# tridivb/attention_based_tbn

Hardware: AMD Instinct MI355X
Metric: clips/sec (3-seg RGB+Flow+Audio TBN fwd+bwd) (higher is better)
Workload: dtype f32; 1 GPU; BASELINE config 4: RGB+Flow+Audio async, attention off, 3 segments, 224x224 frames + 1.279 s (256x256) spectrogram, train step fwd+loss+bwd+clip+SGD; batch_per_gpu=32, global_batch=32, segments=3, parallelism=single, launch_plans=committed (bench_plans.json)

## Files before the change

### attention_based_tbn_amd/_lib.py

```python
import ctypes as C
import os

_HERE = os.path.dirname(os.path.abspath(__file__))
LIB_PATH = os.path.join(_HERE, "libtbn_hip.so")
if os.environ.get("TBN_LIB"):
    import sys as _sys
    LIB_PATH = os.path.abspath(os.environ["TBN_LIB"])
    print(f"[tbn] TBN_LIB set: loading {LIB_PATH} instead of the shipped libtbn_hip.so", file=_sys.stderr)

c_fp = C.c_void_p
c_i = C.c_int
c_sz = C.c_size_t
c_f = C.c_float


class ConvInfo(C.Structure):
    _fields_ = [("name", C.c_char * 64), ("cin", c_i), ("cout", c_i), ("ksize", c_i), ("stride", c_i),
                ("pad", c_i), ("weight_offset", c_sz), ("channel_offset", c_sz)]


class BackboneParams(C.Structure):
    _fields_ = [("weight", c_fp), ("bias", c_fp), ("gamma", c_fp), ("beta", c_fp), ("running_mean", c_fp),
                ("running_var", c_fp), ("momentum", c_f), ("eps", c_f), ("side_stream", c_fp), ("flags", c_i),
                ("weight_planes", c_fp)]
# ... 44 lines not shown
    _fields_ = [("param", c_fp), ("grad", c_fp), ("exp_avg", c_fp), ("exp_avg_sq", c_fp), ("count", c_sz),
                ("step_size", c_f), ("inv_sqrt_bc2", c_f)]


class JpegGeometry(C.Structure):
    _fields_ = [("width", c_i), ("height", c_i), ("components", c_i), ("hsamp", c_i * 3), ("vsamp", c_i * 3),
                ("blocks_w", c_i * 3), ("blocks_h", c_i * 3), ("restart_interval", c_i), ("coef_count", c_sz)]


class FramesClip(C.Structure):
    _fields_ = [("first_img", c_i), ("box_x", c_i), ("box_y", c_i), ("box_w", c_i), ("box_h", c_i), ("resized_w", c_i),
                ("resized_h", c_i), ("crop_x", c_i), ("crop_y", c_i), ("flip", c_i), ("out_row", c_i), ("reserved", c_i)]


SIGNATURES = {
    "tbn_version": (c_i, []),
    "tbn_capabilities": (c_i, []),
    "tbn_last_error": (C.c_char_p, []),
    "tbn_profile_enable": (c_i, [c_i]),
    "tbn_profile_reset": (c_i, []),
    "tbn_profile_num_entries": (c_i, []),
    "tbn_profile_entry": (c_i, [c_i, C.c_char_p, c_i, C.POINTER(C.c_long), C.POINTER(C.c_double),
                                C.POINTER(C.c_double)]),
    "tbn_profile_entry_bytes": (c_i, [c_i, C.POINTER(C.c_double)]),
    "tbn_timeline_enable": (c_i, [c_i]),
    "tbn_timeline_dump": (c_i, [C.c_char_p]),
    "tbn_diag_mfma_burst": (c_i, [c_fp, c_i, c_i, C.POINTER(C.c_double), c_fp]),
    "tbn_backbone_plan_create": (c_i, [c_i, c_i, c_i, c_i, C.POINTER(C.c_void_p)]),
    "tbn_backbone_plan_destroy": (None, [C.c_void_p]),
    "tbn_backbone_num_convs": (c_i, [C.c_void_p]),
    "tbn_backbone_conv_info": (c_i, [C.c_void_p, c_i, C.POINTER(ConvInfo)]),
    "tbn_backbone_weight_floats": (c_sz, [C.c_void_p]),
    "tbn_backbone_channel_floats": (c_sz, [C.c_void_p]),
    "tbn_backbone_workspace_bytes": (c_sz, [C.c_void_p, c_i]),
    "tbn_backbone_out_shape": (c_i, [C.c_void_p, C.POINTER(c_i), C.POINTER(c_i), C.POINTER(c_i)]),
    "tbn_backbone_num_streams": (c_i, [C.c_void_p]),
    "tbn_backbone_rider_launches": (c_i, [C.c_void_p, C.POINTER(c_i), C.POINTER(c_i)]),
    "tbn_backbone_tensor_info": (c_i, [C.c_void_p, C.c_char_p, c_i, C.POINTER(C.c_long), C.POINTER(c_i),
                                       C.POINTER(c_i), C.POINTER(c_i)]),
    "tbn_backbone_launch_info": (c_i, [C.c_void_p, C.c_char_p, c_i, C.POINTER(c_i)]),
    "tbn_backbone_plan_export_bytes": (c_sz, [C.c_void_p]),
    "tbn_backbone_plan_export": (c_i, [C.c_void_p, C.c_void_p, c_sz]),
    "tbn_backbone_plan_import": (c_i, [C.c_void_p, C.c_void_p, c_sz]),
    "tbn_backbone_plan_fingerprint": (C.c_ulonglong, [C.c_void_p]),
    "tbn_backbone_forward": (c_i, [C.c_void_p, c_i, c_fp, C.POINTER(BackboneParams), c_fp, c_sz,
                                   C.POINTER(C.c_void_p), c_fp]),
    "tbn_backbone_weight_planes_bytes": (c_sz, [C.c_void_p, c_i]),
    "tbn_backbone_split_weights": (c_i, [C.c_void_p, c_fp, c_i, c_fp, c_fp]),
    "tbn_backbone_autotune": (c_i, [C.c_void_p, c_i, C.POINTER(BackboneParams), c_fp, c_sz, c_fp]),
    "tbn_backbone_backward": (c_i, [C.c_void_p, c_fp, C.POINTER(BackboneParams), C.POINTER(BackboneGrads), c_fp,
                                    c_sz, c_fp]),
    "tbn_backbone_flip_weights": (c_i, [C.c_void_p, C.POINTER(BackboneParams), c_fp, c_sz, c_fp]),
    "tbn_conv2d_fwd": (c_i, [c_fp, c_i, c_fp, c_fp, c_fp, c_i] + [c_i] * 10 + [c_fp, c_fp, c_fp, c_fp]),
    "tbn_conv2d_stat_tiles": (c_i, [c_i] * 8),
    "tbn_conv_weight_planes_bytes": (c_sz, [c_i, c_i, c_i, c_i]),
    "tbn_conv_split_weights": (c_i, [c_fp, c_i, c_i, c_i, c_i, c_fp, c_fp]),
    "tbn_conv2d_fwd_tile": (c_i, [c_fp, c_i, c_fp, c_fp, c_fp, c_i] + [c_i] * 10 + [c_fp, c_i, c_i, c_fp]),
    "tbn_conv2d_dgrad": (c_i, [c_fp, c_i, c_fp, c_fp, c_i] + [c_i] * 9 + [c_fp, c_fp]),
    "tbn_conv_partial_rows": (c_i, [C.POINTER(ConvDesc), c_i, c_i]),
    "tbn_conv_launch": (c_i, [C.POINTER(ConvDesc), c_i, c_i, c_fp, c_fp]),
    "tbn_conv_launch_pair": (c_i, [C.POINTER(ConvDesc), C.POINTER(ConvDesc), c_i, c_i, c_i, c_fp, c_fp, c_fp]),
    "tbn_conv2d_wgrad_workspace_floats": (c_sz, [c_i] * 8),
    "tbn_conv2d_wgrad": (c_i, [c_fp, c_i, c_fp, c_i, c_fp] + [c_i] * 8 + [c_fp, c_fp]),
    "tbn_stem_geometry": (c_i, [c_i, c_i, c_i, c_i, C.POINTER(c_i)]),
    "tbn_stem_workspace_floats": (c_sz, [c_i] * 6),
    "tbn_stem_conv_fwd": (c_i, [c_fp, c_fp, c_fp, c_fp] + [c_i] * 8 + [c_fp, c_fp, c_fp] + [c_i] * 3 + [c_fp, c_fp]),
    "tbn_stem_conv_wgrad": (c_i, [c_fp, c_i, c_fp, c_fp] + [c_i] * 8 + [c_fp, c_fp]),
    "tbn_linear_fwd": (c_i, [c_fp, c_i, c_fp, c_fp, c_fp, c_i, c_i, c_i, c_i, c_i, c_fp]),
    "tbn_linear_dgrad": (c_i, [c_fp, c_i, c_fp, c_fp, c_i, c_i, c_i, c_i, c_i, c_fp, c_fp]),
    "tbn_linear_wgrad_workspace_floats": (c_sz, [c_i, c_i, c_i]),
    "tbn_linear_wgrad": (c_i, [c_fp, c_i, c_fp, c_i, c_fp, c_fp, c_i, c_i, c_i, c_fp, c_fp]),
    "tbn_bn_workspace_floats": (c_sz, [c_i, c_i]),
    "tbn_bn_relu_train_fwd": (c_i, [c_fp, c_i, c_i, c_fp, c_fp, c_fp, c_fp, c_f, c_f, c_fp, c_fp, c_fp, c_fp, c_fp,
                                    c_i, c_fp, c_fp]),
    "tbn_bn_relu_train_bwd": (c_i, [c_fp, c_i, c_fp, c_i, c_i, c_fp, c_fp, c_fp, c_fp, c_fp, c_fp, c_fp, c_fp, c_fp]),
    "tbn_bn_stats_partials": (c_i, [c_fp, c_i, c_i, c_i, c_fp, C.POINTER(c_i), c_fp]),
    "tbn_bn_fwd_batch": (c_i, [C.POINTER(BnFwdDesc), c_i, c_f, c_f, c_fp]),
    "tbn_bn_bwd_partial_floats": (c_sz, [c_i, c_i]),
    "tbn_bn_bwd_batch": (c_i, [C.POINTER(BnBwdDesc), c_i, c_fp]),
    "tbn_bn_relu_maxpool_train_fwd": (c_i, [c_fp, c_i, c_i, c_i, c_i, c_fp, c_fp, c_fp, c_fp, c_f, c_f, c_fp, c_fp, c_fp,
                                            c_fp, c_fp, c_i, c_fp, c_i, c_i, c_i, c_i, c_fp, c_fp]),
    "tbn_bn_relu_maxpool_train_bwd": (c_i, [c_fp, c_i, c_fp, c_fp, c_i, c_i, c_i, c_i, c_i, c_i, c_i, c_i, c_fp, c_fp,
                                            c_fp, c_fp, c_fp, c_fp, c_fp, c_fp, c_fp]),
    "tbn_bn_res_apply": (c_i, [c_fp, c_i, c_i, c_i, c_fp, c_fp, c_fp, c_i, c_i, c_fp, c_i, c_fp]),
    "tbn_bn_res_fwd": (c_i, [c_fp, c_i, c_i, c_i, c_fp, c_i, c_i, c_fp, c_fp, c_fp, c_fp, c_f, c_f, c_fp, c_fp, c_fp,
                             c_fp, c_fp, c_i, c_i, c_fp, c_i, c_fp]),
    "tbn_bn_res_bwd_workspace_floats": (c_sz, [c_i, c_i]),
    "tbn_bn_res_bwd": (c_i, [c_fp, c_i, c_fp, c_i, c_fp, c_i, c_i, c_i, c_fp, c_fp, c_fp, c_i, c_fp, c_i, c_fp, c_i, c_i,
                             c_fp, c_fp, c_fp, c_fp]),
    "tbn_maxpool3_fwd": (c_i, [c_fp, c_i, c_fp, c_i, c_fp] + [c_i] * 8 + [c_fp]),
    "tbn_maxpool3_bwd": (c_i, [c_fp, c_i, c_fp, c_fp, c_i] + [c_i] * 9 + [c_fp]),
    "tbn_avgpool3_fwd": (c_i, [c_fp, c_i, c_fp, c_i] + [c_i] * 5 + [c_fp]),
    "tbn_spatial_mean_fwd": (c_i, [c_fp, c_i, c_fp, c_i] + [c_i] * 5 + [c_fp]),
    "tbn_spatial_mean_bwd": (c_i, [c_fp, c_i, c_fp, c_i] + [c_i] * 5 + [c_fp]),
    "tbn_pe_concat_fwd": (c_i, [c_fp, c_i, c_fp, c_fp, c_i, c_i, c_i, c_i, c_i, c_fp]),
    "tbn_groupnorm_fwd": (c_i, [c_fp, c_fp, c_fp, c_fp, c_fp, c_fp, c_i, c_i, c_i, c_i, c_f, c_fp]),
    "tbn_groupnorm_bwd": (c_i, [c_fp] * 8 + [c_i] * 4 + [c_fp]),
    "tbn_colsum": (c_i, [c_fp, c_i, c_fp, c_i, c_i, c_fp]),
    "tbn_mha_q1_fwd": (c_i, [c_fp] * 6 + [c_i] * 4 + [c_f, c_fp]),
    "tbn_mha_q1_bwd": (c_i, [c_fp] * 8 + [c_i] * 4 + [c_f, c_fp]),
    "tbn_mha_fwd": (c_i, [c_fp, c_i, c_fp, c_i, c_fp, c_i, c_fp, c_fp, c_i, c_fp, c_fp] + [c_i] * 5 + [c_f, c_fp]),
    "tbn_mha_bwd": (c_i, [c_fp, c_i, c_fp, c_fp, c_i, c_fp, c_i, c_fp, c_i, c_fp, c_fp, c_fp, c_fp, c_i, c_fp, c_i, c_fp,
                          c_i] + [c_i] * 5 + [c_f, c_fp]),
    "tbn_attn_weights_fwd": (c_i, [c_fp, c_i, c_fp, c_f, c_i, c_fp, c_fp, c_fp, c_i, c_i, c_i, c_fp]),
    "tbn_attn_weights_bwd": (c_i, [c_fp, c_fp, c_fp, c_f, c_fp, c_i, c_i, c_i, c_fp]),
    "tbn_attn_reg_fwd": (c_i, [c_fp, c_i, c_fp, c_i, c_i, c_i, c_i, c_i, c_i, c_f, c_i, c_f, c_f, c_f, c_i, c_f, c_i, c_fp, c_fp,
                               c_fp]),
    "tbn_attn_reg_bwd": (c_i, [c_fp, c_fp, c_i, c_fp, c_i, c_fp, c_i, c_i, c_i, c_i, c_i, c_f, c_i, c_f, c_f, c_f, c_i, c_f,
                               c_i, c_fp, c_i, c_fp]),
    "tbn_weighted_sum_fwd": (c_i, [c_fp, c_fp, c_fp, c_i, c_i, c_i, c_i, c_fp]),
    "tbn_weighted_sum_bwd": (c_i, [c_fp, c_i, c_fp, c_fp, c_i, c_i, c_i, c_fp]),
    "tbn_segment_mean_fwd": (c_i, [c_fp, c_fp, c_i, c_i, c_i, c_fp]),
    "tbn_segment_mean_bwd": (c_i, [c_fp, c_fp, c_i, c_i, c_i, c_fp]),
    "tbn_dropout_fwd": (c_i, [c_fp, c_fp, c_f, c_fp, c_fp, c_sz, c_fp]),
    "tbn_ce_heads_fwd": (c_i, [c_fp, c_i, c_i, c_i, C.POINTER(c_i), C.POINTER(c_i), C.POINTER(C.c_void_p), c_fp, c_fp, c_fp, c_fp]),
    "tbn_ce_heads_bwd": (c_i, [c_fp, c_i, c_i, c_i, C.POINTER(c_i), C.POINTER(c_i), c_fp, c_fp, c_fp]),
    "tbn_mul_mask": (c_i, [c_fp, c_fp, c_fp, c_sz, c_fp]),
    "tbn_relu_mask_bwd": (c_i, [c_fp, c_fp, c_fp, c_fp, c_sz, c_fp]),
    "tbn_stft_twiddle_floats": (c_sz, []),
    "tbn_stft_make_twiddle": (c_i, [c_fp]),
    "tbn_stft_logpower": (c_i, [c_fp, c_i, c_i, c_fp, c_fp, c_f, c_fp]),
    "tbn_stft_windows": (c_i, [c_fp, c_fp, c_i, c_i, c_fp, c_fp, c_f, c_i, c_fp, c_fp, c_fp]),
    "tbn_attn_prior_loud": (c_i, [c_fp, c_i, c_i, c_i, c_i, c_fp, c_fp, c_fp]),
    "tbn_opt_num_partials": (c_i, [C.POINTER(OptTensor), c_i]),
    "tbn_opt_sqnorm_partials": (c_i, [C.POINTER(OptTensor), c_i, c_fp, c_fp]),
    "tbn_opt_clip_coef": (c_i, [c_fp, c_i, c_f, c_fp, c_fp, c_fp]),
    "tbn_opt_scale_grads": (c_i, [C.POINTER(OptTensor), c_i, c_fp, c_fp]),
    "tbn_opt_sgd_step": (c_i, [C.POINTER(OptTensor), c_i, c_f, c_f, c_f, c_fp, c_fp]),
    "tbn_opt_adam_step": (c_i, [C.POINTER(AdamTensor), c_i, c_f, c_f, c_f, c_f, c_fp, c_fp]),
    "tbn_topk_correct": (c_i, [c_fp, c_i, c_fp, c_i, c_i, c_i, c_fp, c_fp, c_fp, c_fp]),
    "tbn_frames_to_tensor": (c_i, [c_fp] + [c_i] * 16 + [c_fp, c_fp, c_i, c_i, c_fp, c_fp]),
    "tbn_frames_to_tensor_crops": (c_i, [c_fp] + [c_i] * 10 + [C.POINTER(c_i), C.POINTER(c_i)] + [c_i] * 5 +
                                   [c_fp, c_fp, c_i, c_i, c_fp, c_fp]),
    "tbn_frames_to_tensor_batch": (c_i, [c_fp] + [c_i] * 4 + [C.POINTER(FramesClip), c_fp] + [c_i] * 5 +
                                   [c_fp, c_fp, c_i, c_i, c_fp, c_i, c_fp]),
    "tbn_jpeg_parse": (c_i, [C.c_char_p, c_sz, C.POINTER(JpegGeometry)]),
    "tbn_jpeg_entropy_decode": (c_i, [C.c_char_p, c_sz, C.POINTER(JpegGeometry), c_fp, c_fp]),
    "tbn_jpeg_workspace_bytes": (c_sz, [C.POINTER(JpegGeometry), c_i]),
    "tbn_jpeg_reconstruct": (c_i, [c_fp, c_fp, c_i, C.POINTER(JpegGeometry), c_i, c_fp, c_fp, c_fp]),
    "tbn_jpeg_scan_pack_bytes": (c_sz, [c_sz, c_i]),
    "tbn_jpeg_scan_pack": (c_i, [C.c_char_p, c_sz, C.POINTER(JpegGeometry), c_fp, c_sz, c_i, c_fp, C.POINTER(c_i),
                                 C.POINTER(c_sz)]),
    "tbn_jpeg_entropy_workspace_bytes": (c_sz, [C.POINTER(JpegGeometry), c_i]),
    "tbn_jpeg_entropy_decode_dev": (c_i, [c_fp, c_sz, c_fp, c_i, C.POINTER(JpegGeometry), c_i, c_fp, c_fp, c_fp, c_fp, c_fp]),
}

_lib = None


class TbnHipError(RuntimeError):
    pass


def lib():
    global _lib
    if _lib is None:
        if not os.path.exists(LIB_PATH):
            raise TbnHipError(
                f"{LIB_PATH} not found: build it with `python -m attention_based_tbn_amd.build` "
                "(hipcc --offload-arch=gfx950).  There is no CPU fallback for the TBN hot path.")
        import torch
        handle = C.CDLL(LIB_PATH)
        for name, (res, args) in SIGNATURES.items():
            fn = getattr(handle, name)
            fn.restype = res
            fn.argtypes = args
        _lib = handle
# ... 35 lines not shown
```

### attention_based_tbn_amd/core/models/bn_inception.py

```python
import ctypes as C
import os
import weakref
from collections import OrderedDict

import torch
import torch.nn as nn

from ... import _lib
from ..._lib import BUCKET_CB, BackboneGrads, BackboneParams, ConvInfo, TbnHipError, call, lib, ptr, stream_ptr
from ... import ops

_BLOCKS = [("3a", True, True), ("3b", True, True), ("3c", False, False), ("4a", True, True), ("4b", True, True),
           ("4c", True, True), ("4d", True, True), ("4e", False, False), ("5a", True, True), ("5b", True, True)]


def reference_conv_order():
    names = ["conv1_7x7_s2", "conv2_3x3_reduce", "conv2_3x3"]
    for b, has1, hasp in _BLOCKS:
        p = "inception_" + b
        if has1:
            names.append(p + "_1x1")
        names += [p + "_3x3_reduce", p + "_3x3", p + "_double_3x3_reduce", p + "_double_3x3_1", p + "_double_3x3_2"]
        if hasp:
            names.append(p + "_pool_proj")
# ... 156 lines not shown
            module._last_flip = weakref.ref(f)
        ctx.need_grad = need_grad
        ctx.eval_mode = not training
        return out

    @staticmethod
    def backward(ctx, dout):
        if ctx.needs_input_grad[0]:
            raise TbnHipError("BNInception: the gradient with respect to the input frames is not implemented (the "
                              "first conv's data gradient is never formed); detach the input")
        if not ctx.need_grad:
            if ctx.eval_mode and any(ctx.needs_input_grad[1:7]):
                raise TbnHipError("BNInception: backward through an eval-mode backbone (running-statistics BN) is not "
                                  "implemented; call .train() for fine-tuning or wrap inference in torch.no_grad()")
            return (None,) * 9
        weight, bias, gamma, beta = ctx.saved_tensors
        plan, ws, module = ctx.plan, ctx.ws, ctx.module
        N, H, W, Cc = plan.out_shape
        st = stream_ptr()
        if ctx.freq_only or dout.dim() != 2 or dout.stride(1) != 1 or dout.dtype != torch.float32:
            dout = dout.contiguous().float()
        dout_ld = Cc if ctx.freq_only else dout.stride(0)
        dfeat = torch.empty(plan.out_shape, device=dout.device, dtype=torch.float32)
        call("tbn_spatial_mean_bwd", ptr(dout), dout_ld, ptr(dfeat), Cc, N, H, W, Cc, int(ctx.freq_only), st)
        dw = torch.empty_like(weight)
        db = torch.empty_like(bias)
        need = ctx.needs_input_grad
        bn_first, bn_rest = need[3] or need[5], need[4] or need[6]
        dg = torch.zeros_like(gamma) if (bn_first or bn_rest) else None
        dbe = torch.zeros_like(beta) if (bn_first or bn_rest) else None
        flipped = ctx.flip.done and ctx.flip.version == weight._version
        prm = BackboneParams(ptr(weight), ptr(bias), ptr(gamma), ptr(beta), ptr(module.running_mean),
                             ptr(module.running_var), 0.1, 1e-5, module._side_stream_ptr(),
                             module._engine_flags() | (4 if flipped else 0))
        aux = 0
        if module.use_aux_stream and not torch.cuda.is_current_stream_capturing():
            cur = torch.cuda.current_stream()
            a = module._aux_streams.get(cur.cuda_stream)
            if a is None:
                a = module._aux_streams[cur.cuda_stream] = torch.cuda.Stream(device=dout.device)
            aux = a.cuda_stream
        bucket_fn = module.grad_bucket_fn if need[1] else None
        waits, failure = [], []

        def on_bucket(_user, first, count):
            try:
                w = bucket_fn(module.flat_weight, dw, int(first), int(first) + int(count))
                if w is not None:
                    waits.append(w)
            except BaseException as e:
                failure.append(e)

        cb = BUCKET_CB(on_bucket) if bucket_fn is not None else BUCKET_CB()
        grads = BackboneGrads(ptr(dw), ptr(db), ptr(dg), ptr(dbe), 2 if bn_rest else (1 if bn_first else 0), aux, cb, 0)
        call("tbn_backbone_backward", plan.handle, ptr(dfeat), C.byref(prm), C.byref(grads), ptr(ws), ws.numel(), st)
        ctx.token = None
        for w in waits:
            w()
        if failure:
            raise failure[0]
        n0 = module.first_bn_channels
        return (None, dw if need[1] else None, db if need[2] else None,
                dg[:n0] if need[3] else None, dg[n0:] if need[4] else None,
                dbe[:n0] if need[5] else None, dbe[n0:] if need[6] else None, None, None)


class BNInception(nn.Module):

    def __init__(self, num_classes=1000, in_channels=3):
        super().__init__()
        self.in_channels = in_channels
        self.num_classes = num_classes
        self.is_audio = False
        self.attend = False
        self.feature_size = 1024
        self.eval_chunk = 256
        self.autotune = True
        self.use_aux_stream = True
        self._aux_streams = {}
        self.use_branch_streams = True
        self._side_streams = {}
        self.use_riders = True
        self.stem_wgrad_last = False
        self._conv_math = "f32"
        self._conv_math_layers = "3x3"
        self._planes = None
        self._planes_key = None
        self._last_flip = None
        self._out_slot = None
        self.plan_sync = None
        self.grad_bucket_fn = None
        self._plans = OrderedDict()
        probe = C.c_void_p()
        call("tbn_backbone_plan_create", in_channels, 1, 64, 64, C.byref(probe))
        self._layers = OrderedDict()
        info = ConvInfo()
        for i in range(lib().tbn_backbone_num_convs(probe)):
            call("tbn_backbone_conv_info", probe, i, C.byref(info))
            self._layers[info.name.decode()] = dict(cin=info.cin, cout=info.cout, k=info.ksize, stride=info.stride,
                                                    pad=info.pad, w_off=info.weight_offset, c_off=info.channel_offset)
        nw, nc = lib().tbn_backbone_weight_floats(probe), lib().tbn_backbone_channel_floats(probe)
        lib().tbn_backbone_plan_destroy(probe)
        order = reference_conv_order()
        assert sorted(order) == sorted(self._layers), "engine layer table does not match the reference graph"
        self._order = order
        assert self._layers["conv1_7x7_s2"]["c_off"] == 0
        self.first_bn_channels = self._layers["conv1_7x7_s2"]["cout"]
        n0 = self.first_bn_channels
        self.flat_weight = nn.Parameter(torch.empty(nw))
        self.flat_bias = nn.Parameter(torch.empty(nc))
        self.bn_weight_first = nn.Parameter(torch.ones(n0))
        self.bn_weight_rest = nn.Parameter(torch.ones(nc - n0))
        self.bn_bias_first = nn.Parameter(torch.zeros(n0))
        self.bn_bias_rest = nn.Parameter(torch.zeros(nc - n0))
        self.register_buffer("running_mean", torch.zeros(nc))
        self.register_buffer("running_var", torch.ones(nc))
        self.register_buffer("num_batches_tracked", torch.zeros(len(order), dtype=torch.long))
        self.last_linear = nn.Linear(1024, num_classes)
        self.reset_parameters()

    def reset_parameters(self):
        with torch.no_grad():
            for name, L in self._layers.items():
                w = self.conv_weight(name)
                nn.init.kaiming_uniform_(w, a=5 ** 0.5)
                bound = 1.0 / (L["cin"] * L["k"] * L["k"]) ** 0.5
                self.flat_bias[L["c_off"]:L["c_off"] + L["cout"]].uniform_(-bound, bound)
            torch.autograd.graph.increment_version(self.flat_weight)

    def conv_weight(self, name):
        L = self._layers[name]
        n = L["cout"] * L["k"] * L["k"] * L["cin"]
        return self.flat_weight.data[L["w_off"]:L["w_off"] + n].view(L["cout"], L["k"], L["k"], L["cin"]).permute(
            0, 3, 1, 2)

    def _chan(self, name, flat_first, flat_rest=None):
        L = self._layers[name]
        a, b = L["c_off"], L["c_off"] + L["cout"]
        if flat_rest is None:
            return flat_first.data[a:b]
        n0 = self.first_bn_channels
        return flat_first.data[a:b] if b <= n0 else flat_rest.data[a - n0:b - n0]

    def reference_param_views(self, flat):
        n0 = self.first_bn_channels
        for name in self._order:
            L = self._layers[name]
            n = L["cout"] * L["k"] * L["k"] * L["cin"]
            a, b = L["c_off"], L["c_off"] + L["cout"]
            yield name + ".weight", flat["flat_weight"][L["w_off"]:L["w_off"] + n].view(
                L["cout"], L["k"], L["k"], L["cin"]).permute(0, 3, 1, 2)
            yield name + ".bias", flat["flat_bias"][a:b]
            first = b <= n0
            yield name + "_bn.weight", (flat["bn_weight_first"][a:b] if first else flat["bn_weight_rest"][a - n0:b - n0])
            yield name + "_bn.bias", (flat["bn_bias_first"][a:b] if first else flat["bn_bias_rest"][a - n0:b - n0])

    def named_reference_tensors(self):
        for i, name in enumerate(self._order):
            yield name + ".weight", self.conv_weight(name)
            yield name + ".bias", self._chan(name, self.flat_bias)
            yield name + "_bn.weight", self._chan(name, self.bn_weight_first, self.bn_weight_rest)
            yield name + "_bn.bias", self._chan(name, self.bn_bias_first, self.bn_bias_rest)
            yield name + "_bn.running_mean", self._chan(name, self.running_mean)
            yield name + "_bn.running_var", self._chan(name, self.running_var)
            yield name + "_bn.num_batches_tracked", self.num_batches_tracked[i]

# ... 19 lines not shown
                    continue
                dst.copy_(src)
            torch.autograd.graph.increment_version(self.flat_weight)
        if strict:
            child_prefixes = tuple(prefix + n + "." for n, _ in self.named_children())
            for key in state_dict:
                if key.startswith(prefix) and key not in own and not key.startswith(child_prefixes):
                    unexpected_keys.append(key)

    def set_bn_trainable(self, first, rest):
        self.bn_weight_first.requires_grad = self.bn_bias_first.requires_grad = first
        self.bn_weight_rest.requires_grad = self.bn_bias_rest.requires_grad = rest

    def _plan(self, frames, h, w):
        key = (frames, h, w)
        if key not in self._plans:
            if len(self._plans) >= 4:
                self._plans.popitem(last=False)
            self._plans[key] = _Plan(self.in_channels, frames, h, w)
        else:
            self._plans.move_to_end(key)
        return self._plans[key]

    def plan_fingerprints(self):
        return {k: p.fingerprint() for k, p in self._plans.items()}

    def flip_weights_early(self):
        f = self._last_flip() if getattr(self, "_last_flip", None) is not None else None
        self._last_flip = None
        if f is None or f.done or f.weight._version != f.version or torch.cuda.is_current_stream_capturing():
            return False
        prm = BackboneParams(ptr(f.weight), 0, 0, 0, 0, 0, 0.1, 1e-5, 0, 0)
        call("tbn_backbone_flip_weights", f.plan.handle, C.byref(prm), ptr(f.ws), f.ws.numel(), stream_ptr())
        f.done = True
        return True

    CONV_MATH = {"f32": 0, "bf16x6": 8, "bf16x3": 16}

    @property
    def conv_math(self):
        return self._conv_math

    @conv_math.setter
    def conv_math(self, value):
        if value not in self.CONV_MATH:
            raise ValueError("conv_math must be one of %s, got %r" % (", ".join(map(repr, self.CONV_MATH)), value))
        self._conv_math = value
        if value == "f32":
            self._planes = self._planes_key = None

    CONV_MATH_LAYERS = ("3x3", "all")

    @property
    def conv_math_layers(self):
        return self._conv_math_layers

    @conv_math_layers.setter
    def conv_math_layers(self, value):
        if value not in self.CONV_MATH_LAYERS:
            raise ValueError("conv_math_layers must be one of %s, got %r"
                             % (", ".join(map(repr, self.CONV_MATH_LAYERS)), value))
        self._conv_math_layers = value
        if value != "all":
            self._planes = self._planes_key = None

    def _planes_on(self):
        return not self.training and self._conv_math != "f32" and self._conv_math_layers == "all"

    def _weight_planes(self, plan):
        w = self.flat_weight
        np_ = 6 if self._conv_math == "bf16x6" else 3
        key = (w.data_ptr(), w._version, self._conv_math)
        nbytes = lib().tbn_backbone_weight_planes_bytes(plan.handle, np_)
        if self._planes is None or self._planes.numel() != nbytes or self._planes.device != w.device:
            self._planes, self._planes_key = torch.empty(nbytes, dtype=torch.uint8, device=w.device), None
        capturing = torch.cuda.is_current_stream_capturing()
        if self._planes_key != key or capturing:
            call("tbn_backbone_split_weights", plan.handle, ptr(w), np_, ptr(self._planes), stream_ptr())
            if not capturing:
                self._planes_key = key
        return self._planes

    def _engine_flags(self):
        return ((1 if self.use_riders else 0) | (2 if self.stem_wgrad_last else 0)
                | (0 if self.training else self.CONV_MATH[self._conv_math]) | (32 if self._planes_on() else 0))

    def _side_stream_ptr(self):
        if not self.use_branch_streams or torch.cuda.is_current_stream_capturing():
            return 0
        cur = torch.cuda.current_stream()
        s = self._side_streams.get(cur.cuda_stream)
        if s is None:
            s = self._side_streams[cur.cuda_stream] = torch.cuda.Stream(device=cur.device)
        return s.cuda_stream

    def _run(self, x, freq_only):
        if not x.is_cuda:
            raise TbnHipError("BNInception: input is on the CPU; this backbone only runs on an MI355X via "
                              "libtbn_hip.so (no CPU fallback)")
        x = x.contiguous().float()
        args = (self.flat_weight, self.flat_bias, self.bn_weight_first, self.bn_weight_rest, self.bn_bias_first,
                self.bn_bias_rest, self, freq_only)
        if self.training or x.shape[0] <= self.eval_chunk:
            return _BackboneFn.apply(x, *args)
        outs = [_BackboneFn.apply(x[i:i + self.eval_chunk], *args) for i in range(0, x.shape[0], self.eval_chunk)]
        return torch.cat(outs, 0)

    def forward(self, x):
        freq = bool(self.is_audio and self.attend)
        out = self._run(x, freq)
        if freq:
            return out.permute(0, 2, 1).unsqueeze(2)
        return out

    def forward_sequence(self, x):
        return self._run(x, True)

    def features(self, x):
        x = x.contiguous().float()
        plan = self._plan(x.shape[0], x.shape[2], x.shape[3])
        ws = plan.workspace(False, x.device)
        gamma = torch.cat([self.bn_weight_first, self.bn_weight_rest])
        beta = torch.cat([self.bn_bias_first, self.bn_bias_rest])
        if self.training:
            raise TbnHipError("features(): only available in eval mode; use forward() for training")
        prm = BackboneParams(ptr(self.flat_weight), ptr(self.flat_bias), ptr(gamma), ptr(beta),
                             ptr(self.running_mean), ptr(self.running_var), 0.1, 1e-5, 0,
                             self.CONV_MATH[self._conv_math] | (32 if self._planes_on() else 0))
        if self._planes_on():
            prm.weight_planes = ptr(self._weight_planes(plan))
        feat_ptr = C.c_void_p()
        call("tbn_backbone_forward", plan.handle, 0, ptr(x), C.byref(prm), ptr(ws), ws.numel(), C.byref(feat_ptr),
             stream_ptr())
        N, H, W, Cc = plan.out_shape
        off = (feat_ptr.value - ws.data_ptr()) // 4
        nhwc = ws.view(torch.float32)[off:off + N * H * W * Cc].view(N, H, W, Cc).clone()
        return nhwc.permute(0, 3, 1, 2)

    def logits(self, features):
        nhwc = features.permute(0, 2, 3, 1).contiguous()
        if self.is_audio and self.attend:
            return ops.spatial_mean(nhwc, True).permute(0, 2, 1).unsqueeze(2)
        return ops.spatial_mean(nhwc, False)


def bninception(in_channels, modality, pretrained="imagenet", model_dir="", is_audio=False, attend=False,
                state_dict=None):
    num_classes = 1000
    data_dict = state_dict
    if pretrained is not None:
        if pretrained == "kinetics":
            num_classes = 400
            file = os.path.join(model_dir, "kinetics_bninception_flow.pth")
        elif pretrained == "imagenet":
            file = os.path.join(model_dir, "imagenet_bninception_rgb.pth")
        if data_dict is None:
            data_dict = torch.load(file, map_location="cpu")
    model = BNInception(num_classes=num_classes, in_channels=in_channels)
    if data_dict is not None:
        data_dict = dict(data_dict)
        if modality == "Audio":
            data_dict["conv1_7x7_s2.weight"] = data_dict["conv1_7x7_s2.weight"].mean(dim=1).unsqueeze(dim=1)
            own = model.state_dict()
            for k in [k for k in own.keys() if k not in data_dict]:
                data_dict[k] = own[k]
            for k in [k for k in data_dict.keys() if k not in own]:
                del data_dict[k]
# ... 8 lines not shown
```

### attention_based_tbn_amd/csrc/api.hip

```cpp
#include <cstdarg>
#include <cstdio>
#include <cstdlib>
#include <cstring>

#include "tbn_common.h"
#include "tbn_kernels.h"
#include "../../include/tbn_hip.h"

static thread_local char g_err[512] = "";

void tbn_set_error(const char* fmt, ...) {
  va_list ap;
  va_start(ap, fmt);
  vsnprintf(g_err, sizeof(g_err), fmt, ap);
  va_end(ap);
}

#if TBN_EXPERIMENT
int tbn_env_int(const char* name, int def, int lo, int hi) {
  const char* e = getenv(name);
  if (e == nullptr || *e == 0) return def;
  char* end = nullptr;
  const long v = strtol(e, &end, 10);
  if (end == e || *end != 0 || v < lo || v > hi) {
// ... 7 lines not shown

#define TBN_TRY(expr)                \
  do {                               \
    int rc__ = (expr);               \
    if (rc__ != TBN_OK) return rc__; \
  } while (0)

static void conv_geom(ConvP* p, int n, int h, int w, int cin, int cout, int k, int stride, int pad) {
  memset(p, 0, sizeof(*p));
  p->N = n;
  p->H = h;
  p->W = w;
  p->OH = (h + 2 * pad - k) / stride + 1;
  p->OW = (w + 2 * pad - k) / stride + 1;
  p->Cin = cin;
  p->Cout = cout;
  p->R = p->S = k;
  p->stride = stride;
  p->pad = pad;
  p->up = 1;
  p->M = n * p->OH * p->OW;
  p->K = k * k * cin;
}

#include <map>
#include <atomic>
#include <mutex>
#include <string>
#include <vector>
namespace {
struct ProfRec {
  int name;
  double flops, bytes;
  hipEvent_t a, b;
  bool used;
};
struct ProfAgg {
  long launches = 0;
  double ms = 0, flops = 0, bytes = 0;
};
std::mutex g_prof_mu;
bool g_prof_on = false;
bool g_prof_layers = false;
std::string g_prof_label;
thread_local const char* g_prof_prefix = nullptr;
std::vector<std::string> g_prof_names;
std::vector<ProfRec> g_prof_recs;
std::vector<hipEvent_t> g_prof_pool;
std::map<std::string, ProfAgg> g_prof_agg;
std::vector<std::string> g_prof_keys;
int g_prof_open = -1;

hipEvent_t prof_event() {
  if (!g_prof_pool.empty()) {
    hipEvent_t e = g_prof_pool.back();
    g_prof_pool.pop_back();
    return e;
  }
  hipEvent_t e = nullptr;
  (void)hipEventCreate(&e);
  return e;
}
void prof_collect() {
  for (auto& r : g_prof_recs) {
    if (r.used) {
      (void)hipEventSynchronize(r.b);
      float ms = 0.f;
      (void)hipEventElapsedTime(&ms, r.a, r.b);
      ProfAgg& a = g_prof_agg[g_prof_names[r.name]];
      a.launches += 1;
      a.ms += ms;
      a.flops += r.flops;
      a.bytes += r.bytes;
    }
    g_prof_pool.push_back(r.a);
    g_prof_pool.push_back(r.b);
  }
  g_prof_recs.clear();
  g_prof_keys.clear();
  for (auto& kv : g_prof_agg) g_prof_keys.push_back(kv.first);
}
}

void tbn_prof_begin(const char* kernel, double flops, hipStream_t st, double bytes) {
  if (!g_prof_on) return;
  std::lock_guard<std::mutex> lk(g_prof_mu);
  std::string key = g_prof_prefix ? std::string(g_prof_prefix) + kernel : std::string(kernel);
  if (g_prof_layers) key += " | " + g_prof_label;
  kernel = key.c_str();
  int idx = -1;
  for (size_t i = 0; i < g_prof_names.size(); ++i)
    if (g_prof_names[i] == kernel) idx = (int)i;
  if (idx < 0) {
    g_prof_names.push_back(kernel);
    idx = (int)g_prof_names.size() - 1;
  }
  ProfRec r;
  r.name = idx;
  r.flops = flops;
  r.bytes = bytes;
  r.a = prof_event();
  r.b = prof_event();
  r.used = false;
  (void)st;
  g_prof_recs.push_back(r);
  g_prof_open = (int)g_prof_recs.size() - 1;
}
bool tbn_prof_enabled() { return g_prof_on; }

namespace {
struct TlRec {
  std::string name;
  void* stream;
  hipEvent_t a, b;
};
std::mutex g_tl_mu;
std::atomic<bool> g_tl_on{false};
std::vector<TlRec> g_tl;
void tl_free_events() {
  for (auto& r : g_tl) {
    if (r.a) (void)hipEventDestroy(r.a);
    if (r.b) (void)hipEventDestroy(r.b);
  }
  g_tl.clear();
}
}
bool tbn_tl_on(hipStream_t st) {
  if (!g_tl_on.load(std::memory_order_relaxed)) return false;
  hipStreamCaptureStatus cs = hipStreamCaptureStatusNone;
  if (hipStreamIsCapturing(st, &cs) != hipSuccess) {
    (void)hipGetLastError();
    return false;
  }
  return cs == hipStreamCaptureStatusNone;
}
void tbn_tl_events(const char* name, hipStream_t st, hipEvent_t* start, hipEvent_t* stop) {
  std::lock_guard<std::mutex> lk(g_tl_mu);
  TlRec r;
  r.name = name;
  r.stream = (void*)st;
  r.a = r.b = nullptr;
  (void)hipEventCreate(&r.a);
  (void)hipEventCreate(&r.b);
  *start = r.a;
  *stop = r.b;
  g_tl.push_back(r);
}
extern "C" int tbn_timeline_enable(int on) {
  std::lock_guard<std::mutex> lk(g_tl_mu);
  if (on) {
    (void)hipDeviceSynchronize();
    tl_free_events();
  }
  g_tl_on.store(on != 0, std::memory_order_relaxed);
  return TBN_OK;
}
extern "C" int tbn_timeline_dump(const char* path) {
  TBN_REQUIRE(path != nullptr, "timeline_dump: null path");
  (void)hipDeviceSynchronize();
  std::lock_guard<std::mutex> lk(g_tl_mu);
  FILE* f = fopen(path, "w");
  TBN_REQUIRE(f != nullptr, "timeline_dump: cannot open %s", path);
  fprintf(f, "Kernel_Name,Queue_Id,Start_Timestamp,End_Timestamp\n");
  if (!g_tl.empty()) {
    const hipEvent_t ref = g_tl[0].a;
    for (auto& r : g_tl) {
      float a = 0.f, d = 0.f;
      if (hipEventElapsedTime(&a, ref, r.a) != hipSuccess || hipEventElapsedTime(&d, r.a, r.b) != hipSuccess) {
        (void)hipGetLastError();
        continue;
      }
      std::string nm = r.name;
      for (auto& ch : nm)
        if (ch == ',' || ch == '"') ch = ';';
      const long long s0 = (long long)((double)a * 1e6) + 1000000000ll;
      fprintf(f, "%s,%p,%lld,%lld\n", nm.c_str(), r.stream, s0, s0 + (long long)((double)d * 1e6));
    }
  }
  fclose(f);
  if (!g_tl_on.load(std::memory_order_relaxed)) tl_free_events();
  return TBN_OK;
}
bool tbn_prof_launch_events(hipEvent_t* start, hipEvent_t* stop) {
  if (!g_prof_on) return false;
  std::lock_guard<std::mutex> lk(g_prof_mu);
  if (g_prof_open < 0 || g_prof_recs[g_prof_open].used || !g_prof_recs[g_prof_open].a || !g_prof_recs[g_prof_open].b)
    return false;
  g_prof_recs[g_prof_open].used = true;
  *start = g_prof_recs[g_prof_open].a;
  *stop = g_prof_recs[g_prof_open].b;
  return true;
}
void tbn_prof_label(const char* label) {
  if (!g_prof_on || !g_prof_layers) return;
  std::lock_guard<std::mutex> lk(g_prof_mu);
  g_prof_label = label;
}
void tbn_prof_end(hipStream_t st) {
  if (!g_prof_on) return;
  std::lock_guard<std::mutex> lk(g_prof_mu);
  (void)st;
  g_prof_open = -1;
}

__global__ __launch_bounds__(256) void mfma_burst_kernel(float* sink, int iters) {
  f32x16 a0, a1, a2, a3;
#pragma unroll
  for (int e = 0; e < 16; ++e) a0[e] = a1[e] = a2[e] = a3[e] = 0.f;
  const float x = 1e-3f * (float)(threadIdx.x & 63) + 0.5f, y = 1.0f - 1e-3f * (float)(threadIdx.x >> 6);
  for (int i = 0; i < iters; ++i) {
#pragma unroll
    for (int k = 0; k < 4; ++k) {
      a0 = __builtin_amdgcn_mfma_f32_32x32x2f32(x, y, a0, 0, 0, 0);
      a1 = __builtin_amdgcn_mfma_f32_32x32x2f32(y, x, a1, 0, 0, 0);
      a2 = __builtin_amdgcn_mfma_f32_32x32x2f32(x, x, a2, 0, 0, 0);
      a3 = __builtin_amdgcn_mfma_f32_32x32x2f32(y, y, a3, 0, 0, 0);
    }
  }
  float s = 0.f;
#pragma unroll
  for (int e = 0; e < 16; ++e) s += (a0[e] + a1[e]) + (a2[e] + a3[e]);
  if (s == -1.2345f) sink[0] = s;
}

extern "C" {

int tbn_version(void) { return 102 | (TBN_EXPERIMENT ? 0x10000 : 0); }

int tbn_capabilities(void) { return TBN_CAP_CONV_BF16X | TBN_CAP_CONV_BF16X_PLANES | TBN_CAP_FRAMES_CROPS | TBN_CAP_ATTN_GENERAL | TBN_CAP_ATTN_REG | TBN_CAP_AUDIO_LAYER | TBN_CAP_STEM_OPS | TBN_CAP_BN_BATCH_OPS; }

int tbn_diag_mfma_burst(float* sink, int workgroups, int iters, double* flops, void* stream) {
  TBN_REQUIRE(sink != nullptr && workgroups > 0 && workgroups <= 65536 && iters > 0, "diag_mfma_burst: bad argument");
  hipLaunchKernelGGL(mfma_burst_kernel, dim3(workgroups), dim3(256), 0, (hipStream_t)stream, sink, iters);
  TBN_CHECK_LAUNCH("mfma_burst");
  if (flops) *flops = (double)workgroups * 4.0 * (double)iters * 16.0 * 4096.0;
  return TBN_OK;
}

int tbn_profile_enable(int on) {
  std::lock_guard<std::mutex> lk(g_prof_mu);
  g_prof_on = on != 0;
  g_prof_layers = on == 2;
  return TBN_OK;
}
int tbn_profile_reset(void) {
  std::lock_guard<std::mutex> lk(g_prof_mu);
  prof_collect();
  g_prof_agg.clear();
  g_prof_keys.clear();
  return TBN_OK;
}
int tbn_profile_num_entries(void) {
  std::lock_guard<std::mutex> lk(g_prof_mu);
  prof_collect();
  return (int)g_prof_keys.size();
}
int tbn_profile_entry(int i, char* name, int name_len, long* launches, double* total_ms, double* total_flops) {
  std::lock_guard<std::mutex> lk(g_prof_mu);
  TBN_REQUIRE(i >= 0 && i < (int)g_prof_keys.size() && name && name_len > 0, "profile_entry: bad index");
  const ProfAgg& a = g_prof_agg[g_prof_keys[i]];
  snprintf(name, name_len, "%s", g_prof_keys[i].c_str());
  if (launches) *launches = a.launches;
  if (total_ms) *total_ms = a.ms;
  if (total_flops) *total_flops = a.flops;
  return TBN_OK;
}
int tbn_profile_entry_bytes(int i, double* total_alg_bytes) {
  std::lock_guard<std::mutex> lk(g_prof_mu);
  TBN_REQUIRE(i >= 0 && i < (int)g_prof_keys.size() && total_alg_bytes, "profile_entry_bytes: bad index");
  *total_alg_bytes = g_prof_agg[g_prof_keys[i]].bytes;
  return TBN_OK;
}
const char* tbn_last_error(void) { return g_err; }

int tbn_conv2d_stat_tiles(int n, int h, int w, int cin, int cout, int ksize, int stride, int pad) {
  ConvP p;
  conv_geom(&p, n, h, w, cin, cout, ksize, stride, pad);
  int mt, nt;
  tbn_conv_pick_tile(p.M, p.Cout, p.K, &mt, &nt);
  return cdiv(p.M, 128 * mt);
}
// ... 352 lines not shown
  wp.dy = dy;
  wp.dy_ld = dy_ld;
  wp.x = image;
  wp.N = n;
  wp.H = g.H;
  wp.W = g.W;
  wp.OH = g.OH;
  wp.OW = g.OW;
  wp.Cin = g.rows * g.kw;
  wp.Cout = cout;
  wp.R = g.rows;
  wp.S = 1;
  wp.taps = 1;
  wp.stride = g.stride;
  wp.pad = g.pad;
  wp.M = n * g.OH * g.OW;
  wp.cp = wp.x_ld = g.cp;
  wp.rl = g.kw;
  wp.mt = mt;
  wp.nt = nt;
  wp.alg_flops = 2.0 * wp.M * (double)cout * 49 * cin;
  TBN_TRY(tbn_launch_wgrad(wp, 1, dwpack, workspace + ws.wsplit, st));
  if (g.mode == 1) return tbn_launch_unpack_stem_wgrad_rows(dwpack, dweight, cout, cin, g.kw, st);
  return tbn_launch_unpack_stem_wgrad_s2d(dwpack, dweight, cout, cin, st);
}

namespace {
struct ProfPrefix {
  explicit ProfPrefix(const char* p) { g_prof_prefix = p; }
  ~ProfPrefix() { g_prof_prefix = nullptr; }
};
}

int tbn_linear_fwd(const float* x, int x_ld, const float* w, const float* bias, float* out, int out_ld, int m, int k,
                   int n, int relu, void* stream) {
  ProfPrefix scope("linear: ");
  return tbn_conv2d_fwd(x, x_ld, w, bias, out, out_ld, m, 1, 1, k, n, 1, 1, 0, CONV_EPI_PLAIN,
                        relu ? CONV_FLAG_RELU : 0, nullptr, nullptr, nullptr, stream);
}

int tbn_linear_dgrad(const float* dy, int dy_ld, const float* w, float* dx, int dx_ld, int m, int k, int n,
                     int accumulate, float* workspace, void* stream) {
  ProfPrefix scope("linear: ");
  return tbn_conv2d_dgrad(dy, dy_ld, w, dx, dx_ld, m, 1, 1, k, n, 1, 1, 0, accumulate, workspace, stream);
}

size_t tbn_linear_wgrad_workspace_floats(int m, int k, int n) { return tbn_wgrad_workspace_floats(m, n, k, 1); }

int tbn_linear_wgrad(const float* dy, int dy_ld, const float* x, int x_ld, float* dw, float* dbias, int m, int k,
                     int n, float* workspace, void* stream) {
  ProfPrefix scope("linear: ");
  TBN_TRY(tbn_conv2d_wgrad(dy, dy_ld, x, x_ld, dw, m, 1, 1, k, n, 1, 1, 0, workspace, stream));
  if (dbias) TBN_TRY(tbn_colsum(dy, dy_ld, dbias, m, n, stream));
  return TBN_OK;
}

size_t tbn_bn_workspace_floats(int p, int c) { return (size_t)tbn_bn_stats_parts(p, c) * 2 * c + 3 * (size_t)c; }

int tbn_bn_relu_train_fwd(const float* y, int p, int c, const float* gamma, const float* beta, float* running_mean,
                          float* running_var, float momentum, float eps, float* save_mean, float* save_rstd,
                          float* scale, float* shift, float* z, int z_ld, float* workspace, void* stream) {
  hipStream_t st = (hipStream_t)stream;
  int parts = 0;
  TBN_TRY(tbn_launch_bn_stats(y, c, p, c, workspace, &parts, st));
  TBN_TRY(tbn_launch_bn_finalize(workspace, parts, p, c, gamma, beta, nullptr, running_mean, running_var, momentum, eps,
                                 save_mean, save_rstd, scale, shift, st));
  Seg s;
  s.ptr = z;
  s.ld = z_ld;
  s.col_begin = 0;
  return tbn_launch_bn_apply(y, p, c, scale, shift, &s, 1, st);
}

int tbn_bn_relu_train_bwd(const float* dz, int dz_ld, const float* y, int p, int c, const float* save_mean,
                          const float* save_rstd, const float* scale, const float* shift, float* dy, float* dgamma,
                          float* dbeta, float* workspace, void* stream) {
  hipStream_t st = (hipStream_t)stream;
  CSeg s;
  s.ptr = dz;
  s.ld = dz_ld;
  s.col_begin = 0;
  const int parts = tbn_bn_bwd_parts(p, c);
  float* coef = workspace + (size_t)parts * 2 * c;
  TBN_TRY(tbn_launch_bn_bwd_reduce(&s, 1, y, p, c, scale, shift, save_mean, save_rstd, workspace, st));
  TBN_TRY(tbn_launch_bn_bwd_finalize(workspace, parts, p, c, scale, save_mean, save_rstd, coef, dgamma, dbeta, nullptr,
                                     st));
  return tbn_launch_bn_bwd_apply(&s, 1, y, p, c, scale, shift, coef, dy, st);
}

int tbn_bn_stats_partials(const float* y, int y_ld, int p, int c, float* partial, int* nparts, void* stream) {
  TBN_REQUIRE(y && partial && nparts, "bn_stats_partials: null pointer");
  return tbn_launch_bn_stats(y, y_ld, p, c, partial, nparts, (hipStream_t)stream);
}

size_t tbn_bn_bwd_partial_floats(int p, int c) {
  if (p < 1 || c < 4 || c > 1024 || c % 4 != 0) return 0;
  return (size_t)tbn_bn_bwd_parts(p, c) * 2 * c;
}

int tbn_bn_fwd_batch(const tbn_bn_fwd_desc* members, int n, float momentum, float eps, void* stream) {
  TBN_REQUIRE(members != nullptr, "bn_fwd_batch: null pointer");
  static thread_local BnFwdBatch b;
  memset(&b, 0, sizeof(b));
  b.n = n;
  b.momentum = momentum;
  b.eps = eps;
  for (int i = 0; i < n && n <= TBN_BN_MAXL; ++i) {
    const tbn_bn_fwd_desc& d = members[i];
    TBN_REQUIRE(d.y && d.partial && d.gamma && d.beta && d.save_mean && d.save_rstd && d.scale && d.shift,
                "bn_fwd_batch: null pointer in member %d", i);
    TBN_REQUIRE(d.running_mean == nullptr || d.running_var != nullptr, "bn_fwd_batch: member %d has running_mean without running_var", i);
    BnFwdLayer& L = b.l[i];
    L.y = d.y; L.y_ld = d.y_ld; L.P = d.p; L.C = d.c;
    L.partial = d.partial; L.pld = d.pld; L.nparts = d.nparts;
    L.gamma = d.gamma; L.beta = d.beta; L.conv_bias = d.conv_bias;
    L.running_mean = d.running_mean; L.running_var = d.running_var;
    L.save_mean = d.save_mean; L.save_rstd = d.save_rstd; L.scale = d.scale; L.shift = d.shift;
    L.nseg = d.nseg;
    for (int s = 0; s < 3 && s < d.nseg; ++s) {
      TBN_REQUIRE(d.seg[s].ptr != nullptr, "bn_fwd_batch: null pointer in segment %d of member %d", s, i);
      L.seg[s].ptr = d.seg[s].ptr; L.seg[s].ld = d.seg[s].ld; L.seg[s].col_begin = d.seg[s].col_begin;
    }
  }
  return tbn_launch_bn_fwd_multi(b, (hipStream_t)stream);
}

int tbn_bn_bwd_batch(const tbn_bn_bwd_desc* members, int n, void* stream) {
  TBN_REQUIRE(members != nullptr, "bn_bwd_batch: null pointer");
  static thread_local BnBwdBatch b;
  memset(&b, 0, sizeof(b));
  b.n = n;
  for (int i = 0; i < n && n <= TBN_BN_MAXL; ++i) {
    const tbn_bn_bwd_desc& d = members[i];
    TBN_REQUIRE(d.y && d.dy && d.scale && d.shift && d.mean && d.rstd && d.partial && d.coef,
                "bn_bwd_batch: null pointer in member %d", i);
    BnBwdLayer& L = b.l[i];
    L.nseg = d.nseg;
    for (int s = 0; s < 3 && s < d.nseg; ++s) {
      TBN_REQUIRE(d.dz[s].ptr != nullptr, "bn_bwd_batch: null pointer in segment %d of member %d", s, i);
      L.dz[s].ptr = d.dz[s].ptr; L.dz[s].ld = d.dz[s].ld; L.dz[s].col_begin = d.dz[s].col_begin;
    }
    L.y = d.y; L.dy = d.dy; L.y_ld = d.y_ld; L.P = d.p; L.C = d.c;
    L.scale = d.scale; L.shift = d.shift; L.mean = d.mean; L.rstd = d.rstd;
    L.partial = d.partial; L.ext_parts = d.ext_parts; L.coef = d.coef;
    L.dgamma = d.dgamma; L.dbeta = d.dbeta; L.dbias = d.dbias;
  }
  return tbn_launch_bn_bwd_multi(b, (hipStream_t)stream);
}

int tbn_bn_relu_maxpool_train_fwd(const float* y, int n, int h, int w, int c, const float* gamma, const float* beta,
                                  float* running_mean, float* running_var, float momentum, float eps, float* save_mean,
                                  float* save_rstd, float* scale, float* shift, float* pooled, int pooled_ld,
                                  uint8_t* argmax, int oh, int ow, int stride, int pad, float* workspace, void* stream) {
  hipStream_t st = (hipStream_t)stream;
  TBN_REQUIRE(y && pooled && argmax && workspace, "bn_relu_maxpool_train_fwd: null pointer");
  const int p = n * h * w;
  int parts = 0;
  TBN_TRY(tbn_launch_bn_stats(y, c, p, c, workspace, &parts, st));
  TBN_TRY(tbn_launch_bn_finalize(workspace, parts, p, c, gamma, beta, nullptr, running_mean, running_var, momentum, eps,
                                 save_mean, save_rstd, scale, shift, st));
  return tbn_launch_bn_apply_maxpool(y, n, h, w, c, scale, shift, pooled, pooled_ld, argmax, oh, ow, stride, pad, st);
}

int tbn_bn_relu_maxpool_train_bwd(const float* dpooled, int dpooled_ld, const uint8_t* argmax, const float* y, int n, int h,
                                  int w, int c, int oh, int ow, int stride, int pad, const float* save_mean,
                                  const float* save_rstd, const float* scale, const float* shift, float* dy,
                                  float* dgamma, float* dbeta, float* workspace, void* stream) {
  hipStream_t st = (hipStream_t)stream;
  TBN_REQUIRE(dpooled && argmax && y && dy && workspace, "bn_relu_maxpool_train_bwd: null pointer");
  const int p = n * h * w;
  const int parts = tbn_bn_bwd_pooled_parts(n, h, w, c, stride, pad);
  TBN_REQUIRE(parts <= tbn_bn_bwd_parts(p, c), "bn_relu_maxpool_train_bwd: workspace sized by tbn_bn_workspace_floats is too small");
  float* coef = workspace + (size_t)tbn_bn_bwd_parts(p, c) * 2 * c;
  TBN_TRY(tbn_launch_bn_bwd_reduce_pooled(dpooled, dpooled_ld, argmax, n, h, w, oh, ow, stride, pad, y, c, scale, shift,
                                          save_mean, save_rstd, workspace, st));
  TBN_TRY(tbn_launch_bn_bwd_finalize(workspace, parts, p, c, scale, save_mean, save_rstd, coef, dgamma, dbeta, nullptr, st));
  return tbn_launch_bn_bwd_apply_pooled(dpooled, dpooled_ld, argmax, n, h, w, oh, ow, stride, pad, y, c, scale, shift, coef,
                                        dy, st);
}

int tbn_maxpool3_fwd(const float* in, int in_ld, float* out, int out_ld, uint8_t* argmax, int n, int h, int w, int c,
                     int oh, int ow, int stride, int pad, void* stream) {
  return tbn_launch_maxpool_fwd(in, in_ld, out, out_ld, argmax, n, h, w, c, oh, ow, stride, pad, (hipStream_t)stream);
}
int tbn_maxpool3_bwd(const float* dout, int dout_ld, const uint8_t* argmax, float* din, int din_ld, int n, int h,
                     int w, int c, int oh, int ow, int stride, int pad, int accumulate, void* stream) {
  return tbn_launch_maxpool_bwd(dout, dout_ld, argmax, din, din_ld, n, h, w, c, oh, ow, stride, pad, accumulate,
                                (hipStream_t)stream);
}
int tbn_avgpool3_fwd(const float* in, int in_ld, float* out, int out_ld, int n, int h, int w, int c, int accumulate,
                     void* stream) {
  return tbn_launch_avgpool3_fwd(in, in_ld, out, out_ld, n, h, w, c, accumulate, (hipStream_t)stream);
}
int tbn_spatial_mean_fwd(const float* in, int in_ld, float* out, int out_ld, int n, int h, int w, int c,
                         int freq_only, void* stream) {
  return tbn_launch_spatial_mean_fwd(in, in_ld, out, out_ld, n, h, w, c, freq_only, (hipStream_t)stream);
}
int tbn_spatial_mean_bwd(const float* dout, int dout_ld, float* din, int din_ld, int n, int h, int w, int c,
                         int freq_only, void* stream) {
  return tbn_launch_spatial_mean_bwd(dout, dout_ld, din, din_ld, n, h, w, c, freq_only, (hipStream_t)stream);
}

}
```

### attention_based_tbn_amd/csrc/bn.hip

```cpp
#include "tbn_common.h"
#include "tbn_kernels.h"
#include "tbn_bn_dev.h"
#include "tbn_pool_dev.h"

static inline int pick_chunk(int P, int rp) {
  int pch = cdiv(P, 512);
  if (pch < 64) pch = 64;
  return cdiv(pch, rp) * rp;
}

__global__ __launch_bounds__(256) void bn_stats_kernel(const float* __restrict__ y, int ld, int P, int C, int pch,
                                                       float* __restrict__ partial) {
  __shared__ float red[2 * 2048];
  const int G = C >> 2, RP = 256 / G;
  const int tid = threadIdx.x, cg = tid % G, rs = tid / G;
  const int p0 = blockIdx.x * pch, p1 = min(P, p0 + pch);
  float4 s1 = make_float4(0, 0, 0, 0), s2 = s1;
  if (rs < RP)
    for (int p = p0 + rs; p < p1; p += RP) {
      const float4 v = *reinterpret_cast<const float4*>(y + (size_t)p * ld + cg * 4);
      s1.x += v.x; s1.y += v.y; s1.z += v.z; s1.w += v.w;
      s2.x = fmaf(v.x, v.x, s2.x); s2.y = fmaf(v.y, v.y, s2.y); s2.z = fmaf(v.z, v.z, s2.z); s2.w = fmaf(v.w, v.w, s2.w);
    }
  if (rs < RP) {
// ... 57 lines not shown
    }
  }
}

int tbn_launch_bn_finalize(const float* partial, int nparts, int P, int C, const float* gamma, const float* beta,
                           const float* conv_bias, float* running_mean, float* running_var, float momentum, float eps,
                           float* save_mean, float* save_rstd, float* scale, float* shift, hipStream_t st) {
  TBN_KLAUNCH(bn_finalize_kernel, dim3(cdiv(C, TBN_FIN_CH)), dim3(256), 0, st, partial, nparts, P, C, gamma, beta,
                     conv_bias, running_mean, running_var, momentum, eps, save_mean, save_rstd, scale, shift);
  TBN_CHECK_LAUNCH("bn_finalize");
  return TBN_OK;
}

struct Seg3 {
  Seg s[3];
  int n;
};
struct CSeg3 {
  CSeg s[3];
  int n;
};

__global__ __launch_bounds__(256) void bn_apply_kernel(const float* __restrict__ y, int P, int C,
                                                       const float* __restrict__ scale,
                                                       const float* __restrict__ shift, Seg3 segs, FastDiv divg) {
  const int G = C >> 2;
  const uint32_t total = (uint32_t)P * G;
  for (uint32_t i = blockIdx.x * 256u + threadIdx.x; i < total; i += gridDim.x * 256u) {
    const int p = (int)fdiv(i, divg), c = (int)(i - (uint32_t)p * (uint32_t)G) * 4;
    const float4 v = *reinterpret_cast<const float4*>(y + (size_t)p * C + c);
    const float4 sc = *reinterpret_cast<const float4*>(scale + c);
    const float4 sh = *reinterpret_cast<const float4*>(shift + c);
    float4 z;
    z.x = fmaxf(fmaf(v.x, sc.x, sh.x), 0.f);
    z.y = fmaxf(fmaf(v.y, sc.y, sh.y), 0.f);
    z.z = fmaxf(fmaf(v.z, sc.z, sh.z), 0.f);
    z.w = fmaxf(fmaf(v.w, sc.w, sh.w), 0.f);
    int sg = 0;
    if (segs.n > 1 && c >= segs.s[1].col_begin) sg = 1;
    if (segs.n > 2 && c >= segs.s[2].col_begin) sg = 2;
    *reinterpret_cast<float4*>(segs.s[sg].ptr + (size_t)p * segs.s[sg].ld + (c - segs.s[sg].col_begin)) = z;
  }
}

static inline int ew_grid(size_t items) {
  size_t g = (items + 255) / 256;
  return (int)(g > 4096 ? 4096 : (g < 1 ? 1 : g));
}

int tbn_launch_bn_apply(const float* y, int P, int C, const float* scale, const float* shift, const Seg* segs,
                        int nseg, hipStream_t st) {
  TBN_REQUIRE(C % 4 == 0 && nseg >= 1 && nseg <= 3, "bn_apply: bad C/nseg");
  Seg3 s3;
  s3.n = nseg;
  for (int i = 0; i < nseg; ++i) {
    s3.s[i] = segs[i];
    TBN_REQUIRE(segs[i].ld % 4 == 0 && segs[i].col_begin % 4 == 0, "bn_apply: segment pitch/offset must be x4");
  }
  TBN_REQUIRE((size_t)P * (C / 4) < (1ull << 31), "bn_apply: too many elements per call");
  TBN_KLAUNCH(bn_apply_kernel, dim3(ew_grid((size_t)P * C / 4)), dim3(256), 0, st, y, P, C, scale, shift, s3,
                     make_fastdiv((uint32_t)(C / 4)));
  TBN_CHECK_LAUNCH("bn_apply");
  return TBN_OK;
}

__global__ void bn_fold_kernel(const float* gamma, const float* beta, const float* mean, const float* var,
                               const float* bias, float eps, float* scale, float* shift, int C) {
  const int c = blockIdx.x * blockDim.x + threadIdx.x;
  if (c < C) {
    const float sc = gamma[c] / sqrtf(var[c] + eps);
    scale[c] = sc;
    shift[c] = fmaf((bias != nullptr ? bias[c] : 0.f) - mean[c], sc, beta[c]);
  }
}

int tbn_launch_bn_fold(const float* gamma, const float* beta, const float* mean, const float* var, const float* bias,
                       float eps, float* scale, float* shift, int C, hipStream_t st) {
  TBN_KLAUNCH(bn_fold_kernel, dim3(cdiv(C, 256)), dim3(256), 0, st, gamma, beta, mean, var, bias, eps, scale,
                     shift, C);
  TBN_CHECK_LAUNCH("bn_fold");
  return TBN_OK;
}

__global__ __launch_bounds__(256) void bn_apply_maxpool_kernel(const float* __restrict__ y, int N, int H, int W, int C,
                                                               const float* __restrict__ scale,
                                                               const float* __restrict__ shift,
                                                               float* __restrict__ out, int out_ld,
                                                               unsigned char* __restrict__ argmax, int OH, int OW,
                                                               int stride, int pad, PixDecode dec) {
  const int G = C >> 2;
  const uint32_t total = (uint32_t)N * OH * OW * G;
  const unsigned nb = gridDim.x, bid = blockIdx.x;
  const unsigned q8 = nb >> 3, r8 = nb & 7, xcd = bid & 7, idx = bid >> 3;
  const uint32_t b0 = (xcd < r8 ? xcd * (q8 + 1) : r8 * (q8 + 1) + (xcd - r8) * q8) + idx;
  for (uint32_t i = b0 * 256u + threadIdx.x; i < total; i += gridDim.x * 256u) {
    int g, ox, oy, n;
    uint32_t opix;
    pix_decode(dec, i, g, ox, oy, n, opix);
    const int y0 = oy * stride - pad, x0 = ox * stride - pad;
    const float4 sc = *reinterpret_cast<const float4*>(scale + g * 4);
    const float4 sh = *reinterpret_cast<const float4*>(shift + g * 4);
    float4 best = make_float4(-INFINITY, -INFINITY, -INFINITY, -INFINITY);
    int bx = 0, by = 0, bz = 0, bw = 0;
#pragma unroll
    for (int r = 0; r < 3; ++r)
#pragma unroll
      for (int s2 = 0; s2 < 3; ++s2) {
        const int iy = y0 + r, ix = x0 + s2;
        if ((unsigned)iy < (unsigned)H && (unsigned)ix < (unsigned)W) {
          const float4 v = *reinterpret_cast<const float4*>(y + ((size_t)(n * H + iy) * W + ix) * C + g * 4);
          float4 z;
          z.x = fmaxf(fmaf(v.x, sc.x, sh.x), 0.f);
          z.y = fmaxf(fmaf(v.y, sc.y, sh.y), 0.f);
          z.z = fmaxf(fmaf(v.z, sc.z, sh.z), 0.f);
          z.w = fmaxf(fmaf(v.w, sc.w, sh.w), 0.f);
          const int k = r * 3 + s2;
          if (z.x > best.x || z.x != z.x) { best.x = z.x; bx = k; }
          if (z.y > best.y || z.y != z.y) { best.y = z.y; by = k; }
          if (z.z > best.z || z.z != z.z) { best.z = z.z; bz = k; }
          if (z.w > best.w || z.w != z.w) { best.w = z.w; bw = k; }
        }
      }
    *reinterpret_cast<float4*>(out + (size_t)opix * out_ld + g * 4) = best;
    *reinterpret_cast<uint32_t*>(argmax + (size_t)opix * C + g * 4) =
        (uint32_t)bx | ((uint32_t)by << 8) | ((uint32_t)bz << 16) | ((uint32_t)bw << 24);
  }
}

int tbn_launch_bn_apply_maxpool(const float* y, int N, int H, int W, int C, const float* scale, const float* shift,
                                float* out, int out_ld, unsigned char* argmax, int OH, int OW, int stride, int pad,
                                hipStream_t st) {
  TBN_REQUIRE(C % 4 == 0 && out_ld % 4 == 0 && argmax != nullptr, "bn_apply_maxpool: bad C / pitch / argmax");
  size_t g = ((size_t)N * OH * OW * (C / 4) + 255) / 256;
  if (g > 8192) g = 8192;
  TBN_REQUIRE((size_t)N * H * W * (C / 4) < (1ull << 31), "bn_apply_maxpool: too many elements per call");
  TBN_KLAUNCH(bn_apply_maxpool_kernel, dim3((unsigned)(g < 1 ? 1 : g)), dim3(256), 0, st, y, N, H, W, C, scale,
                     shift, out, out_ld, argmax, OH, OW, stride, pad, make_pixdecode(C / 4, OW, OH));
  TBN_CHECK_LAUNCH("bn_apply_maxpool");
  return TBN_OK;
}

struct PoolGrad {
  const float* dout;
  const unsigned char* argmax;
  int dout_ld, H, W, OH, OW, C, stride, pad;
  FastDiv div_w, div_h;
};
__device__ __forceinline__ float4 pooled_grad(const PoolGrad& q, int p, int c) {
  const uint32_t row = fdiv((uint32_t)p, q.div_w);
  const int ix = p - (int)row * q.W;
  const uint32_t n = fdiv(row, q.div_h);
  const int iy = (int)row - (int)n * q.H;
  float4 acc = make_float4(0.f, 0.f, 0.f, 0.f);
  if (q.stride == 2 && q.pad == 0) {
    const int oyA = iy >> 1, ryA = iy & 1, oxA = ix >> 1, rxA = ix & 1;
    const bool vyA = oyA < q.OH, vyB = (ryA == 0) && (oyA >= 1);
    const bool vxA = oxA < q.OW, vxB = (rxA == 0) && (oxA >= 1);
    const int oy[2] = {vyA ? oyA : 0, vyB ? oyA - 1 : 0}, ry[2] = {ryA, 2};
    const int ox[2] = {vxA ? oxA : 0, vxB ? oxA - 1 : 0}, rx[2] = {rxA, 2};
    const bool vy[2] = {vyA, vyB}, vx[2] = {vxA, vxB};
    uint32_t am[4];
    float4 d[4];
#pragma unroll
    for (int a = 0; a < 2; ++a)
#pragma unroll
      for (int b = 0; b < 2; ++b) {
        const size_t opix = (size_t)((int)n * q.OH + oy[a]) * q.OW + ox[b];
        am[a * 2 + b] = *reinterpret_cast<const uint32_t*>(q.argmax + opix * q.C + c);
        d[a * 2 + b] = *reinterpret_cast<const float4*>(q.dout + opix * q.dout_ld + c);
      }
#pragma unroll
    for (int a = 0; a < 2; ++a)
#pragma unroll
      for (int b = 0; b < 2; ++b) {
        const uint32_t k = (uint32_t)(ry[a] * 3 + rx[b]);
        const uint32_t m = am[a * 2 + b];
        const bool v = vy[a] && vx[b];
        if (v && (m & 0xff) == k) acc.x += d[a * 2 + b].x;
        if (v && ((m >> 8) & 0xff) == k) acc.y += d[a * 2 + b].y;
        if (v && ((m >> 16) & 0xff) == k) acc.z += d[a * 2 + b].z;
        if (v && (m >> 24) == k) acc.w += d[a * 2 + b].w;
      }
    return acc;
  }
  const int oy_hi = min(q.OH - 1, (iy + q.pad) / q.stride);
  const int ox_hi = min(q.OW - 1, (ix + q.pad) / q.stride);
  for (int oy = oy_hi; oy >= 0; --oy) {
    const int r = iy - (oy * q.stride - q.pad);
    if (r > 2) break;
    for (int ox = ox_hi; ox >= 0; --ox) {
      const int s = ix - (ox * q.stride - q.pad);
      if (s > 2) break;
      const uint32_t k = (uint32_t)(r * 3 + s);
      const size_t opix = (size_t)((int)n * q.OH + oy) * q.OW + ox;
      const uint32_t am = *reinterpret_cast<const uint32_t*>(q.argmax + opix * q.C + c);
      const float4 d = *reinterpret_cast<const float4*>(q.dout + opix * q.dout_ld + c);
      if ((am & 0xff) == k) acc.x += d.x;
      if (((am >> 8) & 0xff) == k) acc.y += d.y;
      if (((am >> 16) & 0xff) == k) acc.z += d.z;
      if ((am >> 24) == k) acc.w += d.w;
    }
  }
  return acc;
}

template <bool POOLED>
__global__ __launch_bounds__(256) void bn_bwd_reduce_kernel(CSeg3 dz, PoolGrad pg, const float* __restrict__ y, int P,
                                                            int C, int pch, const float* __restrict__ scale,
                                                            const float* __restrict__ shift,
                                                            const float* __restrict__ mean,
                                                            const float* __restrict__ rstd,
                                                            float* __restrict__ partial) {
  __shared__ float red[2 * 2048];
  const int G = C >> 2, RP = 256 / G;
  const int tid = threadIdx.x, cg = tid % G, rs = tid / G, c = cg * 4;
  const int p0 = blockIdx.x * pch, p1 = min(P, p0 + pch);
  float4 s1 = make_float4(0, 0, 0, 0), s2 = s1;
  if (rs < RP) {
    int sg = 0;
    if (dz.n > 1 && c >= dz.s[1].col_begin) sg = 1;
    if (dz.n > 2 && c >= dz.s[2].col_begin) sg = 2;
    const float* dzp = POOLED ? nullptr : dz.s[sg].ptr + (c - dz.s[sg].col_begin);
    const int dld = dz.s[sg].ld;
    const float4 sc = *reinterpret_cast<const float4*>(scale + c);
    const float4 sh = *reinterpret_cast<const float4*>(shift + c);
    const float4 mu = *reinterpret_cast<const float4*>(mean + c);
    const float4 rs4 = *reinterpret_cast<const float4*>(rstd + c);
    for (int p = p0 + rs; p < p1; p += RP) {
      const float4 v = *reinterpret_cast<const float4*>(y + (size_t)p * C + c);
      const float4 d = POOLED ? pooled_grad(pg, p, c) : *reinterpret_cast<const float4*>(dzp + (size_t)p * dld);
      const float gx = fmaf(v.x, sc.x, sh.x) > 0.f ? d.x : 0.f;
      const float gy = fmaf(v.y, sc.y, sh.y) > 0.f ? d.y : 0.f;
      const float gz = fmaf(v.z, sc.z, sh.z) > 0.f ? d.z : 0.f;
      const float gw = fmaf(v.w, sc.w, sh.w) > 0.f ? d.w : 0.f;
      s1.x += gx; s1.y += gy; s1.z += gz; s1.w += gw;
      s2.x = fmaf(gx, (v.x - mu.x) * rs4.x, s2.x);
      s2.y = fmaf(gy, (v.y - mu.y) * rs4.y, s2.y);
      s2.z = fmaf(gz, (v.z - mu.z) * rs4.z, s2.z);
      s2.w = fmaf(gw, (v.w - mu.w) * rs4.w, s2.w);
    }
    *reinterpret_cast<float4*>(&red[(rs * G + cg) * 4]) = s1;
    *reinterpret_cast<float4*>(&red[2048 + (rs * G + cg) * 4]) = s2;
  }
  __syncthreads();
  for (int cc = tid; cc < C; cc += 256) {
    float a = 0.f, b = 0.f;
    for (int r = 0; r < RP; ++r) {
      a += red[r * C + cc];
      b += red[2048 + r * C + cc];
    }
    partial[((size_t)blockIdx.x * 2 + 0) * C + cc] = a;
    partial[((size_t)blockIdx.x * 2 + 1) * C + cc] = b;
  }
}

int tbn_bn_bwd_parts(int P, int C) { return tbn_bn_stats_parts(P, C); }

static int fill_cseg3(CSeg3* o, const CSeg* s, int n) {
  o->n = n;
  for (int i = 0; i < n; ++i) {
    o->s[i] = s[i];
    if (s[i].ld % 4 != 0 || s[i].col_begin % 4 != 0) return -1;
  }
  return 0;
}

int tbn_launch_bn_bwd_reduce(const CSeg* dz, int nseg, const float* y, int P, int C, const float* scale,
                             const float* shift, const float* mean, const float* rstd, float* partial,
                             hipStream_t st) {
  TBN_REQUIRE(C % 4 == 0 && C <= 1024 && nseg >= 1 && nseg <= 3, "bn_bwd_reduce: bad C/nseg");
  CSeg3 s3;
  TBN_REQUIRE(fill_cseg3(&s3, dz, nseg) == 0, "bn_bwd_reduce: segment pitch/offset must be x4");
  const int rp = 256 / (C / 4), pch = pick_chunk(P, rp), parts = cdiv(P, pch);
  PoolGrad none = {};
  TBN_KLAUNCH(bn_bwd_reduce_kernel<false>, dim3(parts), dim3(256), 0, st, s3, none, y, P, C, pch, scale, shift,
                     mean, rstd, partial);
  TBN_CHECK_LAUNCH("bn_bwd_reduce");
  return TBN_OK;
}

static PoolGrad make_poolgrad(const float* dout, int dout_ld, const unsigned char* argmax, int H, int W, int OH, int OW,
                              int C, int stride, int pad) {
  PoolGrad q;
  q.dout = dout; q.argmax = argmax; q.dout_ld = dout_ld;
  q.H = H; q.W = W; q.OH = OH; q.OW = OW; q.C = C; q.stride = stride; q.pad = pad;
  q.div_w = make_fastdiv((uint32_t)W);
  q.div_h = make_fastdiv((uint32_t)H);
  return q;
}

__global__ __launch_bounds__(256) void bn_bwd_reduce_pooled2x2_kernel(PoolBlk pb, const float* __restrict__ y, int NQ,
                                                                       int C, int qch, const float* __restrict__ scale,
                                                                       const float* __restrict__ shift,
                                                                       const float* __restrict__ mean,
                                                                       const float* __restrict__ rstd,
                                                                       float* __restrict__ partial) {
  __shared__ float red[2 * 2048];
  const int G = C >> 2, RP = 256 / G;
  const int tid = threadIdx.x, cg = tid % G, rs = tid / G, c = cg * 4;
  const int q0 = blockIdx.x * qch, q1 = min(NQ, q0 + qch);
  float4 s1 = make_float4(0, 0, 0, 0), s2 = s1;
  if (rs < RP) {
    const float4 sc = *reinterpret_cast<const float4*>(scale + c);
    const float4 sh = *reinterpret_cast<const float4*>(shift + c);
    const float4 mu = *reinterpret_cast<const float4*>(mean + c);
    const float4 rs4 = *reinterpret_cast<const float4*>(rstd + c);
    for (int q = q0 + rs; q < q1; q += RP) {
      const uint32_t row = fdiv((uint32_t)q, pb.div_bw);
      const int bx = q - (int)row * pb.BW;
      const uint32_t n = fdiv(row, pb.div_bh);
      const int by = (int)row - (int)n * pb.BH;
      float4 g[4];
      pooled_grad_2x2(pb, (int)n, by, bx, c, g);
#pragma unroll
      for (int i = 0; i < 4; ++i) {
        const int iy = 2 * by + (i >> 1), ix = 2 * bx + (i & 1);
        if (iy < pb.H && ix < pb.W) {
          const float4 v = *reinterpret_cast<const float4*>(y + ((size_t)((int)n * pb.H + iy) * pb.W + ix) * C + c);
          const float gx = fmaf(v.x, sc.x, sh.x) > 0.f ? g[i].x : 0.f;
          const float gy = fmaf(v.y, sc.y, sh.y) > 0.f ? g[i].y : 0.f;
          const float gz = fmaf(v.z, sc.z, sh.z) > 0.f ? g[i].z : 0.f;
          const float gw = fmaf(v.w, sc.w, sh.w) > 0.f ? g[i].w : 0.f;
          s1.x += gx; s1.y += gy; s1.z += gz; s1.w += gw;
          s2.x = fmaf(gx, (v.x - mu.x) * rs4.x, s2.x);
          s2.y = fmaf(gy, (v.y - mu.y) * rs4.y, s2.y);
          s2.z = fmaf(gz, (v.z - mu.z) * rs4.z, s2.z);
          s2.w = fmaf(gw, (v.w - mu.w) * rs4.w, s2.w);
        }
      }
    }
    *reinterpret_cast<float4*>(&red[(rs * G + cg) * 4]) = s1;
    *reinterpret_cast<float4*>(&red[2048 + (rs * G + cg) * 4]) = s2;
  }
  __syncthreads();
  for (int cc = tid; cc < C; cc += 256) {
    float a = 0.f, b = 0.f;
    for (int r = 0; r < RP; ++r) {
      a += red[r * C + cc];
      b += red[2048 + r * C + cc];
    }
    partial[((size_t)blockIdx.x * 2 + 0) * C + cc] = a;
    partial[((size_t)blockIdx.x * 2 + 1) * C + cc] = b;
  }
}

__global__ __launch_bounds__(256) void bn_bwd_apply_pooled2x2_kernel(PoolBlk pb, const float* y, int NQ, int C,
                                                                      const float* __restrict__ scale,
                                                                      const float* __restrict__ shift,
                                                                      const float* __restrict__ coef, float* dy,
                                                                      FastDiv divg) {
  const int G = C >> 2;
  const uint32_t total = (uint32_t)NQ * G;
  for (uint32_t i = blockIdx.x * 256u + threadIdx.x; i < total; i += gridDim.x * 256u) {
    const uint32_t q = fdiv(i, divg);
    const int c = (int)(i - q * (uint32_t)G) * 4;
    const uint32_t row = fdiv(q, pb.div_bw);
    const int bx = (int)q - (int)row * pb.BW;
    const uint32_t n = fdiv(row, pb.div_bh);
    const int by = (int)row - (int)n * pb.BH;
    float4 g[4];
    pooled_grad_2x2(pb, (int)n, by, bx, c, g);
    const float4 sc = *reinterpret_cast<const float4*>(scale + c);
    const float4 sh = *reinterpret_cast<const float4*>(shift + c);
    const float4 ca = *reinterpret_cast<const float4*>(coef + c);
    const float4 cb = *reinterpret_cast<const float4*>(coef + C + c);
    const float4 cc = *reinterpret_cast<const float4*>(coef + 2 * C + c);
#pragma unroll
    for (int k = 0; k < 4; ++k) {
      const int iy = 2 * by + (k >> 1), ix = 2 * bx + (k & 1);
      if (iy < pb.H && ix < pb.W) {
        const size_t off = ((size_t)((int)n * pb.H + iy) * pb.W + ix) * C + c;
        const float4 v = tbn_ld4<(TBN_BN_NT & 8) != 0>(y + off);
        float4 o;
        o.x = fmaf(ca.x, fmaf(v.x, sc.x, sh.x) > 0.f ? g[k].x : 0.f, fmaf(cb.x, v.x, cc.x));
        o.y = fmaf(ca.y, fmaf(v.y, sc.y, sh.y) > 0.f ? g[k].y : 0.f, fmaf(cb.y, v.y, cc.y));
        o.z = fmaf(ca.z, fmaf(v.z, sc.z, sh.z) > 0.f ? g[k].z : 0.f, fmaf(cb.z, v.z, cc.z));
        o.w = fmaf(ca.w, fmaf(v.w, sc.w, sh.w) > 0.f ? g[k].w : 0.f, fmaf(cb.w, v.w, cc.w));
        *reinterpret_cast<float4*>(dy + off) = o;
      }
    }
  }
}

int tbn_bn_bwd_pooled_parts(int N, int H, int W, int C, int stride, int pad) {
  if (stride == 2 && pad == 0) {
    const int NQ = N * ((H + 1) / 2) * ((W + 1) / 2);
    const int rp = 256 / (C / 4);
    return cdiv(NQ, pick_chunk(NQ, rp));
  }
  return tbn_bn_bwd_parts(N * H * W, C);
}

int tbn_launch_bn_bwd_reduce_pooled(const float* dpooled, int dpooled_ld, const unsigned char* argmax, int N, int H,
                                    int W, int OH, int OW, int stride, int pad, const float* y, int C,
                                    const float* scale, const float* shift, const float* mean, const float* rstd,
                                    float* partial, hipStream_t st) {
  TBN_REQUIRE(C % 4 == 0 && C <= 1024 && dpooled_ld % 4 == 0, "bn_bwd_reduce_pooled: bad C / pitch");
  TBN_REQUIRE((long)N * H * W < (1l << 31), "bn_bwd_reduce_pooled: too many pixels");
  if (stride == 2 && pad == 0) {
    const int NQ = N * ((H + 1) / 2) * ((W + 1) / 2);
    const int rp = 256 / (C / 4), qch = pick_chunk(NQ, rp), parts = cdiv(NQ, qch);
    TBN_KLAUNCH(bn_bwd_reduce_pooled2x2_kernel, dim3(parts), dim3(256), 0, st,
                       make_poolblk(dpooled, dpooled_ld, argmax, H, W, OH, OW, C), y, NQ, C, qch, scale, shift, mean, rstd,
                       partial);
    TBN_CHECK_LAUNCH("bn_bwd_reduce_pooled2x2");
    return TBN_OK;
  }
  const int P = N * H * W;
  CSeg3 s3 = {};
  s3.n = 1;
  const int rp = 256 / (C / 4), pch = pick_chunk(P, rp), parts = cdiv(P, pch);
  TBN_KLAUNCH(bn_bwd_reduce_kernel<true>, dim3(parts), dim3(256), 0, st, s3,
                     make_poolgrad(dpooled, dpooled_ld, argmax, H, W, OH, OW, C, stride, pad), y, P, C, pch, scale,
                     shift, mean, rstd, partial);
  TBN_CHECK_LAUNCH("bn_bwd_reduce_pooled");
  return TBN_OK;
}

__global__ __launch_bounds__(256) void bn_bwd_finalize_kernel(const float* __restrict__ partial, int nparts, int P,
                                                              int C, const float* __restrict__ scale,
                                                              const float* __restrict__ mean,
                                                              const float* __restrict__ rstd, float* coef,
                                                              float* dgamma, float* dbeta, float* dbias) {
  __shared__ double red[64 * 32];
  const int tid = threadIdx.x;
  const int c = blockIdx.x * TBN_FIN_CH + tid;
  double s1, s2;
  tbn_sum_partials<TBN_FIN_CH>(partial, C, nparts, blockIdx.x * TBN_FIN_CH, C, red, &s1, &s2);
  if (tid < TBN_FIN_CH && c < C) {
    const double sc = scale[c], rs = rstd[c], mu = mean[c];
    const double bb = -sc * rs * (s2 / P);
    coef[c] = (float)sc;
    coef[C + c] = (float)bb;
    coef[2 * C + c] = (float)(-sc * (s1 / P) - bb * mu);
    if (dgamma) dgamma[c] = (float)s2;
    if (dbeta) dbeta[c] = (float)s1;
    if (dbias) dbias[c] = 0.f;
  }
}

int tbn_launch_bn_bwd_finalize(const float* partial, int nparts, int P, int C, const float* scale, const float* mean,
                               const float* rstd, float* coef, float* dgamma, float* dbeta, float* dbias,
                               hipStream_t st) {
  TBN_KLAUNCH(bn_bwd_finalize_kernel, dim3(cdiv(C, TBN_FIN_CH)), dim3(256), 0, st, partial, nparts, P, C, scale, mean,
                     rstd, coef, dgamma, dbeta, dbias);
  TBN_CHECK_LAUNCH("bn_bwd_finalize");
  return TBN_OK;
}

template <bool POOLED>
__global__ __launch_bounds__(256) void bn_bwd_apply_kernel(CSeg3 dz, PoolGrad pg, const float* y, int P, int C,
                                                           const float* __restrict__ scale,
                                                           const float* __restrict__ shift,
                                                           const float* __restrict__ coef, float* dy, FastDiv divg) {
  const int G = C >> 2;
  const uint32_t total = (uint32_t)P * G;
  for (uint32_t i = blockIdx.x * 256u + threadIdx.x; i < total; i += gridDim.x * 256u) {
    const int p = (int)fdiv(i, divg), c = (int)(i - (uint32_t)p * (uint32_t)G) * 4;
    int sg = 0;
    if (dz.n > 1 && c >= dz.s[1].col_begin) sg = 1;
    if (dz.n > 2 && c >= dz.s[2].col_begin) sg = 2;
    const float4 d = POOLED ? pooled_grad(pg, p, c)
                            : *reinterpret_cast<const float4*>(dz.s[sg].ptr + (size_t)p * dz.s[sg].ld +
                                                               (c - dz.s[sg].col_begin));
    const float4 v = *reinterpret_cast<const float4*>(y + (size_t)p * C + c);
    const float4 sc = *reinterpret_cast<const float4*>(scale + c);
    const float4 sh = *reinterpret_cast<const float4*>(shift + c);
    const float4 ca = *reinterpret_cast<const float4*>(coef + c);
    const float4 cb = *reinterpret_cast<const float4*>(coef + C + c);
    const float4 cc = *reinterpret_cast<const float4*>(coef + 2 * C + c);
    float4 o;
    o.x = fmaf(ca.x, fmaf(v.x, sc.x, sh.x) > 0.f ? d.x : 0.f, fmaf(cb.x, v.x, cc.x));
    o.y = fmaf(ca.y, fmaf(v.y, sc.y, sh.y) > 0.f ? d.y : 0.f, fmaf(cb.y, v.y, cc.y));
    o.z = fmaf(ca.z, fmaf(v.z, sc.z, sh.z) > 0.f ? d.z : 0.f, fmaf(cb.z, v.z, cc.z));
    o.w = fmaf(ca.w, fmaf(v.w, sc.w, sh.w) > 0.f ? d.w : 0.f, fmaf(cb.w, v.w, cc.w));
    *reinterpret_cast<float4*>(dy + (size_t)p * C + c) = o;
  }
}

int tbn_launch_bn_bwd_apply(const CSeg* dz, int nseg, const float* y, int P, int C, const float* scale,
                            const float* shift, const float* coef, float* dy, hipStream_t st) {
  CSeg3 s3;
  TBN_REQUIRE(C % 4 == 0 && nseg >= 1 && nseg <= 3 && fill_cseg3(&s3, dz, nseg) == 0, "bn_bwd_apply: bad segments");
  PoolGrad none = {};
  TBN_REQUIRE((size_t)P * (C / 4) < (1ull << 31), "bn_bwd_apply: too many elements per call");
  TBN_KLAUNCH(bn_bwd_apply_kernel<false>, dim3(ew_grid((size_t)P * C / 4)), dim3(256), 0, st, s3, none, y, P, C,
                     scale, shift, coef, dy, make_fastdiv((uint32_t)(C / 4)));
  TBN_CHECK_LAUNCH("bn_bwd_apply");
  return TBN_OK;
}

int tbn_launch_bn_bwd_apply_pooled(const float* dpooled, int dpooled_ld, const unsigned char* argmax, int N, int H, int W,
                                   int OH, int OW, int stride, int pad, const float* y, int C, const float* scale,
                                   const float* shift, const float* coef, float* dy, hipStream_t st) {
  TBN_REQUIRE(C % 4 == 0 && dpooled_ld % 4 == 0, "bn_bwd_apply_pooled: bad C / pitch");
  if (stride == 2 && pad == 0) {
// ... 18 lines not shown
```

### attention_based_tbn_amd/csrc/engine.hip

```cpp
#include <string>
#include <vector>
#include <cstring>
#include <cstdio>

#include <cstdlib>
#include "tbn_common.h"
#include "tbn_kernels.h"
#include "../../include/tbn_hip.h"

namespace {

struct BlockSpec {
  const char* name;
  int cin, c1, c3r, c3, cdr, cd1, cd2;
  int pool;
  int cp, stride;
};
const BlockSpec kBlocks[] = {
    {"3a", 192, 64, 64, 64, 64, 96, 96, 0, 32, 1},     {"3b", 256, 64, 64, 96, 64, 96, 96, 0, 64, 1},
    {"3c", 320, 0, 128, 160, 64, 96, 96, 2, 0, 2},     {"4a", 576, 224, 64, 96, 96, 128, 128, 0, 128, 1},
    {"4b", 576, 192, 96, 128, 96, 128, 128, 0, 128, 1}, {"4c", 576, 160, 128, 160, 128, 160, 160, 0, 128, 1},
    {"4d", 608, 96, 128, 192, 160, 192, 192, 0, 128, 1}, {"4e", 608, 0, 128, 192, 192, 256, 256, 2, 0, 2},
    {"5a", 1056, 352, 192, 320, 160, 224, 224, 0, 128, 1}, {"5b", 1024, 352, 192, 320, 192, 224, 224, 1, 128, 1},
};
const int kNumBlocks = 10;
const int kGradBuckets = 2;
const int kBucketBlock[kGradBuckets] = {8, 3};
const int kMaxParts = TBN_CONV_MAXSEG;

struct Buf {
  int H, W, C;
  size_t off, doff;
};

struct Part {
  std::string name;
  int cout, col0;
  int dst_buf, dst_choff;
  size_t c_off;
  bool pooled = false;
  size_t y2_off = 0;
  size_t yraw_off = 0;
  size_t bpart_off = 0;
  int red_src = -1;
  int slot = 0;
  int slot_b = 0;
};

struct Conv {
  int nparts;
  Part parts[kMaxParts];
  int cin, cout, k, stride, pad;
  int inbuf, inH, inW, outH, outW;
  size_t w_off, c_off;
  size_t y_off;
  int slot = 0;
  int slot_b = 0;
  struct FwdTune {
    int mt = 1, nt = 1, stages = 0;
    int halo = 0;
    bool pair = false;
    int p_variant = 1, p_mt = 1, p_nt = 1;
    float t = 0.f;
  } ft[2];
  int d_mt = 1, d_nt = 1, d_stages = 0;
  int d_halo = 0;
  int pair_next = -1, pair_prev = -1;
  bool pair_dgrad = false;
  int pd_variant = 1, pd_mt = 1, pd_nt = 1;
  float t_dgrad = 0.f;
  int w_mt = 0, w_nt = 0;
  bool stem;
  bool dgrad_accum;
  bool need_dgrad;
  int fuse_pool = -1;
  int nred = 0;
  int red_conv[kMaxParts], red_part[kMaxParts];
};

struct Pool {
  int kind;
  int inbuf, outbuf, out_choff, stride, pad;
  size_t argmax_off;
  bool bwd_accum;
  bool fused = false;
};

struct BnStep {
  int n;
  int conv[kMaxParts], part[kMaxParts];
  int slot0 = 0;
};

enum { OP_CONV = 0, OP_POOL = 1, OP_BN = 2, OP_PREPOOL = 3, OP_FORK = 4, OP_JOIN = 5 };
struct Op {
  int kind;
  int idx;
  int part;
  int side;
};

int pool_out(int in, int k, int stride, int pad, bool ceil_mode) {
  int num = in + 2 * pad - k;
  int o = (ceil_mode ? (num + stride - 1) / stride : num / stride) + 1;
  if (ceil_mode && (o - 1) * stride >= in + pad) --o;
  return o;
}

}

struct tbn_backbone_plan {
  int cin0, frames, H, W;
  int cp, kw;
  int stem_rows, stem_stride, stem_pad, stem_H, stem_W;
  int stem_mode, stem_K;
  std::vector<Buf> bufs;
  std::vector<Conv> convs;
  std::vector<Pool> pools;
  std::vector<BnStep> bns;
  std::vector<Op> ops;
  std::vector<Op> ops_b;
  struct BlockRiders {
    int bn_g, bn_mid, bn_d2;
    int c3, cd2;
    unsigned g_defer, mid_defer;
  };
  std::vector<BlockRiders> riders;
  std::vector<int> bn_block;
  int block_conv[10], block_op[10], block_op_b[10];
  int rider_launches[2] = {0, 0};
  int out_buf;
  size_t weight_floats, chan_floats;
  size_t x0_off, stats_off, partial_off, coef_off, wsplit_off, wt_off, wpack_off, dwpack_off;
  size_t diag_fold_off;
  FlipTab flip;
  size_t partial_floats, wsplit_floats, wt_floats;
  size_t argmax_bytes_off, total_bytes_train, total_bytes_eval;
  size_t eval_floats;
  static const int kEvents = 128;
  hipEvent_t ev[kEvents];
  int n_ev = 0;
};

namespace {

int add_buf(tbn_backbone_plan* P, int H, int W, int C) {
  Buf b;
  b.H = H;
  b.W = W;
  b.C = C;
  b.off = b.doff = 0;
  P->bufs.push_back(b);
  return (int)P->bufs.size() - 1;
}

int add_conv(tbn_backbone_plan* P, int nparts, const std::string* names, const int* couts, int cin, int k, int stride,
             int pad, int inbuf, const int* dst_buf, const int* dst_choff, bool stem) {
  Conv c;
  c.nparts = nparts;
  c.cout = 0;
  c.c_off = P->chan_floats;
  for (int i = 0; i < nparts; ++i) {
    Part& q = c.parts[i];
    q.name = names[i];
    q.cout = couts[i];
    q.col0 = c.cout;
// ... 265 lines not shown
      }
      push(OP_CONV, cd2, 0, 0);
      push(OP_BN, bn_d2, 0, 0);
      push(OP_JOIN, 0, 0, 0);
    }
    x = O;
    h = oh;
    w = ow;
  }
  P->out_buf = x;
  P->bn_block.assign(P->bns.size(), -1);
  for (size_t b = 0; b < P->riders.size(); ++b) {
    P->bn_block[P->riders[b].bn_g] = P->bn_block[P->riders[b].bn_mid] = P->bn_block[P->riders[b].bn_d2] = (int)b;
  }

  std::vector<char> written(P->bufs.size(), 0);
  std::vector<int> last_conv(P->bufs.size(), -1);
  for (int i = (int)P->ops.size() - 1; i >= 0; --i) {
    const Op& o = P->ops[i];
    if (o.kind == OP_CONV) {
      Conv& c = P->convs[o.idx];
      if (c.need_dgrad) {
        c.dgrad_accum = written[c.inbuf] != 0;
        written[c.inbuf] = 1;
        last_conv[c.inbuf] = o.idx;
      }
    } else if (o.kind == OP_POOL) {
      Pool& p = P->pools[o.idx];
      p.bwd_accum = written[p.inbuf] != 0;
      written[p.inbuf] = 1;
      last_conv[p.inbuf] = -1;
    }
  }

  {
    std::vector<char> w2(P->bufs.size(), 0);
    std::vector<int> last2(P->bufs.size(), -1);
    bool same = true;
    for (int i = (int)P->ops_b.size() - 1; i >= 0; --i) {
      const Op& o = P->ops_b[i];
      if (o.kind == OP_CONV) {
        const Conv& c = P->convs[o.idx];
        if (c.need_dgrad) {
          same = same && (c.dgrad_accum == (w2[c.inbuf] != 0));
          w2[c.inbuf] = 1;
          last2[c.inbuf] = o.idx;
        }
      } else if (o.kind == OP_POOL) {
        const Pool& q = P->pools[o.idx];
        same = same && (q.bwd_accum == (w2[q.inbuf] != 0));
        w2[q.inbuf] = 1;
        last2[q.inbuf] = -1;
      }
    }
    if (!same || last2 != last_conv) P->ops_b.clear();
  }

  std::vector<int> readers(P->bufs.size(), 0);
  for (auto& c : P->convs) ++readers[c.inbuf];
  for (auto& q : P->pools) ++readers[q.inbuf];
  for (size_t pi = 0; pi < P->pools.size(); ++pi) {
    Pool& q = P->pools[pi];
    if (q.kind != 1 || q.bwd_accum || readers[q.inbuf] != 1 || q.inbuf == P->out_buf) continue;
    for (auto& c : P->convs)
      if (c.nparts == 1 && c.parts[0].dst_buf == q.inbuf && c.parts[0].dst_choff == 0 && c.cout == P->bufs[q.inbuf].C) {
        c.fuse_pool = (int)pi;
        q.fused = true;
      }
  }

  for (size_t ci = 0; ci < P->convs.size(); ++ci) {
    Conv& f = P->convs[ci];
    if (!f.need_dgrad || last_conv[f.inbuf] != (int)ci || f.inbuf == P->out_buf) continue;
    struct Cand { int conv, part, choff; };
    std::vector<Cand> cand;
    bool ok = true;
    for (size_t cj = 0; cj < P->convs.size(); ++cj) {
      const Conv& c = P->convs[cj];
      for (int k = 0; k < c.nparts; ++k)
        if (c.parts[k].dst_buf == f.inbuf) {
          if (c.fuse_pool >= 0) ok = false;
          cand.push_back({(int)cj, k, c.parts[k].dst_choff});
        }
    }
    if (!ok || cand.empty() || (int)cand.size() > kMaxParts) continue;
    for (size_t a = 0; a < cand.size(); ++a)
      for (size_t b = a + 1; b < cand.size(); ++b)
        if (cand[b].choff < cand[a].choff) std::swap(cand[a], cand[b]);
    for (auto& cd : cand)
      if (cd.choff % 32 != 0) ok = false;
    if (!ok) continue;
    f.nred = (int)cand.size();
    for (int k = 0; k < f.nred; ++k) {
      f.red_conv[k] = cand[k].conv;
      f.red_part[k] = cand[k].part;
      P->convs[cand[k].conv].parts[cand[k].part].red_src = (int)ci;
    }
  }
  return true;
}

#ifndef TBN_DIAG
#define TBN_DIAG 0
#endif
static inline bool diag_skip(int bit) {
#if TBN_DIAG
  static const int mask = getenv("TBN_DIAG_SKIP") ? atoi(getenv("TBN_DIAG_SKIP")) : 0;
  return (mask & bit) != 0;
#else
  (void)bit;
  return false;
#endif
}
static inline bool diag_fold() {
#if TBN_DIAG
  static const int on = getenv("TBN_DIAG_FOLD") ? atoi(getenv("TBN_DIAG_FOLD")) : 0;
  return on != 0;
#else
  return false;
#endif
}
void plan_memory(tbn_backbone_plan* P) {
  const size_t R = P->frames;
  size_t off = 0;
  auto take = [&](size_t n) {
    size_t o = off;
    off += (n + 63) / 64 * 64;
    return o;
  };
  for (size_t i = 0; i < P->bufs.size(); ++i) {
    Buf& b = P->bufs[i];
    b.off = i == 0 ? take(R * P->stem_H * P->stem_W * P->cp) : take(R * b.H * b.W * b.C);
  }
  P->x0_off = P->bufs[0].off;
  P->stats_off = take(4 * P->chan_floats);
  size_t partial = 0, wsplit = 0, wtf = 0;
  for (auto& c : P->convs) {
    const int M = (int)(R * c.outH * c.outW);
    const int K = c.stem ? P->stem_K : c.k * c.k * c.cin;
    tbn_conv_pick_tile(M, c.cout, K, &c.ft[0].mt, &c.ft[0].nt);
    c.ft[1].mt = c.ft[0].mt;
    c.ft[1].nt = c.ft[0].nt;
    size_t a = (size_t)cdiv(M, M <= kSk4MaxRows ? 32 : 128) * 2 * c.cout;
    if (a > partial) partial = a;
    for (int k = 0; k < c.nparts; ++k) {
      size_t bparts = (size_t)tbn_bn_bwd_parts(M, c.parts[k].cout) * 2 * c.parts[k].cout;
      if (bparts > partial) partial = bparts;
    }
    const int taps = c.stem ? 1 : c.k * c.k, ci = c.stem ? P->stem_rows * P->kw : c.cin;
    size_t ws = tbn_wgrad_workspace_floats(M, c.cout, ci, taps);
    if (ws > wsplit) wsplit = ws;
    if (c.need_dgrad) {
      const int Md = (int)(R * c.inH * c.inW);
      tbn_conv_pick_tile(Md, c.cin, c.k * c.k * c.cout, &c.d_mt, &c.d_nt);
    }
  }
  wtf = P->weight_floats;
  memset(&P->flip, 0, sizeof(P->flip));
  for (auto& c : P->convs)
    if (c.need_dgrad && P->flip.n < 64) {
      FlipTab& f = P->flip;
      f.w_off[f.n] = (int)c.w_off;
      f.cout[f.n] = (short)c.cout;
      f.cin[f.n] = (short)c.cin;
      f.taps[f.n] = (short)(c.k * c.k);
      f.blk0[f.n + 1] = f.blk0[f.n] + cdiv(c.cin, 32) * cdiv(c.cout, 32);
      ++f.n;
    }
  P->partial_floats = partial;
  P->wsplit_floats = wsplit;
  P->wt_floats = wtf;
  P->partial_off = take(TBN_BN_MAXL * partial);
  P->wpack_off = take((size_t)64 * P->stem_K);
  for (auto& c : P->convs)
    for (int k = 0; k < c.nparts; ++k)
      if (c.parts[k].pooled) {
        c.parts[k].yraw_off = take(R * c.outH * c.outW * c.parts[k].cout);
        c.parts[k].y2_off = take(R * c.outH * c.outW * c.parts[k].cout);
      }
  P->eval_floats = off;
  for (auto& c : P->convs) c.y_off = take(R * c.outH * c.outW * c.cout);
  for (size_t i = 1; i < P->bufs.size(); ++i) {
    if ((int)i == P->out_buf) continue;
    P->bufs[i].doff = take(R * P->bufs[i].H * P->bufs[i].W * P->bufs[i].C);
  }
  for (auto& c : P->convs)
    for (int k = 0; k < c.nparts; ++k)
      if (c.parts[k].red_src >= 0) {
        const Buf& db = P->bufs[c.parts[k].dst_buf];
        const int drows = (int)(R * db.H * db.W);
        c.parts[k].bpart_off = take(((size_t)cdiv(drows, drows <= kSk4MaxRows ? 32 : 128) + 4) * 2 * c.parts[k].cout);
      }
  P->coef_off = take(TBN_BN_MAXL * 3 * 1024);
  P->diag_fold_off = take(2 * 2048);
  P->wsplit_off = take(wsplit);
  P->wt_off = take(wtf);
  P->dwpack_off = take((size_t)64 * P->stem_rows * P->kw);
  size_t bytes = off * sizeof(float);
  P->argmax_bytes_off = bytes;
  for (auto& p : P->pools)
    if (p.kind == 1) {
      const Buf& ob = P->bufs[p.outbuf];
      const Buf& ib = P->bufs[p.inbuf];
      p.argmax_off = bytes;
      bytes += align_up(R * ob.H * ob.W * ib.C, 256);
    }
  P->total_bytes_train = bytes;
  P->total_bytes_eval = P->eval_floats * sizeof(float);
}

}

extern "C" {

int tbn_backbone_plan_create(int in_channels, int frames, int height, int width, tbn_backbone_plan** out) {
  TBN_REQUIRE(out != nullptr, "plan_create: null out");
  TBN_REQUIRE(in_channels >= 1 && in_channels <= 16 && frames >= 1 && height >= 32 && width >= 32,
              "plan_create: unsupported shape (C=%d, frames=%d, %dx%d)", in_channels, frames, height, width);
  TBN_REQUIRE((long)frames * height * width < (1l << 31) / 4, "plan_create: too many pixels per call (chunk the batch)");
  tbn_backbone_plan* P = new tbn_backbone_plan();
  P->cin0 = in_channels;
  P->frames = frames;
  P->H = height;
  P->W = width;
  if (!build_graph(P) || P->bufs[P->out_buf].H < 1 || P->bufs[P->out_buf].W < 1) {
    delete P;
    tbn_set_error("plan_create: %dx%d input is not a valid BN-Inception size (the stride-2 conv branches and the "
                  "ceil-mode pass-through max pool of inception_3c / 4e disagree; the reference's torch.cat raises)",
                  height, width);
    return TBN_ERR_UNSUPPORTED;
  }
  {
    int nd = 0;
    for (auto& c : P->convs) nd += c.need_dgrad ? 1 : 0;
    if (nd > 64) {
      delete P;
      tbn_set_error("plan_create: %d data-gradient layers exceed the flip table (64)", nd);
      return TBN_ERR_UNSUPPORTED;
    }
  }
  {
    size_t worst = (size_t)frames * P->stem_H * P->stem_W * P->cp;
    const char* what = "network input";
    for (size_t i = 1; i < P->bufs.size(); ++i) {
      const size_t n = (size_t)frames * P->bufs[i].H * P->bufs[i].W * P->bufs[i].C;
      if (n > worst) {
        worst = n;
        what = "an activation buffer";
      }
    }
    for (auto& c : P->convs) {
      const size_t n = (size_t)frames * c.outH * c.outW * c.cout;
      if (n > worst) {
        worst = n;
        what = c.parts[0].name.c_str();
      }
    }
    if (worst * sizeof(float) >= (1ull << 31)) {
      tbn_set_error("plan_create: %d frames of %dx%d make a %.2f GiB tensor (%s); one engine call addresses at most 2 GiB per "
                    "tensor -- use fewer frames per call (eval: chunk them; training: a smaller per-GPU batch)",
                    frames, height, width, (double)(worst * sizeof(float)) / (1ull << 30), what);
      delete P;
      return TBN_ERR_UNSUPPORTED;
    }
  }
  plan_memory(P);
  *out = P;
  return TBN_OK;
}

void tbn_backbone_plan_destroy(tbn_backbone_plan* p) {
  if (!p) return;
  for (int i = 0; i < p->n_ev; ++i) (void)hipEventDestroy(p->ev[i]);
  delete p;
}
// ... 267 lines not shown
    p.mode = CONV_EPI_STATS;
    p.nseg = 1;
    p.seg[0].ptr = ws + c.y_off;
    p.seg[0].ld = c.cout;
    p.seg[0].col_begin = 0;
    p.stat_partial = ws + P->partial_off + (size_t)slot * P->partial_floats;
    return;
  }
  float* scale = ws + P->stats_off + 2 * P->chan_floats;
  p.mode = CONV_EPI_EVAL;
  p.scale = scale + c.c_off;
  p.shift = scale + P->chan_floats + c.c_off;
  p.nseg = c.nparts;
  for (int i = 0; i < c.nparts; ++i) {
    const Part& q = c.parts[i];
    const Buf& db = P->bufs[q.dst_buf];
    p.seg[i].ptr = q.pooled ? ws + q.yraw_off : ws + db.off + q.dst_choff;
    p.seg[i].ld = q.pooled ? q.cout : db.C;
    p.seg[i].col_begin = q.col0;
    if (q.pooled) p.raw_seg1 = i + 1;
  }
}

enum { GEMM_FWD_EVAL = 0, GEMM_FWD_TRAIN = 1, GEMM_DGRAD = 2 };
struct Tuned {
  int halo, mt;
  bool pair;
  int p_mt;
};
Tuned tuned(const Conv& c, int gemm) {
  if (gemm == GEMM_DGRAD) return {c.d_halo, c.d_mt, c.pair_dgrad, c.pd_mt};
  const Conv::FwdTune& T = c.ft[gemm];
  return {T.halo, T.mt, T.pair, T.p_mt};
}
int pair_role(const tbn_backbone_plan* P, const Conv& c, int gemm, bool br) {
  if (br) return 0;
  if (c.pair_next >= 0 && tuned(c, gemm).pair) return 1;
  if (c.pair_prev >= 0 && tuned(P->convs[c.pair_prev], gemm).pair) return 2;
  return 0;
}
int writer_rows(const tbn_backbone_plan* P, const Conv& c, int gemm, bool br) {
  const int role = pair_role(P, c, gemm, br);
  if (role == 0) return tile_rows(tuned(c, gemm).halo, tuned(c, gemm).mt);
  return 128 * tuned(role == 1 ? c : P->convs[c.pair_prev], gemm).p_mt;
}

void fill_dgrad(const tbn_backbone_plan* P, const Conv& c, float* ws, int R, ConvP* pp) {
  ConvP& p = *pp;
  const Buf& ib = P->bufs[c.inbuf];
  memset(&p, 0, sizeof(p));
  p.in = ws + c.y_off;
  p.in_ld = c.cout;
  p.wt = ws + P->wt_off + c.w_off;
  p.N = R;
  p.H = c.outH;
  p.W = c.outW;
  p.OH = c.inH;
  p.OW = c.inW;
  p.Cin = c.cout;
  p.Cout = c.cin;
  p.R = p.S = c.k;
  p.stride = 1;
  p.pad = c.k - 1 - c.pad;
  p.up = c.stride;
  p.M = R * c.inH * c.inW;
  p.K = c.k * c.k * c.cout;
  p.alg_flops = 2.0 * R * c.outH * c.outW * (double)c.cout * c.k * c.k * c.cin;
  p.mode = CONV_EPI_PLAIN;
  p.flags = c.dgrad_accum ? CONV_FLAG_ACCUM : 0;
  p.nseg = 1;
  p.seg[0].ptr = ws + ib.doff;
  p.seg[0].ld = ib.C;
  p.seg[0].col_begin = 0;
  p.stages = c.d_stages;
  p.halo = c.d_halo;
  p.nred = c.nred;
  p.red_chan = (int)P->chan_floats;
  for (int k = 0; k < c.nred; ++k) {
    const Conv& pc = P->convs[c.red_conv[k]];
    const Part& q = pc.parts[c.red_part[k]];
    RedSeg& r = p.red[k];
    r.y = q.pooled ? ws + q.y2_off : ws + pc.y_off + q.col0;
    r.y_ld = q.pooled ? q.cout : pc.cout;
    r.partial = ws + q.bpart_off;
    r.stats = ws + P->stats_off;
    r.col_begin = q.dst_choff;
    r.C = q.cout;
    r.c_off = (int)q.c_off;
  }
  if (c.nred > 0 && p.red[0].col_begin != 0) {
    p.nred = 0;
  }
}

void fill_wgrad(const tbn_backbone_plan* P, const Conv& c, float* ws, int R, WgradP* wp) {
  const Buf& ib = P->bufs[c.inbuf];
  memset(wp, 0, sizeof(*wp));
  wp->dy = ws + c.y_off;
  wp->dy_ld = c.cout;
  wp->x = ws + ib.off;
  wp->x_ld = ib.C;
  wp->N = R;
  wp->H = c.inH;
  wp->W = c.inW;
  wp->OH = c.outH;
  wp->OW = c.outW;
  wp->Cout = c.cout;
  wp->stride = c.stride;
  wp->pad = c.pad;
  wp->M = R * c.outH * c.outW;
  wp->alg_flops = 2.0 * wp->M * (double)c.cout * c.k * c.k * c.cin;
  wp->mt = c.w_mt;
  wp->nt = c.w_nt;
  if (c.stem) {
    wp->Cin = P->stem_rows * P->kw;
    wp->R = P->stem_rows;
    wp->S = 1;
    wp->taps = 1;
    wp->cp = wp->x_ld = P->cp;
    wp->rl = P->kw;
    wp->H = P->stem_H;
    wp->W = P->stem_W;
    wp->stride = P->stem_stride;
    wp->pad = P->stem_pad;
  } else {
    wp->Cin = c.cin;
    wp->R = wp->S = c.k;
    wp->taps = c.k * c.k;
    if (diag_fold() && c.k == 3) {
      wp->fold_scale = ws + P->diag_fold_off;
      wp->fold_shift = ws + P->diag_fold_off + 2048;
    }
  }
}

int ensure_events(tbn_backbone_plan* PM) {
  constexpr int NE = tbn_backbone_plan::kEvents;
  for (int i = PM->n_ev; i < NE; ++i) {
    if (hipEventCreateWithFlags(&PM->ev[i], hipEventDisableTiming) != hipSuccess) {
      tbn_set_error("backbone: hipEventCreate failed");
      return TBN_ERR_LAUNCH;
    }
    PM->n_ev = i + 1;
  }
  return TBN_OK;
}

void order_after(hipEvent_t e, hipStream_t from, hipStream_t to) {
  (void)hipEventRecord(e, from);
  (void)hipStreamWaitEvent(to, e, 0);
}

struct AuxJoin {
  hipStream_t st, aux;
  hipEvent_t ev;
  bool forked = false;
  ~AuxJoin() {
    if (aux != nullptr && forked) order_after(ev, aux, st);
  }
};

struct SideJoin {
  hipStream_t st, side;
  hipEvent_t ev;
  bool open = false;
  void turn(hipEvent_t e, bool fork) {
    order_after(e, fork ? st : side, fork ? side : st);
    open = fork;
  }
// ... 116 lines not shown
    }
    if (o.kind == OP_CONV) {
      const Conv& c = P->convs[o.idx];
      const Conv::FwdTune& T = c.ft[tr];
      int role = pair_role(P, c, tr, br);
      if (role != 0 && (bf16x_layer(c) || bf16x_layer(P->convs[role == 1 ? c.pair_next : c.pair_prev]))) role = 0;
      if (role == 2) continue;
      const RiderP* rd = (pend_host == o.idx) ? &pend_rider : nullptr;
      if (rd != nullptr) {
        pend_host = -1;
        ++PM->rider_launches[0];
      }
      ConvP p;
      if (role == 1) {
        const Conv& c2 = P->convs[c.pair_next];
        ConvP pb;
        for (int k = 0; k < 2; ++k) {
          const Conv& m = k ? c2 : c;
          fill_fwd(P, m, training, ws, prm->weight, R, k ? &pb : &p);
          fill_fwd_epilogue(P, m, training, ws, m.slot, k ? &pb : &p);
        }
        tbn_prof_label(("fwd " + c.parts[0].name + " | " + c2.parts[0].name).c_str());
        TBN_TRY(tbn_launch_conv_pair(p, pb, T.p_variant, T.p_mt, T.p_nt, st, rd));
        continue;
      }
      fill_fwd(P, c, training, ws, prm->weight, R, &p);
      fill_fwd_epilogue(P, c, training, ws, br ? c.slot_b : c.slot, &p);
      tbn_prof_label(("fwd " + c.parts[c.nparts - 1].name).c_str());
      const bool bx = bf16x_layer(c);
      if (bx || bf16x_pw_layer(c)) {
        p.flags |= bf16x_flag;
        p.halo = 0;
        if (bf16x_all) {
          p.flags |= CONV_FLAG_BF16X_PLANES;
          p.wt = reinterpret_cast<const float*>(static_cast<const char*>(prm->weight_planes) + planes_off[o.idx]);
        }
        const bool own_tile = bx && T.halo == 1;
        TBN_TRY(tbn_launch_conv(p, 0, own_tile ? T.mt : 0, own_tile ? T.nt : 0, st, nullptr));
        continue;
      }
      TBN_TRY(tbn_launch_conv(p, c.stem, T.mt, T.nt, st, rd));
    } else if (o.kind == OP_PREPOOL) {
      const Conv& c = P->convs[o.idx];
      const Part& q = c.parts[o.part];
      const int M = R * c.outH * c.outW;
      const float* src = training ? ws + c.y_off + q.col0 : ws + q.yraw_off;
      const int src_ld = training ? c.cout : q.cout;
      if (!diag_skip(4)) TBN_TRY(tbn_launch_avgpool3_fwd(src, src_ld, ws + q.y2_off, q.cout, R, c.outH, c.outW, q.cout, 0, st));
      if (training) {
        int nparts = 0;
        TBN_TRY(tbn_launch_bn_stats(ws + q.y2_off, q.cout, M, q.cout,
                                    ws + P->partial_off + (size_t)(br ? q.slot_b : q.slot) * P->partial_floats, &nparts, st));
      }
    } else if (o.kind == OP_BN) {
      const BnStep& s = P->bns[o.idx];
      if (!training) {
        for (int k = 0; k < s.n; ++k) {
          const Conv& c = P->convs[s.conv[k]];
          const Part& q = c.parts[s.part[k]];
          if (!q.pooled) continue;
          const Buf& db = P->bufs[q.dst_buf];
          Seg z;
          z.ptr = ws + db.off + q.dst_choff;
          z.ld = db.C;
          z.col_begin = 0;
          if (!diag_skip(2))
            TBN_TRY(tbn_launch_bn_apply(ws + q.y2_off, R * c.outH * c.outW, q.cout, scale + q.c_off, shift + q.c_off, &z, 1, st));
        }
        continue;
      }
      const Conv& c0 = P->convs[s.conv[0]];
      if (s.n == 1 && c0.fuse_pool >= 0) {
        const Part& q = c0.parts[0];
        const int M = R * c0.outH * c0.outW;
        const Pool& pl = P->pools[c0.fuse_pool];
        const Buf& ob = P->bufs[pl.outbuf];
        if (!diag_skip(2)) {
          TBN_TRY(tbn_launch_bn_finalize(ws + P->partial_off + (size_t)c0.slot * P->partial_floats, cdiv(M, writer_rows(P, c0, GEMM_FWD_TRAIN, br)), M,
                                         q.cout, prm->gamma + q.c_off, prm->beta + q.c_off, prm->bias + q.c_off,
                                         prm->running_mean + q.c_off, prm->running_var + q.c_off, prm->momentum, prm->eps,
                                         mean + q.c_off, rstd + q.c_off, scale + q.c_off, shift + q.c_off, st));
          TBN_TRY(tbn_launch_bn_apply_maxpool(ws + c0.y_off, (int)R, c0.outH, c0.outW, q.cout, scale + q.c_off,
                                              shift + q.c_off, ws + ob.off + pl.out_choff, ob.C,
                                              (uint8_t*)workspace + pl.argmax_off, ob.H, ob.W, pl.stride, pl.pad, st));
        }
        continue;
      }
      BnFwdBatch fb;
      memset(&fb, 0, sizeof(fb));
      fb.n = s.n;
      fb.momentum = prm->momentum;
      fb.eps = prm->eps;
      for (int k = 0; k < s.n; ++k) {
        const Conv& c = P->convs[s.conv[k]];
        const Part& q = c.parts[s.part[k]];
        const Buf& db = P->bufs[q.dst_buf];
        const int M = R * c.outH * c.outW;
        BnFwdLayer& L = fb.l[k];
        L.P = M;
        L.C = q.cout;
        if (q.pooled) {
          L.y = ws + q.y2_off;
          L.y_ld = q.cout;
          L.partial = ws + P->partial_off + (size_t)(br ? q.slot_b : q.slot) * P->partial_floats;
          L.pld = q.cout;
          L.nparts = tbn_bn_stats_parts(M, q.cout);
        } else {
          L.y = ws + c.y_off + q.col0;
          L.y_ld = c.cout;
          L.partial = ws + P->partial_off + (size_t)(br ? c.slot_b : c.slot) * P->partial_floats + q.col0;
          L.pld = c.cout;
          L.nparts = cdiv(M, writer_rows(P, c, GEMM_FWD_TRAIN, br));
        }
        L.gamma = prm->gamma + q.c_off;
        L.beta = prm->beta + q.c_off;
        L.conv_bias = prm->bias + q.c_off;
        L.running_mean = prm->running_mean + q.c_off;
        L.running_var = prm->running_var + q.c_off;
        L.save_mean = mean + q.c_off;
        L.save_rstd = rstd + q.c_off;
        L.scale = scale + q.c_off;
        L.shift = shift + q.c_off;
        L.nseg = 1;
        L.seg[0].ptr = ws + db.off + q.dst_choff;
        L.seg[0].ld = db.C;
        L.seg[0].col_begin = 0;
      }
      unsigned defer = 0;
      if (use_riders && P->bn_block[o.idx] >= 0) {
        const tbn_backbone_plan::BlockRiders& R = P->riders[P->bn_block[o.idx]];
        if (o.idx == R.bn_g && R.g_defer) {
          defer = R.g_defer;
          pend_host = R.c3;
        } else if (o.idx == R.bn_mid && R.mid_defer) {
          defer = R.mid_defer;
          pend_host = R.cd2;
        }
      }
      if (!diag_skip(2)) TBN_TRY(tbn_launch_bn_fwd_multi_defer(fb, defer, defer ? &pend_rider : nullptr, st));
    } else {
      const Pool& q = P->pools[o.idx];
      const Buf& ib = P->bufs[q.inbuf];
      const Buf& ob = P->bufs[q.outbuf];
      if (training && q.fused) continue;
      if (q.kind == 0) {
        if (!diag_skip(4)) TBN_TRY(tbn_launch_avgpool3_fwd(ws + ib.off, ib.C, ws + ob.off + q.out_choff, ob.C, R, ib.H, ib.W, ib.C, 0, st));
      } else {
        uint8_t* am = training ? (uint8_t*)workspace + q.argmax_off : nullptr;
        if (!diag_skip(4)) TBN_TRY(tbn_launch_maxpool_fwd(ws + ib.off, ib.C, ws + ob.off + q.out_choff, ob.C, am, R, ib.H, ib.W, ib.C,
                                       ob.H, ob.W, q.stride, q.pad, st));
      }
    }
  }
  st = st_main;
  TBN_REQUIRE(pend_host < 0, "backbone_forward: a rider was left without its host launch (conv %d)", pend_host);
  *features_out = ws + P->bufs[P->out_buf].off;
  return TBN_OK;
}

}

namespace {

constexpr int kMaxCand = 40;
struct Cand {
  int mt, nt, stages, halo;
  int variant;
// ... 191 lines not shown
      const int w = rank_candidates(cand, ms, ncand);
      const Cand win = w >= 0 ? cand[w] : Cand{1, 1, 1, 0, 1};
      const float singles = pass == 0 ? c.ft[tr].t + c2.ft[tr].t : c.t_dgrad + c2.t_dgrad;
      const bool take = w >= 0 && ms[w] < 0.97f * singles;
      if (pass == 0) {
        c.ft[tr].pair = take;
        c.ft[tr].p_variant = win.variant;
        c.ft[tr].p_mt = win.mt;
        c.ft[tr].p_nt = win.nt;
      } else {
        c.pair_dgrad = take;
        c.pd_variant = win.variant;
        c.pd_mt = win.mt;
        c.pd_nt = win.nt;
      }
    }
  }
  return TBN_OK;
}

int tbn_backbone_flip_weights(const tbn_backbone_plan* P, const tbn_backbone_params* prm, void* workspace, size_t workspace_bytes,
                              void* stream) {
  TBN_REQUIRE(P && prm && workspace && prm->weight, "backbone_flip_weights: null argument");
  TBN_REQUIRE(workspace_bytes >= P->total_bytes_train, "backbone_flip_weights: workspace too small (training workspace expected)");
  return tbn_launch_weight_flip_transpose_all(prm->weight, (float*)workspace + P->wt_off, P->flip, (hipStream_t)stream);
}

int tbn_backbone_backward(const tbn_backbone_plan* P, const float* dfeatures, const tbn_backbone_params* prm,
                          const tbn_backbone_grads* g, void* workspace, size_t workspace_bytes, void* stream) {
  TBN_REQUIRE(P && dfeatures && prm && g && workspace, "backbone_backward: null argument");
  TBN_REQUIRE(g->dweight && g->dbias, "backbone_backward: dweight/dbias required");
  TBN_REQUIRE(workspace_bytes >= P->total_bytes_train, "backbone_backward: workspace too small");
  hipStream_t st = (hipStream_t)stream;
  hipStream_t aux = (hipStream_t)g->aux_stream;
  tbn_backbone_plan* PM = const_cast<tbn_backbone_plan*>(P);
  if (aux == st) aux = nullptr;
  constexpr int NE = tbn_backbone_plan::kEvents;
  hipStream_t side = (hipStream_t)prm->side_stream;
  if (side == st || side == aux || P->ops_b.empty()) side = nullptr;
  hipStreamCaptureStatus cap = hipStreamCaptureStatusNone;
  if (hipStreamIsCapturing(st, &cap) != hipSuccess) {
    (void)hipGetLastError();
    tbn_set_error("backbone_backward: hipStreamIsCapturing failed on the launch stream (invalid stream handle?)");
    return TBN_ERR_LAUNCH;
  }
  const bool capturing = cap != hipStreamCaptureStatusNone;
  if (capturing) side = nullptr;
  const bool br = side != nullptr;
  if ((aux != nullptr || br) && !capturing) TBN_TRY(ensure_events(PM));
  TBN_REQUIRE((aux == nullptr && !br) || capturing || (PM->n_ev == NE && (int)P->convs.size() + 2 * kNumBlocks + 3 + kGradBuckets < NE),
              "backbone_backward: event pool too small");
  if (aux != nullptr) {
    if (capturing) {
      tbn_set_error("backbone_backward: aux_stream inside a stream capture is not supported (nested capture forks overflow "
                    "the stack of hipStreamEndCapture in ROCm 7.x): capture with aux_stream = NULL");
      return TBN_ERR_UNSUPPORTED;
    }
  }
  AuxJoin join{st, aux, aux != nullptr ? PM->ev[NE - 1] : nullptr};
  SideJoin sjoin{st, side, br ? PM->ev[NE - 2] : nullptr};
  int ev_next = 0;
  float* ws = (float*)workspace;
  const int R = P->frames;
  float* mean = ws + P->stats_off;
  float* rstd = mean + P->chan_floats;
  float* scale = rstd + P->chan_floats;
  float* shift = scale + P->chan_floats;
  float* partial = ws + P->partial_off;
  float* coef = ws + P->coef_off;
  auto dptr = [&](int buf) -> const float* {
    return buf == P->out_buf ? dfeatures : ws + P->bufs[buf].doff;
  };

  if ((prm->flags & TBN_BACKBONE_WEIGHTS_FLIPPED) == 0)
    TBN_TRY(tbn_launch_weight_flip_transpose_all(prm->weight, ws + P->wt_off, P->flip, st));
  const std::vector<Op>& prog = br ? P->ops_b : P->ops;
  const hipStream_t st_main = st;
  const bool use_riders = !br && (prm->flags & TBN_BACKBONE_RIDERS) != 0 && !tbn_prof_enabled() && !P->riders.empty();
  RiderP bpend;
  int bpend_host = -1;
  PM->rider_launches[1] = 0;
  int deferred[8], ndef = 0;
  const bool stem_last = !br && aux == nullptr && (prm->flags & TBN_BACKBONE_STEM_WGRAD_LAST) != 0;
  auto issue_wgrad = [&](const Conv& c, hipStream_t wst) -> int {
    tbn_prof_label(("wgrad " + c.parts[c.nparts - 1].name).c_str());
    WgradP wp;
    fill_wgrad(P, c, ws, R, &wp);
    if (c.stem) {
      float* dwp = ws + P->dwpack_off;
      TBN_TRY(tbn_launch_wgrad(wp, 1, dwp, ws + P->wsplit_off, wst));
      if (P->stem_mode == 1) return tbn_launch_unpack_stem_wgrad_rows(dwp, g->dweight + c.w_off, 64, P->cin0, P->kw, wst);
      return tbn_launch_unpack_stem_wgrad_s2d(dwp, g->dweight + c.w_off, 64, P->cin0, wst);
    }
    return tbn_launch_wgrad(wp, 0, g->dweight + c.w_off, ws + P->wsplit_off, wst);
  };
  const int* blk_op = br ? P->block_op_b : P->block_op;
  size_t bucket_hi = P->weight_floats;
  auto fire_bucket = [&](int blk) -> int {
    const size_t lo = P->convs[P->block_conv[blk]].w_off;
    TBN_REQUIRE(ndef == 0, "backbone_backward: a weight gradient of block %d is still deferred at its bucket boundary", blk);
    if (aux != nullptr && join.forked) {
      order_after(PM->ev[ev_next++], aux, st_main);
    }
    g->bucket_cb(g->bucket_user, lo, bucket_hi - lo);
    bucket_hi = lo;
    return TBN_OK;
  };
  for (int oi = (int)prog.size() - 1; oi >= 0; --oi) {
    if (g->bucket_cb != nullptr && !capturing)
      for (int k = 0; k < kGradBuckets; ++k)
        if (oi + 1 == blk_op[kBucketBlock[k]]) TBN_TRY(fire_bucket(kBucketBlock[k]));
    const Op& o = prog[oi];
    st = (br && o.side) ? side : st_main;
    if (o.kind == OP_FORK || o.kind == OP_JOIN) {
      const bool fork = o.kind == OP_JOIN;
      sjoin.turn(PM->ev[ev_next++], fork);
      if (!fork) {
        for (int k = 0; k < ndef; ++k) TBN_TRY(issue_wgrad(P->convs[deferred[k]], st_main));
        ndef = 0;
      }
      continue;
    }
    if (o.kind == OP_POOL) {
      const Pool& q = P->pools[o.idx];
      const Buf& ib = P->bufs[q.inbuf];
      const Buf& ob = P->bufs[q.outbuf];
      if (q.inbuf == 0) continue;
      if (q.fused) continue;
      float* din = ws + ib.doff;
      if (q.kind == 0) {
        if (!diag_skip(4)) TBN_TRY(tbn_launch_avgpool3_fwd(dptr(q.outbuf) + q.out_choff, ob.C, din, ib.C, R, ib.H, ib.W, ib.C, q.bwd_accum,
                                        st));
      } else {
        if (!diag_skip(4)) TBN_TRY(tbn_launch_maxpool_bwd(dptr(q.outbuf) + q.out_choff, ob.C, (const uint8_t*)workspace + q.argmax_off,
                                       din, ib.C, R, ib.H, ib.W, ib.C, ob.H, ob.W, q.stride, q.pad, q.bwd_accum, st));
      }
      continue;
    }
    if (o.kind == OP_PREPOOL) {
      const Conv& c = P->convs[o.idx];
      const Part& q = c.parts[o.part];
      if (!diag_skip(4))
        TBN_TRY(tbn_launch_avgpool3_fwd(ws + q.y2_off, q.cout, ws + c.y_off + q.col0, c.cout, R, c.outH, c.outW, q.cout, 0, st));
      continue;
    }
    if (o.kind == OP_BN) {
      const BnStep& s = P->bns[o.idx];
      const Conv& c0 = P->convs[s.conv[0]];
      if (s.n == 1 && c0.fuse_pool >= 0) {
        const Part& q = c0.parts[0];
        const int M = R * c0.outH * c0.outW;
        const Pool& pl = P->pools[c0.fuse_pool];
        const Buf& ob = P->bufs[pl.outbuf];
        const float* dpool = dptr(pl.outbuf) + pl.out_choff;
        const uint8_t* am = (const uint8_t*)workspace + pl.argmax_off;
        float* y = ws + c0.y_off;
        const bool bn_grad = g->dgamma && g->dbeta && (g->bn_grad_layers == 2 || (g->bn_grad_layers == 1 && s.conv[0] == 0));
        if (!diag_skip(8)) {
          TBN_TRY(tbn_launch_bn_bwd_reduce_pooled(dpool, ob.C, am, R, c0.outH, c0.outW, ob.H, ob.W, pl.stride, pl.pad, y,
                                                  q.cout, scale + q.c_off, shift + q.c_off, mean + q.c_off,
                                                  rstd + q.c_off, partial, st));
          TBN_TRY(tbn_launch_bn_bwd_finalize(partial, tbn_bn_bwd_pooled_parts(R, c0.outH, c0.outW, q.cout, pl.stride, pl.pad), M,
                                             q.cout, scale + q.c_off,
                                             mean + q.c_off, rstd + q.c_off, coef, bn_grad ? g->dgamma + q.c_off : nullptr,
                                             bn_grad ? g->dbeta + q.c_off : nullptr, g->dbias + q.c_off, st));
          TBN_TRY(tbn_launch_bn_bwd_apply_pooled(dpool, ob.C, am, R, c0.outH, c0.outW, ob.H, ob.W, pl.stride, pl.pad, y,
                                                 q.cout, scale + q.c_off, shift + q.c_off, coef, y, st));
        }
        continue;
      }
      auto fill_layer = [&](BnBwdLayer& L, int ci, int pk, int slot) {
        const Conv& c = P->convs[ci];
        const Part& q = c.parts[pk];
        const Buf& db = P->bufs[q.dst_buf];
        L.nseg = 1;
        L.dz[0].ptr = dptr(q.dst_buf) + q.dst_choff;
        L.dz[0].ld = db.C;
        L.dz[0].col_begin = 0;
        L.y = L.dy = q.pooled ? ws + q.y2_off : ws + c.y_off + q.col0;
        L.y_ld = q.pooled ? q.cout : c.cout;
        L.P = R * c.outH * c.outW;
        L.C = q.cout;
        L.scale = scale + q.c_off;
        L.shift = shift + q.c_off;
        L.mean = mean + q.c_off;
        L.rstd = rstd + q.c_off;
        if (q.red_src >= 0) {
          const Conv& f = P->convs[q.red_src];
          L.partial = ws + q.bpart_off;
          L.ext_parts = tbn_conv_red_rows(R, f.inH, f.inW, f.stride, writer_rows(P, f, GEMM_DGRAD, br));
        } else {
          L.partial = partial + (size_t)slot * P->partial_floats;
          L.ext_parts = 0;
        }
        L.coef = coef + (size_t)slot * 3 * 1024;
        const bool first = (ci == 0);
        const bool bg = g->dgamma && g->dbeta && (g->bn_grad_layers == 2 || (g->bn_grad_layers == 1 && first));
        L.dgamma = bg ? g->dgamma + q.c_off : nullptr;
        L.dbeta = bg ? g->dbeta + q.c_off : nullptr;
        L.dbias = g->dbias + q.c_off;
      };
      BnBwdBatch bb;
      memset(&bb, 0, sizeof(bb));
      unsigned skip = 0, defer = 0;
      const tbn_backbone_plan::BlockRiders* RB = (use_riders && P->bn_block[o.idx] >= 0) ? &P->riders[P->bn_block[o.idx]] : nullptr;
      if (RB != nullptr && o.idx == RB->bn_g) skip = RB->g_defer;
      if (RB != nullptr && o.idx == RB->bn_mid) skip = RB->mid_defer;
      for (int k = 0; k < s.n; ++k)
        if (!(skip & (1u << k))) {
          fill_layer(bb.l[bb.n], s.conv[k], s.part[k], s.slot0 + bb.n);
          ++bb.n;
        }
      if (RB != nullptr && o.idx == RB->bn_d2 && (RB->g_defer | RB->mid_defer)) {
        for (int pass = 0; pass < 2; ++pass) {
          const BnStep& t = P->bns[pass == 0 ? RB->bn_g : RB->bn_mid];
          const unsigned m = pass == 0 ? RB->g_defer : RB->mid_defer;
          for (int k = 0; k < t.n; ++k)
            if (m & (1u << k)) {
              TBN_REQUIRE(bb.n < TBN_BN_MAXL, "backbone_backward: too many rider members");
              defer |= 1u << bb.n;
              fill_layer(bb.l[bb.n], t.conv[k], t.part[k], bb.n);
              ++bb.n;
            }
        }
        bpend_host = RB->cd2;
      }
      if (bb.n == 0) continue;
      if (!diag_skip(8)) TBN_TRY(tbn_launch_bn_bwd_multi_defer(bb, defer, defer ? &bpend : nullptr, st));
      continue;
    }
    const Conv& c = P->convs[o.idx];
    if (aux != nullptr) {
      order_after(PM->ev[ev_next++], st, aux);
      join.forked = true;
      TBN_TRY(issue_wgrad(c, aux));
    } else if (br && o.side) {
      TBN_REQUIRE(ndef < 8, "backbone_backward: too many deferred weight gradients");
      deferred[ndef++] = o.idx;
    } else if (stem_last && (o.idx == 1 || o.idx == 2)) {
      deferred[ndef++] = o.idx;
    } else {
      TBN_TRY(issue_wgrad(c, st));
    }
    if (c.need_dgrad) {
      const int role = pair_role(P, c, GEMM_DGRAD, br);
      if (role == 2) continue;
      if (role == 1) {
        const Conv& c2 = P->convs[c.pair_next];
        ConvP pa, pb;
        fill_dgrad(P, c, ws, R, &pa);
        fill_dgrad(P, c2, ws, R, &pb);
        tbn_prof_label(("dgrad " + c.parts[0].name + " | " + c2.parts[0].name).c_str());
        TBN_TRY(tbn_launch_conv_pair(pa, pb, c.pd_variant, c.pd_mt, c.pd_nt, st));
        continue;
      }
      tbn_prof_label(("dgrad " + c.parts[c.nparts - 1].name).c_str());
      ConvP p;
      fill_dgrad(P, c, ws, R, &p);
      const RiderP* rd = (bpend_host == o.idx) ? &bpend : nullptr;
      if (rd != nullptr) {
        bpend_host = -1;
        ++PM->rider_launches[1];
      }
      TBN_TRY(tbn_launch_conv(p, 0, c.d_mt, c.d_nt, st, rd));
    }
  }
  if (stem_last) {
    for (int k = 0; k < ndef; ++k) TBN_TRY(issue_wgrad(P->convs[deferred[k]], st_main));
    ndef = 0;
  }
  TBN_REQUIRE(bpend_host < 0, "backbone_backward: a rider was left without its host launch (conv %d)", bpend_host);
  return TBN_OK;
}

}
```

### attention_based_tbn_amd/csrc/tbn_kernels.h

```cpp
#pragma once
#include "tbn_common.h"
#include <hip/hip_ext.h>
#include <type_traits>

enum { CONV_EPI_PLAIN = 0, CONV_EPI_STATS = 1, CONV_EPI_EVAL = 2 };
enum {
  CONV_FLAG_ACCUM = 1,
  CONV_FLAG_RELU = 2,
  CONV_FLAG_HALO = 4,
  CONV_FLAG_DMA = 8,
  CONV_FLAG_SK4 = 16,
  CONV_FLAG_BF16X6 = 32,
  CONV_FLAG_BF16X3 = 64,
  CONV_FLAG_BF16X_PLANES = 128,
  CONV_FLAG_DESC_OUT2 = 256
};

#define TBN_CONV_MAXSEG 4
struct RedSeg {
  const float* y;
  float* partial;
  const float* stats;
  int y_ld, col_begin, C, c_off;
  unsigned y_bytes;
// ... 143 lines not shown
  } while (0)

void tbn_conv_pick_tile(int M, int Cout, int K, int* mt, int* nt);
int tbn_launch_conv(ConvP p, int rowmode, int mt, int nt, hipStream_t st, const RiderP* rider = nullptr);
int tbn_launch_conv_pair(ConvP a, ConvP b, int variant, int mt, int nt, hipStream_t st, const RiderP* rider = nullptr);
int tbn_conv_red_rows(int N, int OH, int OW, int up, int tile_rows);
size_t tbn_conv_halo_lds_bytes(const ConvP& p, int mt, int nt);
template <int MAXM, int MAXN, int I = 0, class F>
static int with_tile(int mt, int nt, F&& f) {
  if constexpr (I == MAXM * MAXN) {
    tbn_set_error("conv: unsupported tile %dx%d", mt, nt);
    return TBN_ERR_UNSUPPORTED;
  } else {
    constexpr int MT = I / MAXN + 1, NT = I % MAXN + 1;
    if (mt == MT && nt == NT) return f(std::integral_constant<int, MT>{}, std::integral_constant<int, NT>{});
    return with_tile<MAXM, MAXN, I + 1>(mt, nt, f);
  }
}

static inline void conv_set_tiles(ConvP& p, int tile_rows, int mt, int nt) {
  p.tiles_m = cdiv(p.M, tile_rows * mt);
  p.tiles_n = cdiv(p.Cout, 32 * nt);
}
enum { TBN_DYN_LDS_DEFAULT = 64 * 1024, TBN_DYN_LDS_MAX = 160 * 1024 };
static inline int tbn_raise_dyn_lds(const void* kernel, size_t need, size_t& allowed, const char* who) {
  if (need <= allowed) return TBN_OK;
  if (hipFuncSetAttribute(kernel, hipFuncAttributeMaxDynamicSharedMemorySize, TBN_DYN_LDS_MAX) != hipSuccess) {
    tbn_set_error("%s: cannot raise the dynamic LDS limit", who);
    return TBN_ERR_LAUNCH;
  }
  allowed = TBN_DYN_LDS_MAX;
  return TBN_OK;
}

enum Bf16xLayer { BF16X_LAYER_NONE = 0, BF16X_LAYER_3X3, BF16X_LAYER_PW };
static inline bool bf16x_gemm_ok(int stride, int cin) { return stride == 1 && cin % 32 == 0; }
static inline Bf16xLayer bf16x_layer_kind(int k, int stride, int pad, int cin) {
  if (!bf16x_gemm_ok(stride, cin)) return BF16X_LAYER_NONE;
  if (k == 3 && pad == 1) return BF16X_LAYER_3X3;
  if (k == 1 && pad == 0) return BF16X_LAYER_PW;
  return BF16X_LAYER_NONE;
}
static inline bool bf16x_3x3_map_ok(int W) { return W <= 64; }
int tbn_launch_conv_bf16x(ConvP& p, int rowmode, int mt, int nt, double alg_bytes, hipStream_t st, const RiderP* rider);
struct SplitTab {
  int n;
  size_t w_off[64];
  size_t p_off[64];
  size_t floats[64];
  int blk0[65];
};
static inline bool split_tab_push(SplitTab& tab, size_t w_off, size_t p_off, size_t floats) {
  if (tab.n >= 64) return false;
  if (tab.n == 0) tab.blk0[0] = 0;
  tab.w_off[tab.n] = w_off;
  tab.p_off[tab.n] = p_off;
  tab.floats[tab.n] = floats;
  tab.blk0[tab.n + 1] = tab.blk0[tab.n] + (int)((floats + 1023) / 1024);
  ++tab.n;
  return true;
}
size_t tbn_bf16x_planes_bytes(size_t floats, int np);
int tbn_launch_bf16x_split(const float* w, void* planes, const SplitTab& tab, int np, hipStream_t st);
void tbn_wgrad_plan(int M, int Cout, int Cin, int taps, int* mt, int* nt, int* splits, int* rows_per_split);
size_t tbn_wgrad_workspace_floats(int M, int Cout, int Cin, int taps);
int tbn_launch_wgrad(WgradP p, int rowmode, float* dw, float* workspace, hipStream_t st);
int tbn_launch_weight_flip_transpose(const float* w, float* wt, int Cout, int taps, int Cin, hipStream_t st);
struct FlipTab {
  int n;
  int w_off[64];
  short cout[64], cin[64], taps[64];
  int blk0[65];
};
int tbn_launch_weight_flip_transpose_all(const float* w, float* wt, const FlipTab& tab, hipStream_t st);

int tbn_launch_bn_stats(const float* y, int ld, int P, int C, float* partial, int* nparts, hipStream_t st);
int tbn_bn_stats_parts(int P, int C);
int tbn_launch_bn_finalize(const float* partial, int nparts, int P, int C, const float* gamma, const float* beta,
                           const float* conv_bias, float* running_mean, float* running_var, float momentum, float eps,
                           float* save_mean, float* save_rstd, float* scale, float* shift, hipStream_t st);
int tbn_launch_bn_apply(const float* y, int P, int C, const float* scale, const float* shift, const Seg* segs,
                        int nseg, hipStream_t st);
int tbn_launch_bn_apply_maxpool(const float* y, int N, int H, int W, int C, const float* scale, const float* shift,
                                float* out, int out_ld, unsigned char* argmax, int OH, int OW, int stride, int pad,
                                hipStream_t st);
int tbn_launch_bn_bwd_reduce_pooled(const float* dpooled, int dpooled_ld, const unsigned char* argmax, int N, int H,
                                    int W, int OH, int OW, int stride, int pad, const float* y, int C,
                                    const float* scale, const float* shift, const float* mean, const float* rstd,
                                    float* partial, hipStream_t st);
int tbn_bn_bwd_pooled_parts(int N, int H, int W, int C, int stride, int pad);
int tbn_launch_bn_bwd_apply_pooled(const float* dpooled, int dpooled_ld, const unsigned char* argmax, int N, int H, int W,
                                   int OH, int OW, int stride, int pad, const float* y, int C, const float* scale,
                                   const float* shift, const float* coef, float* dy, hipStream_t st);
#define TBN_BN_MAXL 4
struct BnFwdLayer {
  const float* y;
  int y_ld;
  int P, C;
  const float* partial;
  int pld, nparts;
  const float *gamma, *beta, *conv_bias;
  float *running_mean, *running_var, *save_mean, *save_rstd, *scale, *shift;
  Seg seg[3];
  int nseg;
  int app_rows;
};
struct BnFwdBatch {
  int n;
  float momentum, eps;
  BnFwdLayer l[TBN_BN_MAXL];
  int fin_blk0[TBN_BN_MAXL + 1], app_blk0[TBN_BN_MAXL + 1];
};
struct BnBwdLayer {
  CSeg dz[3];
  int nseg;
  const float* y;
  float* dy;
  int y_ld;
  int P, C;
  const float *scale, *shift, *mean, *rstd;
  float* partial;
  int ext_parts;
  float* coef;
  float *dgamma, *dbeta, *dbias;
  int pch, nparts;
  int app_rows;
};
struct BnBwdBatch {
  int n;
  BnBwdLayer l[TBN_BN_MAXL];
  int red_blk0[TBN_BN_MAXL + 1], fin_blk0[TBN_BN_MAXL + 1], app_blk0[TBN_BN_MAXL + 1];
};
int tbn_launch_bn_fwd_multi(BnFwdBatch& b, hipStream_t st);
int tbn_launch_bn_bwd_multi(BnBwdBatch& b, hipStream_t st);
int tbn_launch_bn_fwd_multi_defer(BnFwdBatch& b, unsigned defer_mask, RiderP* rider, hipStream_t st);
int tbn_launch_bn_bwd_multi_defer(BnBwdBatch& b, unsigned defer_mask, RiderP* rider, hipStream_t st);
bool tbn_prof_enabled();
int tbn_launch_bn_fold(const float* gamma, const float* beta, const float* mean, const float* var, const float* bias,
                       float eps, float* scale, float* shift, int C, hipStream_t st);
int tbn_bn_bwd_parts(int P, int C);
int tbn_launch_bn_bwd_reduce(const CSeg* dz, int nseg, const float* y, int P, int C, const float* scale,
                             const float* shift, const float* mean, const float* rstd, float* partial, hipStream_t st);
int tbn_launch_bn_bwd_finalize(const float* partial, int nparts, int P, int C, const float* scale, const float* mean,
                               const float* rstd, float* coef, float* dgamma, float* dbeta, float* dbias,
                               hipStream_t st);
int tbn_launch_bn_bwd_apply(const CSeg* dz, int nseg, const float* y, int P, int C, const float* scale,
                            const float* shift, const float* coef, float* dy, hipStream_t st);

int tbn_launch_maxpool_fwd(const float* in, int in_ld, float* out, int out_ld, uint8_t* argmax, int N, int H, int W,
                           int C, int OH, int OW, int stride, int pad, hipStream_t st);
int tbn_launch_maxpool_bwd(const float* dout, int dout_ld, const uint8_t* argmax, float* din, int din_ld, int N,
                           int H, int W, int C, int OH, int OW, int stride, int pad, int accumulate, hipStream_t st);
int tbn_launch_avgpool3_fwd(const float* in, int in_ld, float* out, int out_ld, int N, int H, int W, int C,
                            int accumulate, hipStream_t st);
int tbn_launch_spatial_mean_fwd(const float* in, int in_ld, float* out, int out_ld, int N, int H, int W, int C,
                                int freq_only, hipStream_t st);
int tbn_launch_spatial_mean_bwd(const float* dout, int dout_ld, float* din, int din_ld, int N, int H, int W, int C,
                                int freq_only, hipStream_t st);
int tbn_launch_nchw_to_s2d_pad(const float* in, float* out, int N, int C, int H, int W, hipStream_t st);
int tbn_launch_pack_stem_weight_s2d(const float* w, float* wp, int Cout, int C, hipStream_t st);
int tbn_launch_unpack_stem_wgrad_s2d(const float* dwp, float* dw, int Cout, int C, hipStream_t st);
int tbn_launch_nchw_to_nhwc_pad(const float* in, float* out, int N, int C, int H, int W, int HP, int WP, hipStream_t st);
int tbn_launch_pack_stem_weight_rows(const float* w, float* wp, int Cout, int C, int RL, int K, hipStream_t st);
int tbn_launch_unpack_stem_wgrad_rows(const float* dwp, float* dw, int Cout, int C, int RL, hipStream_t st);
```

### attention_based_tbn_amd/ops_conv.py

```python
import ctypes as C

import torch

from ._lib import BnBwdDesc, BnFwdDesc, BnSeg, call, lib, ptr, stream_ptr, TbnHipError

MOMENTUM = 0.1
EPS = 1e-5


class BnState:
    __slots__ = ("stride", "pad", "running_mean", "running_var", "wcache", "fcache")

    def __init__(self, stride, pad, running_mean, running_var):
        self.stride, self.pad = stride, pad
        self.running_mean, self.running_var = running_mean, running_var
        self.wcache, self.fcache = {}, {}


def _need_cuda(t, what):
    if not t.is_cuda:
        raise TbnHipError(f"{what}: tensor is on {t.device}; the TBN hot path only runs on an MI355X "
                          "(HIP) device -- there is no CPU fallback")


# ... 269 lines not shown
            if pneed(i, 0):
                grads[3 * i] = _conv_wgrad(dy, inp, wk, states[i])
            grads[3 * i + 1] = dg if pneed(i, 1) else None
            grads[3 * i + 2] = db if pneed(i, 2) else None
            if i > 0:
                if need[0] or any(pneed(u, j) for u in range(i) for j in range(3)):
                    dz = _conv_dgrad(dy, wk, inp.shape, states[i])
            elif need[0]:
                dx = _conv_dgrad(dy, wk, x.shape, states[0], dx=dx)
        return (dx, None, None, None) + tuple(grads)


def residual_block(x, main, downsample=None, training=True):
    units = list(main) + ([downsample] if downsample is not None else [])
    params = [t for u in units for t in u[:3]]
    return _ResidualBlockFn.apply(x, [u[3] for u in units], len(main), bool(training), *params)


class _GlobalMeanFn(torch.autograd.Function):

    @staticmethod
    def forward(ctx, x):
        _need_cuda(x, "global_mean")
        x = _f32c(x)
        n, h, w, c = x.shape
        out = torch.empty(n, c, device=x.device, dtype=torch.float32)
        for c0 in range(0, c, 1024):
            call("tbn_spatial_mean_fwd", x.data_ptr() + 4 * c0, c, out.data_ptr() + 4 * c0, c, n, h, w, min(1024, c - c0),
                 0, stream_ptr())
        ctx.shape = tuple(x.shape)
        return out

    @staticmethod
    def backward(ctx, dout):
        n, h, w, c = ctx.shape
        dout = _f32c(dout)
        dx = torch.empty(ctx.shape, device=dout.device, dtype=torch.float32)
        call("tbn_spatial_mean_bwd", ptr(dout), c, ptr(dx), c, n, h, w, c, 0, stream_ptr())
        return dx


def global_mean(x_nhwc):
    return _GlobalMeanFn.apply(x_nhwc)


_NO_INPUT_GRAD = ("{}: the gradient with respect to the input frames is not implemented (the first conv's data gradient "
                  "is never formed); detach the input")


class _StemFn(torch.autograd.Function):
    @staticmethod
    def forward(ctx, x, weight, gamma, beta, state, training, who):
        _need_cuda(x, who)
        x = _f32c(x)
        n, cin, h, w = x.shape
        cout = weight.shape[0]
        if tuple(weight.shape[1:]) != (cin, 7, 7) or not 1 <= cin <= 16 or cout % 32:
            raise TbnHipError(f"{who}: the stem is a 7x7 / stride 2 / pad 3 conv of 1..16 input channels, got weight "
                              f"{tuple(weight.shape)} for input {tuple(x.shape)}")
        wk = kernel_weight(weight, state.wcache)
        st = stream_ptr()
        oh, ow = _out_size(h, w, 7, 2, 3)
        ph, pw = _out_size(oh, ow, 3, 2, 1)
        ws = torch.empty(lib().tbn_stem_workspace_floats(cin, h, w, 0, n, cout), device=x.device, dtype=torch.float32)
        y = torch.empty(n, oh, ow, cout, device=x.device, dtype=torch.float32)
        pooled = torch.empty(n, ph, pw, cout, device=x.device, dtype=torch.float32)
        argmax = torch.empty(n, ph, pw, cout, device=x.device, dtype=torch.uint8)
        ctx.eval_mode = not training
        ctx.live = training and any(ctx.needs_input_grad[1:4])
        ctx.who = who
        if not training:
            ss = folded_bn(gamma, beta, state)
            call("tbn_stem_conv_fwd", ptr(x), ptr(wk), 0, ptr(y), cout, n, h, w, cin, cout, 0, 2, ss[0].data_ptr(),
                 ss[1].data_ptr(), 0, 0, 0, 0, ptr(ws), st)
            call("tbn_maxpool3_fwd", ptr(y), cout, ptr(pooled), cout, ptr(argmax), n, oh, ow, cout, ph, pw, 2, 1, st)
            return pooled
        m = n * oh * ow
        partial = torch.zeros((m + 127) // 128 * 2 * cout, device=x.device, dtype=torch.float32)
        call("tbn_stem_conv_fwd", ptr(x), ptr(wk), 0, ptr(y), cout, n, h, w, cin, cout, 0, 1, 0, 0, ptr(partial), 0, 0, 0,
             ptr(ws), st)
        stats = torch.empty(4, cout, device=x.device, dtype=torch.float32)
        bnws = torch.empty(lib().tbn_bn_workspace_floats(m, cout), device=x.device, dtype=torch.float32)
        rm, rv = state.running_mean, state.running_var
        call("tbn_bn_relu_maxpool_train_fwd", ptr(y), n, oh, ow, cout, ptr(gamma), ptr(beta), ptr(rm), ptr(rv), MOMENTUM,
             EPS, stats[0].data_ptr(), stats[1].data_ptr(), stats[2].data_ptr(), stats[3].data_ptr(), ptr(pooled), cout,
             ptr(argmax), ph, pw, 2, 1, ptr(bnws), st)
        if rm is not None:
            torch.autograd.graph.increment_version((rm, rv))
        if ctx.live:
            ctx.save_for_backward(x, y, argmax, stats)
        return pooled

    @staticmethod
    def backward(ctx, dpooled):
        need = ctx.needs_input_grad
        if need[0]:
            raise TbnHipError(_NO_INPUT_GRAD.format(ctx.who))
        if not ctx.live:
            if ctx.eval_mode and any(need[1:4]):
                raise TbnHipError(_EVAL_BACKWARD.format(ctx.who))
            return (None,) * 7
        x, y, argmax, stats = ctx.saved_tensors
        n, cin, h, w = x.shape
        _, oh, ow, cout = y.shape
        ph, pw = argmax.shape[1], argmax.shape[2]
        st = stream_ptr()
        dpooled = _f32c(dpooled)
        m = n * oh * ow
        dy = torch.empty_like(y)
        dgb = torch.empty(2, cout, device=x.device, dtype=torch.float32)
        bnws = torch.empty(lib().tbn_bn_workspace_floats(m, cout), device=x.device, dtype=torch.float32)
        call("tbn_bn_relu_maxpool_train_bwd", ptr(dpooled), cout, ptr(argmax), ptr(y), n, oh, ow, cout, ph, pw, 2, 1,
             stats[0].data_ptr(), stats[1].data_ptr(), stats[2].data_ptr(), stats[3].data_ptr(), ptr(dy),
             dgb[0].data_ptr(), dgb[1].data_ptr(), ptr(bnws), st)
        dw = None
        if need[1]:
            ws = torch.empty(lib().tbn_stem_workspace_floats(cin, h, w, 0, n, cout), device=x.device, dtype=torch.float32)
            dwk = torch.empty(cout, 7, 7, cin, device=x.device, dtype=torch.float32)
            call("tbn_stem_conv_wgrad", ptr(dy), cout, ptr(x), ptr(dwk), n, h, w, cin, cout, 0, 0, 0, ptr(ws), st)
            dw = _oihw(dwk)
        return None, dw, dgb[0] if need[2] else None, dgb[1] if need[3] else None, None, None, None


def stem_bn_pool(x_nchw, weight, gamma, beta, state, training=True, who="stem_bn_pool"):
    return _StemFn.apply(x_nchw, weight, gamma, beta, state, bool(training), who)
```

### include/tbn_hip.h

```cpp
#ifndef TBN_HIP_H
#define TBN_HIP_H
#include <stddef.h>
#include <stdint.h>
#ifdef __cplusplus
extern "C" {
#endif

#define TBN_ERR_ARG (-1)
#define TBN_ERR_LAUNCH (-2)
#define TBN_ERR_UNSUPPORTED (-3)

int tbn_version(void);
#define TBN_CAP_CONV_BF16X 1
#define TBN_CAP_CONV_BF16X_PLANES 2
#define TBN_CAP_FRAMES_CROPS 4
#define TBN_CAP_ATTN_GENERAL 8
#define TBN_CAP_ATTN_REG 16
#define TBN_CAP_AUDIO_LAYER 32
#define TBN_CAP_STEM_OPS 64
#define TBN_CAP_BN_BATCH_OPS 128
int tbn_capabilities(void);
const char* tbn_last_error(void);

int tbn_profile_enable(int on);
int tbn_profile_reset(void);
int tbn_profile_num_entries(void);
int tbn_profile_entry(int i, char* name, int name_len, long* launches, double* total_ms, double* total_flops);
int tbn_profile_entry_bytes(int i, double* total_alg_bytes);
int tbn_diag_mfma_burst(float* sink, int workgroups, int iters, double* flops, void* stream);

typedef struct tbn_backbone_plan tbn_backbone_plan;

typedef struct {
  char name[64];
  int cin, cout, ksize, stride, pad;
  size_t weight_offset;
  size_t channel_offset;
} tbn_conv_info;

typedef struct {
  const float* weight;
  const float* bias;
  const float* gamma;
  const float* beta;
  float* running_mean;
  float* running_var;
  float momentum;
  float eps;
  void* side_stream;
  int flags;
  const void* weight_planes;
} tbn_backbone_params;
#define TBN_BACKBONE_RIDERS 1
#define TBN_BACKBONE_STEM_WGRAD_LAST 2
#define TBN_BACKBONE_WEIGHTS_FLIPPED 4
#define TBN_BACKBONE_CONV_BF16X6 8
#define TBN_BACKBONE_CONV_BF16X3 16
#define TBN_BACKBONE_CONV_BF16X_ALL 32

typedef struct {
  float* dweight;
  float* dbias;
  float* dgamma;
  float* dbeta;
  int bn_grad_layers;
  void* aux_stream;
  void (*bucket_cb)(void* user, size_t first_float, size_t num_floats);
  void* bucket_user;
} tbn_backbone_grads;

int tbn_backbone_plan_create(int in_channels, int frames, int height, int width, tbn_backbone_plan** plan);
void tbn_backbone_plan_destroy(tbn_backbone_plan* plan);
int tbn_backbone_num_convs(const tbn_backbone_plan* plan);
int tbn_backbone_conv_info(const tbn_backbone_plan* plan, int idx, tbn_conv_info* info);
size_t tbn_backbone_weight_floats(const tbn_backbone_plan* plan);
size_t tbn_backbone_channel_floats(const tbn_backbone_plan* plan);
size_t tbn_backbone_workspace_bytes(const tbn_backbone_plan* plan, int training);
int tbn_backbone_out_shape(const tbn_backbone_plan* plan, int* h, int* w, int* c);
int tbn_backbone_num_streams(const tbn_backbone_plan* plan);
int tbn_timeline_enable(int on);
int tbn_timeline_dump(const char* path);
int tbn_backbone_rider_launches(const tbn_backbone_plan* plan, int* forward, int* backward);
int tbn_backbone_tensor_info(const tbn_backbone_plan* plan, const char* conv_name, int kind, long* offset, int* rows,
                             int* cols, int* ld);
int tbn_backbone_launch_info(const tbn_backbone_plan* plan, const char* conv_name, int training, int* out16);
size_t tbn_backbone_plan_export_bytes(const tbn_backbone_plan* plan);
int tbn_backbone_plan_export(const tbn_backbone_plan* plan, void* buf, size_t bytes);
int tbn_backbone_plan_import(tbn_backbone_plan* plan, const void* buf, size_t bytes);
unsigned long long tbn_backbone_plan_fingerprint(const tbn_backbone_plan* plan);
int tbn_backbone_forward(const tbn_backbone_plan* plan, int training, const float* x_nchw,
                         const tbn_backbone_params* params, void* workspace, size_t workspace_bytes,
                         float** features_out, void* stream);
size_t tbn_backbone_weight_planes_bytes(const tbn_backbone_plan* plan, int np);
int tbn_backbone_split_weights(const tbn_backbone_plan* plan, const float* weight, int np, void* planes, void* stream);
int tbn_backbone_autotune(tbn_backbone_plan* plan, int training, const tbn_backbone_params* params, void* workspace,
                          size_t workspace_bytes, void* stream);
int tbn_backbone_backward(const tbn_backbone_plan* plan, const float* dfeatures,
                          const tbn_backbone_params* params, const tbn_backbone_grads* grads, void* workspace,
                          size_t workspace_bytes, void* stream);
int tbn_backbone_flip_weights(const tbn_backbone_plan* plan, const tbn_backbone_params* params, void* workspace,
                              size_t workspace_bytes, void* stream);


int tbn_conv2d_fwd(const float* in, int in_ld, const float* weight, const float* bias, float* out, int out_ld,
                   int n, int h, int w, int cin, int cout, int ksize, int stride, int pad, int epilogue, int flags,
                   const float* scale, const float* shift, float* stat_partial, void* stream);
int tbn_conv2d_stat_tiles(int n, int h, int w, int cin, int cout, int ksize, int stride, int pad);
size_t tbn_conv_weight_planes_bytes(int cout, int ksize, int cin, int np);
int tbn_conv_split_weights(const float* weight, int cout, int ksize, int cin, int np, void* planes, void* stream);
int tbn_conv2d_fwd_tile(const float* in, int in_ld, const float* weight, const float* bias, float* out, int out_ld,
                        int n, int h, int w, int cin, int cout, int ksize, int stride, int pad, int epilogue, int flags,
                        float* stat_partial, int mt, int nt, void* stream);
int tbn_conv2d_dgrad(const float* dout, int dout_ld, const float* weight, float* din, int din_ld, int n, int h, int w,
                     int cin, int cout, int ksize, int stride, int pad, int accumulate, float* workspace,
                     void* stream);
typedef struct {
  const float* y;
  int y_ld;
  int col_begin;
  int channels;
  int stat_offset;
  float* partial;
} tbn_conv_red;
typedef struct {
  const float* in;
  int in_ld;
  const float* weight;
  const float* bias;
  float* out;
  int out_ld;
  int n, h, w, cin, cout, ksize, stride, pad;
  int dgrad;
  int epilogue;
  int flags;
  int stages;
  const float* scale;
  const float* shift;
  float* stat_partial;
  int nred;
  tbn_conv_red red[4];
  const float* red_stats;
  int red_stats_stride;
  float* out2;
  int out2_ld;
  int out2_col_begin;
  int out2_raw;
} tbn_conv_desc;
int tbn_conv_partial_rows(const tbn_conv_desc* d, int mt, int pair);
int tbn_conv_launch(const tbn_conv_desc* d, int mt, int nt, float* workspace, void* stream);
int tbn_conv_launch_pair(const tbn_conv_desc* a, const tbn_conv_desc* b, int variant, int mt, int nt,
                         float* workspace_a, float* workspace_b, void* stream);

size_t tbn_conv2d_wgrad_workspace_floats(int n, int h, int w, int cin, int cout, int ksize, int stride, int pad);
int tbn_conv2d_wgrad(const float* dout, int dout_ld, const float* in, int in_ld, float* dweight, int n, int h, int w,
                     int cin, int cout, int ksize, int stride, int pad, float* workspace, void* stream);

int tbn_stem_geometry(int cin, int h, int w, int layout, int* out8);
size_t tbn_stem_workspace_floats(int cin, int h, int w, int layout, int n, int cout);
int tbn_stem_conv_fwd(const float* x_nchw, const float* weight, const float* bias, float* out, int out_ld, int n, int h, int w,
                      int cin, int cout, int layout, int epilogue, const float* scale, const float* shift, float* stat_partial,
                      int mt, int nt, int stages, float* workspace, void* stream);
int tbn_stem_conv_wgrad(const float* dy, int dy_ld, const float* x_nchw, float* dweight, int n, int h, int w, int cin, int cout,
                        int layout, int mt, int nt, float* workspace, void* stream);

int tbn_linear_fwd(const float* x, int x_ld, const float* w, const float* bias, float* out, int out_ld, int m, int k,
                   int n, int relu, void* stream);
int tbn_linear_dgrad(const float* dy, int dy_ld, const float* w, float* dx, int dx_ld, int m, int k, int n,
                     int accumulate, float* workspace, void* stream);
size_t tbn_linear_wgrad_workspace_floats(int m, int k, int n);
int tbn_linear_wgrad(const float* dy, int dy_ld, const float* x, int x_ld, float* dw, float* dbias, int m, int k,
                     int n, float* workspace, void* stream);

size_t tbn_bn_workspace_floats(int p, int c);
int tbn_bn_relu_train_fwd(const float* y, int p, int c, const float* gamma, const float* beta, float* running_mean,
                          float* running_var, float momentum, float eps, float* save_mean, float* save_rstd,
                          float* scale, float* shift, float* z, int z_ld, float* workspace, void* stream);
int tbn_bn_relu_train_bwd(const float* dz, int dz_ld, const float* y, int p, int c, const float* save_mean,
                          const float* save_rstd, const float* scale, const float* shift, float* dy, float* dgamma,
                          float* dbeta, float* workspace, void* stream);

int tbn_bn_relu_maxpool_train_fwd(const float* y, int n, int h, int w, int c, const float* gamma, const float* beta,
                                  float* running_mean, float* running_var, float momentum, float eps, float* save_mean,
                                  float* save_rstd, float* scale, float* shift, float* pooled, int pooled_ld,
                                  uint8_t* argmax, int oh, int ow, int stride, int pad, float* workspace, void* stream);
int tbn_bn_relu_maxpool_train_bwd(const float* dpooled, int dpooled_ld, const uint8_t* argmax, const float* y, int n, int h,
                                  int w, int c, int oh, int ow, int stride, int pad, const float* save_mean,
                                  const float* save_rstd, const float* scale, const float* shift, float* dy,
                                  float* dgamma, float* dbeta, float* workspace, void* stream);

typedef struct {
  float* ptr;
  int ld;
  int col_begin;
} tbn_bn_seg;
typedef struct {
  const float* y;
  int y_ld;
  int p, c;
  const float* partial;
  int pld, nparts;
  const float* gamma;
  const float* beta;
  const float* conv_bias;
  float* running_mean;
  float* running_var;
  float* save_mean;
  float* save_rstd;
  float* scale;
  float* shift;
  tbn_bn_seg seg[3];
  int nseg;
} tbn_bn_fwd_desc;
typedef struct {
  tbn_bn_seg dz[3];
  int nseg;
  const float* y;
  float* dy;
  int y_ld;
  int p, c;
  const float* scale;
  const float* shift;
  const float* mean;
  const float* rstd;
  float* partial;
  int ext_parts;
  float* coef;
  float* dgamma;
  float* dbeta;
  float* dbias;
} tbn_bn_bwd_desc;
int tbn_bn_stats_partials(const float* y, int y_ld, int p, int c, float* partial, int* nparts, void* stream);
int tbn_bn_fwd_batch(const tbn_bn_fwd_desc* members, int n, float momentum, float eps, void* stream);
size_t tbn_bn_bwd_partial_floats(int p, int c);
int tbn_bn_bwd_batch(const tbn_bn_bwd_desc* members, int n, void* stream);

int tbn_bn_res_apply(const float* y, int y_ld, int p, int c, const float* scale, const float* shift, const float* res,
                     int res_ld, int relu, float* z, int z_ld, void* stream);
int tbn_bn_res_fwd(const float* y, int y_ld, int p, int c, const float* partial, int pld, int nparts, const float* gamma,
                   const float* beta, float* running_mean, float* running_var, float momentum, float eps,
                   float* save_mean, float* save_rstd, float* scale, float* shift, const float* res, int res_ld,
                   int relu, float* z, int z_ld, void* stream);
size_t tbn_bn_res_bwd_workspace_floats(int p, int c);
int tbn_bn_res_bwd(const float* dz, int dz_ld, const float* z, int z_ld, const float* y, int y_ld, int p, int c,
                   const float* save_mean, const float* save_rstd, const float* scale, int relu, float* dy, int dy_ld,
                   float* dres, int dres_ld, int accumulate, float* dgamma, float* dbeta, float* workspace,
                   void* stream);

int tbn_maxpool3_fwd(const float* in, int in_ld, float* out, int out_ld, uint8_t* argmax, int n, int h, int w, int c,
                     int oh, int ow, int stride, int pad, void* stream);
int tbn_maxpool3_bwd(const float* dout, int dout_ld, const uint8_t* argmax, float* din, int din_ld, int n, int h,
                     int w, int c, int oh, int ow, int stride, int pad, int accumulate, void* stream);
int tbn_avgpool3_fwd(const float* in, int in_ld, float* out, int out_ld, int n, int h, int w, int c, int accumulate,
                     void* stream);
int tbn_spatial_mean_fwd(const float* in, int in_ld, float* out, int out_ld, int n, int h, int w, int c,
                         int freq_only, void* stream);
int tbn_spatial_mean_bwd(const float* dout, int dout_ld, float* din, int din_ld, int n, int h, int w, int c,
                         int freq_only, void* stream);

int tbn_pe_concat_fwd(const float* feat, int feat_ld, const float* pe, float* out, int out_ld, int r, int t, int c,
                      int pe_dim, void* stream);
int tbn_groupnorm_fwd(const float* x, float* y, const float* gamma, const float* beta, float* save_mean,
                      float* save_rstd, int r, int t, int c, int groups, float eps, void* stream);
int tbn_groupnorm_bwd(const float* dy, const float* x, const float* gamma, const float* save_mean,
                      const float* save_rstd, float* dx, float* dgamma_part, float* dbeta_part, int r, int t, int c,
                      int groups, void* stream);
int tbn_colsum(const float* x, int x_ld, float* out, int rows, int cols, void* stream);
int tbn_mha_q1_fwd(const float* q, const float* kv, const float* drop_mask, float* ctx, float* probs, float* avg_w,
                   int r, int t, int e, int heads, float scale, void* stream);
int tbn_mha_q1_bwd(const float* dctx, const float* davg_w, const float* q, const float* kv, const float* probs,
                   const float* drop_mask, float* dq, float* dkv, int r, int t, int e, int heads, float scale,
                   void* stream);
// ... 133 lines not shown
```

Before: 911.8 clips/s.

## Save pre-BN values at maxpool winners to reduce BN backward over pooled grid

The fused BN+ReLU+maxpool forward now also writes the pre-BN activation at each pooling argmax location (ypool). In backward, the BN gradient reduction reads only the pooled-size grid (ypool plus dpooled) rather than scattering through argmax over the full-resolution tensor. In the backbone engine, that reduction can also ride along as a rider on the upstream dgrad conv, so no separate pass is needed. This trades an extra pooled-size buffer write in forward and more workspace for a smaller backward read. The timeline-naming tweak in api.hip is incidental.

```diff
diff --git a/attention_based_tbn_amd/_lib.py b/attention_based_tbn_amd/_lib.py
--- a/attention_based_tbn_amd/_lib.py
+++ b/attention_based_tbn_amd/_lib.py
@@ -150,7 +150,11 @@
                                             c_fp, c_fp, c_i, c_fp, c_i, c_i, c_i, c_i, c_fp, c_fp]),
     "tbn_bn_relu_maxpool_train_bwd": (c_i, [c_fp, c_i, c_fp, c_fp, c_i, c_i, c_i, c_i, c_i, c_i, c_i, c_i, c_fp, c_fp,
                                             c_fp, c_fp, c_fp, c_fp, c_fp, c_fp, c_fp]),
-    "tbn_bn_res_apply": (c_i, [c_fp, c_i, c_i, c_i, c_fp, c_fp, c_fp, c_i, c_i, c_fp, c_i, c_fp]),
+    "tbn_bn_relu_maxpool_ypool_train_fwd": (c_i, [c_fp, c_i, c_i, c_i, c_i, c_fp, c_fp, c_fp, c_fp, c_f, c_f, c_fp, c_fp,
+                                                  c_fp, c_fp, c_fp, c_i, c_fp, c_fp, c_i, c_i, c_i, c_i, c_i, c_fp, c_fp]),
+    "tbn_bn_relu_maxpool_ypool_train_bwd": (c_i, [c_fp, c_i, c_fp, c_fp, c_i, c_fp, c_i, c_i, c_i, c_i, c_i, c_i, c_i, c_i,
+                                                  c_fp, c_fp, c_fp, c_fp, c_fp, c_fp, c_fp, c_fp, c_fp]),
+    "tbn_bn_res_apply":(c_i, [c_fp, c_i, c_i, c_i, c_fp, c_fp, c_fp, c_i, c_i, c_fp, c_i, c_fp]),
     "tbn_bn_res_fwd": (c_i, [c_fp, c_i, c_i, c_i, c_fp, c_i, c_i, c_fp, c_fp, c_fp, c_fp, c_f, c_f, c_fp, c_fp, c_fp,
                              c_fp, c_fp, c_i, c_i, c_fp, c_i, c_fp]),
     "tbn_bn_res_bwd_workspace_floats": (c_sz, [c_i, c_i]),
diff --git a/attention_based_tbn_amd/core/models/bn_inception.py b/attention_based_tbn_amd/core/models/bn_inception.py
--- a/attention_based_tbn_amd/core/models/bn_inception.py
+++ b/attention_based_tbn_amd/core/models/bn_inception.py
@@ -262,6 +262,7 @@
         self._side_streams = {}
         self.use_riders = True
         self.stem_wgrad_last = False
+        self.pool_reduce_own = False
         self._conv_math = "f32"
         self._conv_math_layers = "3x3"
         self._planes = None
@@ -447,7 +448,7 @@
         return self._planes
 
     def _engine_flags(self):
-        return ((1 if self.use_riders else 0) | (2 if self.stem_wgrad_last else 0)
+        return ((1 if self.use_riders else 0) | (2 if self.stem_wgrad_last else 0) | (64 if self.pool_reduce_own else 0)
                 | (0 if self.training else self.CONV_MATH[self._conv_math]) | (32 if self._planes_on() else 0))
 
     def _side_stream_ptr(self):
diff --git a/attention_based_tbn_amd/csrc/api.hip b/attention_based_tbn_amd/csrc/api.hip
--- a/attention_based_tbn_amd/csrc/api.hip
+++ b/attention_based_tbn_amd/csrc/api.hip
@@ -113,7 +113,9 @@
 }
 }
 
+static thread_local char g_tl_name[96] = "";
 void tbn_prof_begin(const char* kernel, double flops, hipStream_t st, double bytes) {
+  strncpy(g_tl_name, kernel, sizeof(g_tl_name) - 1);
   if (!g_prof_on) return;
   std::lock_guard<std::mutex> lk(g_prof_mu);
   std::string key = g_prof_prefix ? std::string(g_prof_prefix) + kernel : std::string(kernel);
@@ -168,7 +170,7 @@
 void tbn_tl_events(const char* name, hipStream_t st, hipEvent_t* start, hipEvent_t* stop) {
   std::lock_guard<std::mutex> lk(g_tl_mu);
   TlRec r;
-  r.name = name;
+  r.name = g_tl_name[0] ? g_tl_name : name;
   r.stream = (void*)st;
   r.a = r.b = nullptr;
   (void)hipEventCreate(&r.a);
@@ -228,6 +230,7 @@
   g_prof_label = label;
 }
 void tbn_prof_end(hipStream_t st) {
+  g_tl_name[0] = 0;
   if (!g_prof_on) return;
   std::lock_guard<std::mutex> lk(g_prof_mu);
   (void)st;
@@ -746,7 +749,7 @@
   s.col_begin = 0;
   const int parts = tbn_bn_bwd_parts(p, c);
   float* coef = workspace + (size_t)parts * 2 * c;
-  TBN_TRY(tbn_launch_bn_bwd_reduce(&s, 1, y, p, c, scale, shift, save_mean, save_rstd, workspace, st));
+  TBN_TRY(tbn_launch_bn_bwd_reduce(&s, 1, y, c, p, c, scale, shift, save_mean, save_rstd, workspace, st));
   TBN_TRY(tbn_launch_bn_bwd_finalize(workspace, parts, p, c, scale, save_mean, save_rstd, coef, dgamma, dbeta, nullptr,
                                      st));
   return tbn_launch_bn_bwd_apply(&s, 1, y, p, c, scale, shift, coef, dy, st);
@@ -823,7 +826,45 @@
   TBN_TRY(tbn_launch_bn_stats(y, c, p, c, workspace, &parts, st));
   TBN_TRY(tbn_launch_bn_finalize(workspace, parts, p, c, gamma, beta, nullptr, running_mean, running_var, momentum, eps,
                                  save_mean, save_rstd, scale, shift, st));
-  return tbn_launch_bn_apply_maxpool(y, n, h, w, c, scale, shift, pooled, pooled_ld, argmax, oh, ow, stride, pad, st);
+  return tbn_launch_bn_apply_maxpool(y, n, h, w, c, scale, shift, pooled, pooled_ld, argmax, nullptr, 0, oh, ow, stride, pad, st);
+}
+
+int tbn_bn_relu_maxpool_ypool_train_fwd(const float* y, int n, int h, int w, int c, const float* gamma, const float* beta,
+                                        float* running_mean, float* running_var, float momentum, float eps, float* save_mean,
+                                        float* save_rstd, float* scale, float* shift, float* pooled, int pooled_ld,
+                                        uint8_t* argmax, float* ypool, int ypool_ld, int oh, int ow, int stride, int pad,
+                                        float* workspace, void* stream) {
+  hipStream_t st = (hipStream_t)stream;
+  TBN_REQUIRE(y && pooled && argmax && ypool && workspace, "bn_relu_maxpool_ypool_train_fwd: null pointer");
+  const int p = n * h * w;
+  int parts = 0;
+  TBN_TRY(tbn_launch_bn_stats(y, c, p, c, workspace, &parts, st));
+  TBN_TRY(tbn_launch_bn_finalize(workspace, parts, p, c, gamma, beta, nullptr, running_mean, running_var, momentum, eps,
+                                 save_mean, save_rstd, scale, shift, st));
+  return tbn_launch_bn_apply_maxpool(y, n, h, w, c, scale, shift, pooled, pooled_ld, argmax, ypool, ypool_ld, oh, ow, stride,
+                                     pad, st);
+}
+
+int tbn_bn_relu_maxpool_ypool_train_bwd(const float* dpooled, int dpooled_ld, const uint8_t* argmax, const float* ypool,
+                                        int ypool_ld, const float* y, int n, int h, int w, int c, int oh, int ow, int stride,
+                                        int pad, const float* save_mean, const float* save_rstd, const float* scale,
+                                        const float* shift, float* dy, float* dgamma, float* dbeta, float* workspace,
+                                        void* stream) {
+  hipStream_t st = (hipStream_t)stream;
+  TBN_REQUIRE(dpooled && argmax && ypool && y && dy && workspace, "bn_relu_maxpool_ypool_train_bwd: null pointer");
+  TBN_REQUIRE(n >= 1 && oh >= 1 && ow >= 1 && (long)n * oh * ow < (1l << 31), "bn_relu_maxpool_ypool_train_bwd: bad pooled extent");
+  const int p = n * h * w, pq = n * oh * ow;
+  const int parts = tbn_bn_bwd_parts(pq, c);
+  TBN_REQUIRE(parts <= tbn_bn_bwd_parts(p, c), "bn_relu_maxpool_ypool_train_bwd: workspace sized by tbn_bn_workspace_floats is too small");
+  float* coef = workspace + (size_t)tbn_bn_bwd_parts(p, c) * 2 * c;
+  CSeg s;
+  s.ptr = dpooled;
+  s.ld = dpooled_ld;
+  s.col_begin = 0;
+  TBN_TRY(tbn_launch_bn_bwd_reduce(&s, 1, ypool, ypool_ld, pq, c, scale, shift, save_mean, save_rstd, workspace, st));
+  TBN_TRY(tbn_launch_bn_bwd_finalize(workspace, parts, p, c, scale, save_mean, save_rstd, coef, dgamma, dbeta, nullptr, st));
+  return tbn_launch_bn_bwd_apply_pooled(dpooled, dpooled_ld, argmax, n, h, w, oh, ow, stride, pad, y, c, scale, shift, coef,
+                                        dy, st);
 }
 
 int tbn_bn_relu_maxpool_train_bwd(const float* dpooled, int dpooled_ld, const uint8_t* argmax, const float* y, int n, int h,
diff --git a/attention_based_tbn_amd/csrc/bn.hip b/attention_based_tbn_amd/csrc/bn.hip
--- a/attention_based_tbn_amd/csrc/bn.hip
+++ b/attention_based_tbn_amd/csrc/bn.hip
@@ -163,11 +163,13 @@
   return TBN_OK;
 }
 
+template <bool YPOOL>
 __global__ __launch_bounds__(256) void bn_apply_maxpool_kernel(const float* __restrict__ y, int N, int H, int W, int C,
                                                                const float* __restrict__ scale,
                                                                const float* __restrict__ shift,
                                                                float* __restrict__ out, int out_ld,
-                                                               unsigned char* __restrict__ argmax, int OH, int OW,
+                                                               unsigned char* __restrict__ argmax,
+                                                               float* __restrict__ ypool, int ypool_ld, int OH, int OW,
                                                                int stride, int pad, PixDecode dec) {
   const int G = C >> 2;
   const uint32_t total = (uint32_t)N * OH * OW * G;
@@ -183,6 +185,7 @@
     const float4 sh = *reinterpret_cast<const float4*>(shift + g * 4);
     float4 best = make_float4(-INFINITY, -INFINITY, -INFINITY, -INFINITY);
     int bx = 0, by = 0, bz = 0, bw = 0;
+    float4 yb = make_float4(0.f, 0.f, 0.f, 0.f);
 #pragma unroll
     for (int r = 0; r < 3; ++r)
 #pragma unroll
@@ -196,12 +199,13 @@
           z.z = fmaxf(fmaf(v.z, sc.z, sh.z), 0.f);
           z.w = fmaxf(fmaf(v.w, sc.w, sh.w), 0.f);
           const int k = r * 3 + s2;
-          if (z.x > best.x || z.x != z.x) { best.x = z.x; bx = k; }
-          if (z.y > best.y || z.y != z.y) { best.y = z.y; by = k; }
-          if (z.z > best.z || z.z != z.z) { best.z = z.z; bz = k; }
-          if (z.w > best.w || z.w != z.w) { best.w = z.w; bw = k; }
+          if (z.x > best.x || z.x != z.x) { best.x = z.x; bx = k; if (YPOOL) yb.x = v.x; }
+          if (z.y > best.y || z.y != z.y) { best.y = z.y; by = k; if (YPOOL) yb.y = v.y; }
+          if (z.z > best.z || z.z != z.z) { best.z = z.z; bz = k; if (YPOOL) yb.z = v.z; }
+          if (z.w > best.w || z.w != z.w) { best.w = z.w; bw = k; if (YPOOL) yb.w = v.w; }
         }
       }
+    if (YPOOL) *reinterpret_cast<float4*>(ypool + (size_t)opix * ypool_ld + g * 4) = yb;
     *reinterpret_cast<float4*>(out + (size_t)opix * out_ld + g * 4) = best;
     *reinterpret_cast<uint32_t*>(argmax + (size_t)opix * C + g * 4) =
         (uint32_t)bx | ((uint32_t)by << 8) | ((uint32_t)bz << 16) | ((uint32_t)bw << 24);
@@ -209,14 +213,20 @@
 }
 
 int tbn_launch_bn_apply_maxpool(const float* y, int N, int H, int W, int C, const float* scale, const float* shift,
-                                float* out, int out_ld, unsigned char* argmax, int OH, int OW, int stride, int pad,
-                                hipStream_t st) {
+                                float* out, int out_ld, unsigned char* argmax, float* ypool, int ypool_ld, int OH, int OW,
+                                int stride, int pad, hipStream_t st) {
   TBN_REQUIRE(C % 4 == 0 && out_ld % 4 == 0 && argmax != nullptr, "bn_apply_maxpool: bad C / pitch / argmax");
+  TBN_REQUIRE(ypool == nullptr || (ypool_ld % 4 == 0 && ypool_ld >= C), "bn_apply_maxpool: bad ypool pitch");
   size_t g = ((size_t)N * OH * OW * (C / 4) + 255) / 256;
   if (g > 8192) g = 8192;
   TBN_REQUIRE((size_t)N * H * W * (C / 4) < (1ull << 31), "bn_apply_maxpool: too many elements per call");
-  TBN_KLAUNCH(bn_apply_maxpool_kernel, dim3((unsigned)(g < 1 ? 1 : g)), dim3(256), 0, st, y, N, H, W, C, scale,
-                     shift, out, out_ld, argmax, OH, OW, stride, pad, make_pixdecode(C / 4, OW, OH));
+  if (ypool != nullptr) {
+    TBN_KLAUNCH(bn_apply_maxpool_kernel<true>, dim3((unsigned)(g < 1 ? 1 : g)), dim3(256), 0, st, y, N, H, W, C, scale,
+                       shift, out, out_ld, argmax, ypool, ypool_ld, OH, OW, stride, pad, make_pixdecode(C / 4, OW, OH));
+  } else {
+    TBN_KLAUNCH(bn_apply_maxpool_kernel<false>, dim3((unsigned)(g < 1 ? 1 : g)), dim3(256), 0, st, y, N, H, W, C, scale,
+                       shift, out, out_ld, argmax, ypool, ypool_ld, OH, OW, stride, pad, make_pixdecode(C / 4, OW, OH));
+  }
   TBN_CHECK_LAUNCH("bn_apply_maxpool");
   return TBN_OK;
 }
@@ -286,7 +296,7 @@
 }
 
 template <bool POOLED>
-__global__ __launch_bounds__(256) void bn_bwd_reduce_kernel(CSeg3 dz, PoolGrad pg, const float* __restrict__ y, int P,
+__global__ __launch_bounds__(256) void bn_bwd_reduce_kernel(CSeg3 dz, PoolGrad pg, const float* __restrict__ y, int yld, int P,
                                                             int C, int pch, const float* __restrict__ scale,
                                                             const float* __restrict__ shift,
                                                             const float* __restrict__ mean,
@@ -308,7 +318,7 @@
     const float4 mu = *reinterpret_cast<const float4*>(mean + c);
     const float4 rs4 = *reinterpret_cast<const float4*>(rstd + c);
     for (int p = p0 + rs; p < p1; p += RP) {
-      const float4 v = *reinterpret_cast<const float4*>(y + (size_t)p * C + c);
+      const float4 v = *reinterpret_cast<const float4*>(y + (size_t)p * yld + c);
       const float4 d = POOLED ? pooled_grad(pg, p, c) : *reinterpret_cast<const float4*>(dzp + (size_t)p * dld);
       const float gx = fmaf(v.x, sc.x, sh.x) > 0.f ? d.x : 0.f;
       const float gy = fmaf(v.y, sc.y, sh.y) > 0.f ? d.y : 0.f;
@@ -346,15 +356,16 @@
   return 0;
 }
 
-int tbn_launch_bn_bwd_reduce(const CSeg* dz, int nseg, const float* y, int P, int C, const float* scale,
+int tbn_launch_bn_bwd_reduce(const CSeg* dz, int nseg, const float* y, int y_ld, int P, int C, const float* scale,
                              const float* shift, const float* mean, const float* rstd, float* partial,
                              hipStream_t st) {
   TBN_REQUIRE(C % 4 == 0 && C <= 1024 && nseg >= 1 && nseg <= 3, "bn_bwd_reduce: bad C/nseg");
+  TBN_REQUIRE(y_ld % 4 == 0 && y_ld >= C, "bn_bwd_reduce: bad y pitch");
   CSeg3 s3;
   TBN_REQUIRE(fill_cseg3(&s3, dz, nseg) == 0, "bn_bwd_reduce: segment pitch/offset must be x4");
   const int rp = 256 / (C / 4), pch = pick_chunk(P, rp), parts = cdiv(P, pch);
   PoolGrad none = {};
-  TBN_KLAUNCH(bn_bwd_reduce_kernel<false>, dim3(parts), dim3(256), 0, st, s3, none, y, P, C, pch, scale, shift,
+  TBN_KLAUNCH(bn_bwd_reduce_kernel<false>, dim3(parts), dim3(256), 0, st, s3, none, y, y_ld, P, C, pch, scale, shift,
                      mean, rstd, partial);
   TBN_CHECK_LAUNCH("bn_bwd_reduce");
   return TBN_OK;
@@ -492,7 +503,7 @@
   s3.n = 1;
   const int rp = 256 / (C / 4), pch = pick_chunk(P, rp), parts = cdiv(P, pch);
   TBN_KLAUNCH(bn_bwd_reduce_kernel<true>, dim3(parts), dim3(256), 0, st, s3,
-                     make_poolgrad(dpooled, dpooled_ld, argmax, H, W, OH, OW, C, stride, pad), y, P, C, pch, scale,
+                     make_poolgrad(dpooled, dpooled_ld, argmax, H, W, OH, OW, C, stride, pad), y, C, P, C, pch, scale,
                      shift, mean, rstd, partial);
   TBN_CHECK_LAUNCH("bn_bwd_reduce_pooled");
   return TBN_OK;
diff --git a/attention_based_tbn_amd/csrc/engine.hip b/attention_based_tbn_amd/csrc/engine.hip
--- a/attention_based_tbn_amd/csrc/engine.hip
+++ b/attention_based_tbn_amd/csrc/engine.hip
@@ -82,6 +82,7 @@
   int kind;
   int inbuf, outbuf, out_choff, stride, pad;
   size_t argmax_off;
+  size_t ypool_off = 0;
   bool bwd_accum;
   bool fused = false;
 };
@@ -513,6 +514,11 @@
           if (c.fuse_pool >= 0) ok = false;
           cand.push_back({(int)cj, k, c.parts[k].dst_choff});
         }
+      if (c.fuse_pool >= 0 && P->pools[c.fuse_pool].outbuf == f.inbuf) {
+        const Pool& q = P->pools[c.fuse_pool];
+        if (q.out_choff != 0 || c.cout != P->bufs[f.inbuf].C) ok = false;
+        cand.push_back({(int)cj, 0, q.out_choff});
+      }
     }
     if (!ok || cand.empty() || (int)cand.size() > kMaxParts) continue;
     for (size_t a = 0; a < cand.size(); ++a)
@@ -618,10 +624,12 @@
   for (auto& c : P->convs)
     for (int k = 0; k < c.nparts; ++k)
       if (c.parts[k].red_src >= 0) {
-        const Buf& db = P->bufs[c.parts[k].dst_buf];
+        const Buf& db = P->bufs[P->convs[c.parts[k].red_src].inbuf];
         const int drows = (int)(R * db.H * db.W);
         c.parts[k].bpart_off = take(((size_t)cdiv(drows, drows <= kSk4MaxRows ? 32 : 128) + 4) * 2 * c.parts[k].cout);
       }
+  for (auto& p : P->pools)
+    if (p.fused) p.ypool_off = take(R * P->bufs[p.outbuf].H * P->bufs[p.outbuf].W * P->bufs[p.inbuf].C);
   P->coef_off = take(TBN_BN_MAXL * 3 * 1024);
   P->diag_fold_off = take(2 * 2048);
   P->wsplit_off = take(wsplit);
@@ -1055,9 +1063,13 @@
     RedSeg& r = p.red[k];
     r.y = q.pooled ? ws + q.y2_off : ws + pc.y_off + q.col0;
     r.y_ld = q.pooled ? q.cout : pc.cout;
+    if (pc.fuse_pool >= 0) {
+      r.y = ws + P->pools[pc.fuse_pool].ypool_off;
+      r.y_ld = q.cout;
+    }
     r.partial = ws + q.bpart_off;
     r.stats = ws + P->stats_off;
-    r.col_begin = q.dst_choff;
+    r.col_begin = pc.fuse_pool >= 0 ? P->pools[pc.fuse_pool].out_choff : q.dst_choff;
     r.C = q.cout;
     r.c_off = (int)q.c_off;
   }
@@ -1340,7 +1352,8 @@
                                          mean + q.c_off, rstd + q.c_off, scale + q.c_off, shift + q.c_off, st));
           TBN_TRY(tbn_launch_bn_apply_maxpool(ws + c0.y_off, (int)R, c0.outH, c0.outW, q.cout, scale + q.c_off,
                                               shift + q.c_off, ws + ob.off + pl.out_choff, ob.C,
-                                              (uint8_t*)workspace + pl.argmax_off, ob.H, ob.W, pl.stride, pl.pad, st));
+                                              (uint8_t*)workspace + pl.argmax_off, ws + pl.ypool_off, q.cout, ob.H, ob.W,
+                                              pl.stride, pl.pad, st));
         }
         continue;
       }
@@ -1698,6 +1711,7 @@
   PM->rider_launches[1] = 0;
   int deferred[8], ndef = 0;
   const bool stem_last = !br && aux == nullptr && (prm->flags & TBN_BACKBONE_STEM_WGRAD_LAST) != 0;
+  const bool pool_red_own = (prm->flags & TBN_BACKBONE_POOL_REDUCE_OWN) != 0;
   auto issue_wgrad = [&](const Conv& c, hipStream_t wst) -> int {
     tbn_prof_label(("wgrad " + c.parts[c.nparts - 1].name).c_str());
     WgradP wp;
@@ -1773,10 +1787,24 @@
         float* y = ws + c0.y_off;
         const bool bn_grad = g->dgamma && g->dbeta && (g->bn_grad_layers == 2 || (g->bn_grad_layers == 1 && s.conv[0] == 0));
         if (!diag_skip(8)) {
-          TBN_TRY(tbn_launch_bn_bwd_reduce_pooled(dpool, ob.C, am, R, c0.outH, c0.outW, ob.H, ob.W, pl.stride, pl.pad, y,
-                                                  q.cout, scale + q.c_off, shift + q.c_off, mean + q.c_off,
-                                                  rstd + q.c_off, partial, st));
-          TBN_TRY(tbn_launch_bn_bwd_finalize(partial, tbn_bn_bwd_pooled_parts(R, c0.outH, c0.outW, q.cout, pl.stride, pl.pad), M,
+          const float* red_partial = partial;
+          int red_parts = 0;
+          if (q.red_src >= 0 && !pool_red_own) {
+            const Conv& f = P->convs[q.red_src];
+            red_partial = ws + q.bpart_off;
+            red_parts = tbn_conv_red_rows(R, f.inH, f.inW, f.stride, writer_rows(P, f, GEMM_DGRAD, br));
+          } else {
+            const int rows = R * ob.H * ob.W;
+            CSeg dz;
+            dz.ptr = dpool;
+            dz.ld = ob.C;
+            dz.col_begin = 0;
+            red_parts = tbn_bn_bwd_parts(rows, q.cout);
+            TBN_REQUIRE((size_t)red_parts * 2 * q.cout <= P->partial_floats, "backbone_backward: reduce scratch too small");
+            TBN_TRY(tbn_launch_bn_bwd_reduce(&dz, 1, ws + pl.ypool_off, q.cout, rows, q.cout, scale + q.c_off, shift + q.c_off,
+                                             mean + q.c_off, rstd + q.c_off, partial, st));
+          }
+          TBN_TRY(tbn_launch_bn_bwd_finalize(red_partial, red_parts, M,
                                              q.cout, scale + q.c_off,
                                              mean + q.c_off, rstd + q.c_off, coef, bn_grad ? g->dgamma + q.c_off : nullptr,
                                              bn_grad ? g->dbeta + q.c_off : nullptr, g->dbias + q.c_off, st));
@@ -1873,6 +1901,7 @@
       tbn_prof_label(("dgrad " + c.parts[c.nparts - 1].name).c_str());
       ConvP p;
       fill_dgrad(P, c, ws, R, &p);
+      if (pool_red_own && c.nred > 0 && P->convs[c.red_conv[0]].fuse_pool >= 0) p.nred = 0;
       const RiderP* rd = (bpend_host == o.idx) ? &bpend : nullptr;
       if (rd != nullptr) {
         bpend_host = -1;
diff --git a/attention_based_tbn_amd/csrc/tbn_kernels.h b/attention_based_tbn_amd/csrc/tbn_kernels.h
--- a/attention_based_tbn_amd/csrc/tbn_kernels.h
+++ b/attention_based_tbn_amd/csrc/tbn_kernels.h
@@ -249,8 +249,8 @@
 int tbn_launch_bn_apply(const float* y, int P, int C, const float* scale, const float* shift, const Seg* segs,
                         int nseg, hipStream_t st);
 int tbn_launch_bn_apply_maxpool(const float* y, int N, int H, int W, int C, const float* scale, const float* shift,
-                                float* out, int out_ld, unsigned char* argmax, int OH, int OW, int stride, int pad,
-                                hipStream_t st);
+                                float* out, int out_ld, unsigned char* argmax, float* ypool, int ypool_ld, int OH, int OW,
+                                int stride, int pad, hipStream_t st);
 int tbn_launch_bn_bwd_reduce_pooled(const float* dpooled, int dpooled_ld, const unsigned char* argmax, int N, int H,
                                     int W, int OH, int OW, int stride, int pad, const float* y, int C,
                                     const float* scale, const float* shift, const float* mean, const float* rstd,
@@ -306,7 +306,7 @@
 int tbn_launch_bn_fold(const float* gamma, const float* beta, const float* mean, const float* var, const float* bias,
                        float eps, float* scale, float* shift, int C, hipStream_t st);
 int tbn_bn_bwd_parts(int P, int C);
-int tbn_launch_bn_bwd_reduce(const CSeg* dz, int nseg, const float* y, int P, int C, const float* scale,
+int tbn_launch_bn_bwd_reduce(const CSeg* dz, int nseg, const float* y, int y_ld, int P, int C, const float* scale,
                              const float* shift, const float* mean, const float* rstd, float* partial, hipStream_t st);
 int tbn_launch_bn_bwd_finalize(const float* partial, int nparts, int P, int C, const float* scale, const float* mean,
                                const float* rstd, float* coef, float* dgamma, float* dbeta, float* dbias,
diff --git a/attention_based_tbn_amd/ops_conv.py b/attention_based_tbn_amd/ops_conv.py
--- a/attention_based_tbn_amd/ops_conv.py
+++ b/attention_based_tbn_amd/ops_conv.py
@@ -375,13 +375,14 @@
         stats = torch.empty(4, cout, device=x.device, dtype=torch.float32)
         bnws = torch.empty(lib().tbn_bn_workspace_floats(m, cout), device=x.device, dtype=torch.float32)
         rm, rv = state.running_mean, state.running_var
-        call("tbn_bn_relu_maxpool_train_fwd", ptr(y), n, oh, ow, cout, ptr(gamma), ptr(beta), ptr(rm), ptr(rv), MOMENTUM,
-             EPS, stats[0].data_ptr(), stats[1].data_ptr(), stats[2].data_ptr(), stats[3].data_ptr(), ptr(pooled), cout,
-             ptr(argmax), ph, pw, 2, 1, ptr(bnws), st)
+        ypool = torch.empty(n, ph, pw, cout, device=x.device, dtype=torch.float32)
+        call("tbn_bn_relu_maxpool_ypool_train_fwd", ptr(y), n, oh, ow, cout, ptr(gamma), ptr(beta), ptr(rm), ptr(rv),
+             MOMENTUM, EPS, stats[0].data_ptr(), stats[1].data_ptr(), stats[2].data_ptr(), stats[3].data_ptr(), ptr(pooled),
+             cout, ptr(argmax), ptr(ypool), cout, ph, pw, 2, 1, ptr(bnws), st)
         if rm is not None:
             torch.autograd.graph.increment_version((rm, rv))
         if ctx.live:
-            ctx.save_for_backward(x, y, argmax, stats)
+            ctx.save_for_backward(x, y, argmax, stats, ypool)
         return pooled
 
     @staticmethod
@@ -393,7 +394,7 @@
             if ctx.eval_mode and any(need[1:4]):
                 raise TbnHipError(_EVAL_BACKWARD.format(ctx.who))
             return (None,) * 7
-        x, y, argmax, stats = ctx.saved_tensors
+        x, y, argmax, stats, ypool = ctx.saved_tensors
         n, cin, h, w = x.shape
         _, oh, ow, cout = y.shape
         ph, pw = argmax.shape[1], argmax.shape[2]
@@ -403,8 +404,8 @@
         dy = torch.empty_like(y)
         dgb = torch.empty(2, cout, device=x.device, dtype=torch.float32)
         bnws = torch.empty(lib().tbn_bn_workspace_floats(m, cout), device=x.device, dtype=torch.float32)
-        call("tbn_bn_relu_maxpool_train_bwd", ptr(dpooled), cout, ptr(argmax), ptr(y), n, oh, ow, cout, ph, pw, 2, 1,
-             stats[0].data_ptr(), stats[1].data_ptr(), stats[2].data_ptr(), stats[3].data_ptr(), ptr(dy),
+        call("tbn_bn_relu_maxpool_ypool_train_bwd", ptr(dpooled), cout, ptr(argmax), ptr(ypool), cout, ptr(y), n, oh, ow,
+             cout, ph, pw, 2, 1, stats[0].data_ptr(), stats[1].data_ptr(), stats[2].data_ptr(), stats[3].data_ptr(), ptr(dy),
              dgb[0].data_ptr(), dgb[1].data_ptr(), ptr(bnws), st)
         dw = None
         if need[1]:
diff --git a/include/tbn_hip.h b/include/tbn_hip.h
--- a/include/tbn_hip.h
+++ b/include/tbn_hip.h
@@ -55,6 +55,7 @@
 #define TBN_BACKBONE_STEM_WGRAD_LAST 2
 #define TBN_BACKBONE_WEIGHTS_FLIPPED 4
 #define TBN_BACKBONE_CONV_BF16X6 8
+#define TBN_BACKBONE_POOL_REDUCE_OWN 64
 #define TBN_BACKBONE_CONV_BF16X3 16
 #define TBN_BACKBONE_CONV_BF16X_ALL 32
 
@@ -187,6 +188,16 @@
                                   int w, int c, int oh, int ow, int stride, int pad, const float* save_mean,
                                   const float* save_rstd, const float* scale, const float* shift, float* dy,
                                   float* dgamma, float* dbeta, float* workspace, void* stream);
+int tbn_bn_relu_maxpool_ypool_train_fwd(const float* y, int n, int h, int w, int c, const float* gamma, const float* beta,
+                                        float* running_mean, float* running_var, float momentum, float eps, float* save_mean,
+                                        float* save_rstd, float* scale, float* shift, float* pooled, int pooled_ld,
+                                        uint8_t* argmax, float* ypool, int ypool_ld, int oh, int ow, int stride, int pad,
+                                        float* workspace, void* stream);
+int tbn_bn_relu_maxpool_ypool_train_bwd(const float* dpooled, int dpooled_ld, const uint8_t* argmax, const float* ypool,
+                                        int ypool_ld, const float* y, int n, int h, int w, int c, int oh, int ow, int stride,
+                                        int pad, const float* save_mean, const float* save_rstd, const float* scale,
+                                        const float* shift, float* dy, float* dgamma, float* dbeta, float* workspace,
+                                        void* stream);
 
 typedef struct {
   float* ptr;
```

Measured after the change: 918.6 clips/s (median of 6 runs). About the same (+0.7%).
